# tyb311/TCCT

Hardware: AMD Instinct MI355X
Metric: OCT B-scans/sec fwd+bwd(+clip+AdamW), stc_tt bs=8 1x800x1100 (higher is better)
Workload: dtype bf16; 1 GPU; stc_tt --los=di bs=8/GPU 1x800x1100 (net tensors 3x800x1104); global_batch=8, parallelism=dp1, ranks=1, grad_allreduce=none, slowest_step=101

## Files before the change

include/tcct_hip.h:

```cpp
#ifndef TCCT_HIP_H
#define TCCT_HIP_H
#include <stdint.h>
#ifdef __cplusplus
extern "C" {
#endif

typedef void* tcct_stream_t;

enum { TCCT_F32 = 0, TCCT_BF16 = 1 };
enum { TCCT_ACT_NONE = 0, TCCT_ACT_LRELU = 1, TCCT_ACT_HSWISH = 2, TCCT_ACT_GELU = 3, TCCT_ACT_SIGMOID = 4,
       TCCT_ACT_ABS = 5 };

int tcct_version(void);
const char* tcct_last_error(void);
int tcct_set_outputs_prezeroed(int on);

int tcct_image_to_nhwc4(const float* img, void* out, int N, int Csrc, int H, int Wsrc, int Wdst, int dtype,
                        tcct_stream_t stream);
int tcct_u8_gather2d(const uint8_t* src, uint8_t* dst, int N, int SH, int SW, int C, int sy0, int sx0, int sh, int sw, int DH, int DW,
                     int dy0, int dx0, int dh, int dw, int flipy, int flipx, int mul, int div, int fill, tcct_stream_t stream);
int tcct_onehot_to_index(const int64_t* onehot, uint8_t* lab, int N, int C, int64_t HW, tcct_stream_t stream);
int tcct_labels_to_u8(const int64_t* lab, uint8_t* out, int N, int H, int Wsrc, int Wdst, tcct_stream_t stream);
int tcct_nhwc_to_nchw_f32(const void* x, float* y, int N, int64_t HW, int C, int dtype, tcct_stream_t stream);

// ... 74 lines not shown
                      int KW, int padh, int padw, int dy_dtype, int dx_dtype, tcct_stream_t stream);
int tcct_conv2d_wgrad(const void* x, const void* dy, float* dw, float* dbias, int N, int H, int W, int Cin,
                      int Cin_w, int Cout, int KH, int KW, int stride, int padh, int padw, int x_dtype, int dy_dtype,
                      tcct_stream_t stream);

int tcct_conv32f_pack_weights(const float* w, float* wp, int KH, int KW, int transposed, tcct_stream_t stream);
int tcct_conv32f_fwd(const float* x, const float* wp, const float* bias, const float* yadd, float* y, int N, int H, int W, int KH, int KW, int PH,
                     int PW, tcct_stream_t stream);
int tcct_conv32f_wgrad(const float* x, const float* dy, float* dw, float* dbias, int N, int H, int W, int KH, int KW, int PH, int PW,
                       tcct_stream_t stream);
int tcct_conv32f_pack_weights_sub(const float* w, float* wp, int KH, int KW, int transposed, int cin_total, int o_off, int i_off, tcct_stream_t stream);
int tcct_conv32f_fwd_strided(const float* x, const float* wp, const float* bias, float* y, int N, int H, int W, int KH, int KW, int PH, int PW, int xs,
                             int xo, int ys, int yo, int accumulate, tcct_stream_t stream);
int tcct_conv32f_wgrad_strided(const float* x, const float* dy, float* dw, float* dbias, int N, int H, int W, int KH, int KW, int PH, int PW, int xs,
                               int xo, int ds, int dof, int ldi, int o_off, int i_off, tcct_stream_t stream);
int tcct_pwf_fwd(const float* x, const float* w, const float* bias, float* y, int64_t M, int K, int N, int transposed, tcct_stream_t stream);
int tcct_pwf_wgrad(const float* x, const float* dy, float* dw, float* dbias, int64_t M, int K, int N, tcct_stream_t stream);
int tcct_conv32_pack_weights(const float* w, void* wp, int KH, int KW, int transposed, tcct_stream_t stream);
int tcct_conv32_pack_weights_multi(const void* desc, int n, tcct_stream_t stream);
int tcct_conv32_pack_weights_both(const float* w, void* wp2, int KH, int KW, tcct_stream_t stream);
int tcct_conv32_fwd(const void* x, const void* wp, const float* bias, void* y, int N, int H, int W, int KH, int KW, int PH,
                    int PW, tcct_stream_t stream);

int tcct_conv32_fwd_bnstats(const void* x, const void* wp, const float* bias, void* y, int N, int H, int W, int KH, int KW, int PH,
                            int PW, double* stats, int pre_act, tcct_stream_t stream);
int tcct_conv32_fwd_affine(const void* x, const void* wp, const float* bias, void* y, int N, int H, int W, int KH, int KW,
                           int PH, int PW, const float* ab, int pre_act, int post_act, tcct_stream_t stream);
int tcct_pw_fwd_affine(const void* x, const float* w, const float* bias, void* y, int64_t M, int K, int N, const float* ab,
                       int pre_act, int post_act, int out_dtype, tcct_stream_t stream);
int tcct_pw_fwd_affine_residual(const void* x, const float* w, const float* bias, const float* ab, const void* res, void* y, int64_t M, int K, int N,
                                tcct_stream_t stream);
int tcct_pw_fwd_cat2_affine(const void* x1, const void* x2, const float* w, const float* bias, const float* ab, int post_act, void* y, int64_t M, int K, int N,
                            tcct_stream_t stream);
int tcct_pw_fwd_xaff_affine_residual(const void* y_prev, const float* ab_prev, const float* w, const float* bias, const float* ab, const void* res, void* y,
                                     int64_t M, int K, int N, tcct_stream_t stream);
int tcct_conv32_fwd_add(const void* x, const void* wp, const float* bias, const void* res, void* y, int N, int H, int W, int KH, int KW,
                        int PH, int PW, tcct_stream_t stream);
int tcct_conv32_chain33(const void* x, const void* wp1, const float* bias1, void* mid, const void* wp2, const float* bias2, void* y,
                        const void* res, int N, int H, int W, double* stats, tcct_stream_t stream);
int tcct_conv32_pack_weights_sub(const float* w, void* wp, int KH, int KW, int transposed, int cin_total, int o_off, int i_off,
                                 tcct_stream_t stream);
int tcct_conv32_fwd_strided(const void* x, const void* wp, const float* bias, void* y, int N, int H, int W, int KH, int KW, int PH,
                            int PW, int xs, int xo, int ys, int yo, int accumulate, tcct_stream_t stream);
int tcct_conv32_fwd_strided_bnstats(const void* x, const void* wp, const float* bias, void* y, int N, int H, int W, int KH, int KW, int PH,
                                    int PW, int xs, int xo, int ys, int yo, int accumulate, double* stats, int pre_act, tcct_stream_t stream);
int tcct_conv32_fwd_strided_affine(const void* x, const void* wp, const float* bias, void* y, int N, int H, int W, int KH, int KW, int PH, int PW, int xs,
                                   int xo, int ys, int yo, const float* ab, int pre_act, int post_act, tcct_stream_t stream);
int64_t tcct_conv32_wgrad_mode(int mode);
int64_t tcct_conv32_fwd_mode(int mode);
int tcct_conv32_wgrad_strided(const void* x, const void* dy, float* dw, float* dbias, int N, int H, int W, int KH, int KW, int PH,
                              int PW, int xs, int xo, int ds, int dof, int cin_total, int o_off, int i_off, tcct_stream_t stream);
int tcct_conv32_wgrad(const void* x, const void* dy, float* dw, float* dbias, int N, int H, int W, int KH, int KW, int PH,
                      int PW, tcct_stream_t stream);
int tcct_conv32_bwd3x3(const void* x, const void* dy, const void* wp_t, const void* dskip, void* dx, float* dw, float* dbias, int N, int H,
                       int W, tcct_stream_t stream);

int tcct_pw_fwd(const void* x, const float* w, const float* bias, void* y, int64_t M, int K, int N, int transposed,
                int out_dtype, tcct_stream_t stream);
int tcct_pw_wgrad(const void* x, const void* dy, float* dw, float* dbias, int64_t M, int K, int N, tcct_stream_t stream);
int tcct_pw_bwd(const void* x, const void* dy, const float* w, const void* res, void* dx, float* dw, float* dbias, int64_t M, int K, int N,
                tcct_stream_t stream);
int tcct_pw_bwd_cat2(const void* x1, const void* x2, const void* dy, const float* w, void* dx1, void* dx2, float* dw, int64_t M, int K, int N,
                     tcct_stream_t stream);
int tcct_pw_bwd_residual2(const void* x, const void* dy, const float* w, const void* res, void* dx_sum, void* dx_plain, float* dw, float* dbias,
                          int64_t M, int K, int N, tcct_stream_t stream);
int64_t tcct_pw_bwd_bn_supported(int K, int N, int post, int red_post, int split);
int tcct_pw_bwd_bn(const void* x, const void* x2, const void* dz, const void* y, const float* coef, int post, const float* w, const void* res,
                   void* dx, void* dx2, float* dw, float* dbias, int64_t M, int K, int N, const void* y_prev, const float* ab_prev,
                   int red_post, double* sums_prev, tcct_stream_t stream);
int tcct_pw_bwd_bn_sums(const void* x, const void* x2, const void* dz, const void* y, const double* sums, int raw, const float* mean_rstd,
                        const float* ab, float* dgamma, float* dbeta, int post, const float* w, const void* res, void* dx, void* dx2, float* dw,
                        float* dbias, int64_t M, int K, int N, const void* y_prev, const float* ab_prev, int red_post, double* sums_prev,
                        tcct_stream_t stream);
int tcct_pw_wgrad_strided(const void* x, const void* dy, int64_t ldy, float* dw, float* dbias, int64_t M, int K, int N,
                          tcct_stream_t stream);
int tcct_pw_fwd_residual(const void* x, const float* w, const float* bias, const void* res, const float* scale, int64_t per_sample,
                         void* y, void* y_plain, int64_t M, int K, int N, tcct_stream_t stream);
int tcct_pw_fwd_bnstats_xaff(const void* y_prev, const float* ab_prev, const float* w, const float* bias, void* y, int64_t M, int K, int N, double* stats,
                             tcct_stream_t stream);
int tcct_pw_bwd_bn_sums_xaff(const void* y_prev, const float* ab_prev, const void* dz, const void* y, const double* sums, int raw, const float* mean_rstd,
                             const float* ab, float* dgamma, float* dbeta, const float* w, const void* res, void* dx, float* dw, float* dbias, int64_t M,
                             int K, int N, int red_post, double* sums_prev, tcct_stream_t stream);
int tcct_pw_fwd_gelu_residual(const void* x1, const float* w, const float* bias, const void* res, const float* scale, int64_t per_sample, void* y,
                              int64_t M, int K, int N, tcct_stream_t stream);
int tcct_pw_bwd_residual2_sum(const void* x, const void* dy_a, const void* dy_b, const float* w, const void* res, void* dx_sum, void* dx_plain, float* dw,
                              float* dbias, int64_t M, int K, int N, tcct_stream_t stream);
int tcct_pw_bwd_lnb(const void* x, const void* dy, const float* w, const void* t, const float* mean_rstd, const float* gamma, const void* res, void* dt,
                    float* dw, float* dbias, float* dgamma, float* dbeta, int64_t M, int K, int N, tcct_stream_t stream);
int tcct_pw_bwd_gelu(const void* x1, const void* dy, const float* w, void* dx1, float* dw, float* dbias, int64_t M, int K, int N, tcct_stream_t stream);
int tcct_pw_dgrad_residual(const void* dy, const float* w, const void* res, void* dx_sum, void* dx_plain, int64_t M, int Nout, int K,
                           tcct_stream_t stream);
int tcct_pw_fwd_cat2(const void* x1, const void* x2, int K1, const float* w, const float* bias, void* y, int64_t M, int K, int N,
                     double* stats, int pre_act, tcct_stream_t stream);
int tcct_pw_fwd_f32_upadd(const void* x, const float* w, const float* bias, float* y, int B, int uH, int uW, int K, int N, const float* up, tcct_stream_t stream);
int tcct_pw_dgrad_split2(const void* dy, const float* w, void* dx1, void* dx2, int K1, int64_t M, int Nout, int K, tcct_stream_t stream);
int tcct_pw_bwd_cat2_bias(const void* x1, const void* x2, const void* dy, const float* w, void* dx1, void* dx2, float* dw, float* dbias, int64_t M,
                          int K, int N, tcct_stream_t stream);
int tcct_tail_compose(const float* w1, const float* b1, const float* w2, const float* b2, float* wc, float* c, tcct_stream_t stream);
int tcct_tail_compose_bwd(const float* w1, const float* b1, const float* w2, const float* dwc, const float* dc, float* dw1, float* db1, float* dw2,
                          float* db2, tcct_stream_t stream);
int tcct_tail_compose3(const float* w1, const float* b1, const float* w2, const float* b2, const float* w3, const float* b3, int C, float* wcc, float* wa,
                       float* wb, float* ccc, tcct_stream_t stream);
int tcct_tail_compose3_bwd(const float* w1, const float* b1, const float* w2, const float* b2, const float* w3, int C, const float* dwa, const float* dwb,
                           const float* dccc, float* dw1, float* db1, float* dw2, float* db2, float* dw3, float* db3, tcct_stream_t stream);
int tcct_pw_fwd_cat2_f32(const void* x1, const void* x2, int K1, const float* w, const float* bias, float* y, int64_t M, int K, int N, tcct_stream_t stream);
int tcct_head_compose(const float* wt, const float* bt, const float* wa, const float* ba, int C, float* wh, float* ch, tcct_stream_t stream);
int tcct_head_compose_bwd(const float* wt, const float* bt, const float* wa, int C, const float* dwh, const float* dch, float* dwt, float* dbt,
                          float* dwa, float* dba, tcct_stream_t stream);
int tcct_pw_wgrad_cat2(const void* x1, const void* x2, int K1, const void* dy, float* dw, float* dbias, int64_t M, int K, int N,
                       tcct_stream_t stream);
int tcct_pw_fwd_bnstats(const void* x, const float* w, const float* bias, void* y, int64_t M, int K, int N, double* stats, int pre_act,
                        tcct_stream_t stream);

int tcct_im2col3x3_c3(const void* x4, void* out, int N, int H, int W, int stride, int dtype, tcct_stream_t stream);
int tcct_c3_fwd(const void* x4, const float* w, const float* bias, void* y, int B, int H, int W, int stride, double* stats, int stat_pre,
                const float* ab, int pre_act, int post_act, tcct_stream_t stream);
int tcct_c3_wgrad(const void* x4, const void* dy, float* dw, float* dbias, int B, int H, int W, int stride, tcct_stream_t stream);
int tcct_c3_bn_fwd_train(const void* x4, const float* w, const float* bias, void* z, int B, int H, int W, int stride, double* sums,
                         const float* gamma, const float* beta, float eps, float momentum, float* running_mean, float* running_var,
                         int64_t* num_batches_tracked, float* mean_rstd, float* ab, int post_act, tcct_stream_t stream);
int tcct_c3_bn_fwd_eval(const void* x4, const float* w, const float* bias, void* z, int B, int H, int W, int stride, const float* ab, int post_act,
                        tcct_stream_t stream);
int tcct_c3_bn_bwd_reduce(const void* x4, const float* w, const float* bias, const void* dz, int B, int H, int W, int stride, const float* ab,
                          double* raw, int post_act, tcct_stream_t stream);
int tcct_c3_bn_bwd_wgrad(const void* x4, const float* w, const float* bias, const void* dz, int B, int H, int W, int stride, const float* coef,
                         float* dw, float* dbias, int post_act, tcct_stream_t stream);
int64_t tcct_c3_bn_bwd_prefetch(int tiles_ahead);
int tcct_c3_bn_bwd_onepass(const void* x4, const float* w, const float* bias, const void* dz, int B, int H, int W, int stride, const float* mean_rstd,
                           const float* ab, float* work, double* sums, float* dw, float* dbias, float* dgamma, float* dbeta, int post_act, tcct_stream_t stream);
int tcct_pw_wgrad_smalln(const void* x, const void* dy, float* dw, float* dbias, int64_t M, int K, int N, int x_dtype,
                         int dy_dtype, tcct_stream_t stream);

int tcct_stream_copy(const void* src, void* dst, int64_t nbytes, tcct_stream_t stream);

int64_t tcct_kernel_census(int which, int reset);
int tcct_marker(int id, tcct_stream_t stream);

int tcct_dwconv3x3_fwd(const void* x, const float* w, const float* bias, void* y, int N, int H, int W, int C,
                       int stride, int add_input, int dtype, tcct_stream_t stream);
int tcct_dwconv3x3_fwd_bnstats(const void* x, const float* w, const float* bias, void* y, int N, int H, int W, int C, int stride,
                               int add_input, double* stats, int dtype, tcct_stream_t stream);
int tcct_dwconv3x3_dgrad(const void* dy, const float* w, void* dx, int N, int H, int W, int C, int stride,
                         int add_input, int dtype, tcct_stream_t stream);
int tcct_dwconv3x3_dgrad_add(const void* dy, const float* w, const void* res, void* dx, int N, int H, int W, int C, int stride,
                             int add_input, int dtype, tcct_stream_t stream);
int tcct_dwconv3x3_wgrad(const void* x, const void* dy, float* dw, float* dbias, int N, int H, int W, int C,
                         int stride, int dtype, tcct_stream_t stream);
int tcct_dwconv3x3_fwd_xaff(const void* x, const float* xab, const float* w, const float* bias, void* y, int N, int H, int W, int C, int stride,
                            double* stats, int dtype, tcct_stream_t stream);
int tcct_dwconv3x3_wgrad_xaff(const void* x, const float* xab, const void* dy, float* dw, float* dbias, int N, int H, int W, int C, int stride, int dtype,
                              tcct_stream_t stream);
int tcct_dwconv3x3_dgrad_bnred(const void* dy, const float* w, const void* y_prev, const float* ab_prev, void* dx, double* raw, int N, int H, int W, int C,
                               int dtype, tcct_stream_t stream);

int tcct_metapool_fwd(const void* x, void* y, int B, int64_t N, int C, int dtype, tcct_stream_t stream);
int tcct_metapool_bwd(const void* dy, void* dx, int B, int64_t N, int C, int dtype, tcct_stream_t stream);
int tcct_metapool_residual_fwd(const void* x, const void* res, const float* scale, void* y, int B, int64_t N, int C, int dtype,
                               tcct_stream_t stream);
int tcct_metapool_scaled_bwd(const void* dy, const float* scale, void* dx, int B, int64_t N, int C, int dtype, tcct_stream_t stream);
int tcct_ln_metapool_residual_fwd(const void* t, void* y, int B, int64_t N, int C, const float* gamma, const float* beta, float eps, const float* scale,
                                  int dtype, tcct_stream_t stream);
int tcct_ln_metapool_residual_ln_fwd(const void* t, void* y, void* y2, int B, int64_t N, int C, const float* gamma, const float* beta, float eps,
                                     const float* scale, const float* gamma2, const float* beta2, float eps2, float* mean_rstd2, int dtype, tcct_stream_t stream);
int tcct_ln_metapool_residual_bwd(const void* t, const void* dy, void* dt, int B, int64_t N, int C, const float* gamma, float eps, const float* scale,
                                  float* dgamma, float* dbeta, int dtype, tcct_stream_t stream);
int tcct_maxpool2_fwd(const void* x, void* y, int N, int H, int W, int C, int dtype, tcct_stream_t stream);
int tcct_maxpool2_bwd(const void* x, const void* dy, void* dx, int N, int H, int W, int C, int dtype, tcct_stream_t stream);
int tcct_maxpool2_bwd_add(const void* x, const void* dy, const void* res, void* dx, int N, int H, int W, int C, int dtype,
                          tcct_stream_t stream);
int tcct_bilinear_fwd(const void* x, void* y, int N, int H, int W, int C, int Ho, int Wo, int align_corners, int dtype,
                      tcct_stream_t stream);
int tcct_bilinear_bwd_separable(const float* dy, float* dx, float* workspace, int N, int H, int W, int C, int Ho, int Wo,
                                int align_corners, tcct_stream_t stream);
int tcct_bilinear_add_fwd(const void* x, const void* res, void* y, int N, int H, int W, int C, int Ho, int Wo, int align_corners,
                          int dtype, tcct_stream_t stream);
int64_t tcct_bilinear_bwd_x2(int on);
int tcct_bilinear_bwd(const void* dy, void* dx, int N, int H, int W, int C, int Ho, int Wo, int align_corners, int dtype,
                      tcct_stream_t stream);
int tcct_l2norm_fwd(const void* x, void* y, int64_t M, int C, float eps, int dtype, tcct_stream_t stream);
int tcct_l2norm_bwd(const void* x, const void* dy, void* dx, int64_t M, int C, float eps, int dtype, tcct_stream_t stream);
int tcct_l2norm_bwd_scaled(const void* x, const void* dy, void* dx, int64_t M, int C, float eps, float scale, int dtype,
                           tcct_stream_t stream);
int tcct_l2norm_bwd_scaled_add(const void* x, const void* dy, const void* res, void* dx, int64_t M, int C, float eps, float scale, int dtype,
                               tcct_stream_t stream);
int tcct_normadd_fwd(const void* g0, const void* g1, const void* g2, float* inv1, float* inv2, void* out, int N, int H, int W, int C,
                     int h1, int w1, int h2, int w2, float eps, int dtype, tcct_stream_t stream);

int tcct_softmax_dice_fwd(const void* logits, const uint8_t* labels, int64_t M, int C, double* sums, float* loss,
                          int dtype, tcct_stream_t stream);
int tcct_softmax_dice_bwd(const void* logits, const uint8_t* labels, int64_t M, int C, const double* sums,
                          const float* grad_out, float grad_scale, void* dlogits, int dtype, tcct_stream_t stream);
int tcct_updice_fwd(const float* low, const uint8_t* labels, int B, int h, int w, int H, int W, int C, double* sums, float* loss,
                    tcct_stream_t stream);
int tcct_updice_bwd(const float* low, const uint8_t* labels, int B, int h, int w, int H, int W, int C, const double* sums,
                    const float* grad_out, float grad_scale, float* ws, float* dlow, tcct_stream_t stream);
int tcct_dice_ds_fwd(const void* logits, int dtype, const uint8_t* labels, int B, int H, int W, int C, const float* low1, int h1, int w1, const float* low2,
                     int h2, int w2, const float* low3, int h3, int w3, float coff, double* sums, float* loss, tcct_stream_t stream);
int tcct_softmax_pick(const void* logits, const uint8_t* labels, int64_t M, int C, float* prob_lab, uint8_t* argmax,
                      int dtype, tcct_stream_t stream);
int tcct_confusion_counts(const uint8_t* pred, const uint8_t* labels, int N, int64_t HW, int C, float* out,
                          tcct_stream_t stream);

int tcct_gate_fusion_fwd(const void* x1, const void* x2, const float* field, void* y, int N, int H, int W, int C, int hs, int ws,
                         int dtype, tcct_stream_t stream);
int tcct_gate_fusion_bwd(const void* dy, const float* field, void* dx1, void* dx2, int N, int H, int W, int C, int hs, int ws,
                         int dtype, tcct_stream_t stream);

int tcct_mask_boundaries(const uint8_t* mask, int32_t* out, int N, int H, int W, int C, tcct_stream_t stream);

int tcct_slice_channels_fwd(const void* x, float* y, int64_t M, int C, int start, int n, int dtype, tcct_stream_t stream);
int tcct_slice_channels_bwd(const float* dy, void* dx, int64_t M, int C, int start, int n, int dtype, tcct_stream_t stream);
int tcct_label_planes(const uint8_t* labels, float* onehot, float* edge, int N, int H, int W, int start, int n,
                      tcct_stream_t stream);
int tcct_gumbel_colsoftmax_fwd(const float* x, const float* eps, float* out, float* stats, int N, int H, int W, int CH,
                               tcct_stream_t stream);
int tcct_gumbel_colsoftmax_bwd(const float* x, const float* eps, const float* stats, const float* dout, float* dx, int N,
                               int H, int W, int CH, tcct_stream_t stream);
int tcct_colsoftmax_fwd(const float* x, float* y, int N, int H, int W, tcct_stream_t stream);
int tcct_colsoftmax_bwd(const float* y, const float* dy, float* dx, int N, int H, int W, tcct_stream_t stream);
int tcct_colwsum_fwd(const float* x, const float* wts, float* out, int N, int H, int W, tcct_stream_t stream);
int tcct_colwsum_bwd(const float* dout, const float* wts, float* dx, int N, int H, int W, tcct_stream_t stream);
int tcct_mse_fwd(const float* a, const float* b, int64_t n, double* acc, float* out, tcct_stream_t stream);
int tcct_mse_bwd(const float* a, const float* b, int64_t n, const float* grad_out, float grad_scale, float* da, float* db,
                 tcct_stream_t stream);

int64_t tcct_fpl_select_workspace_bytes();
int tcct_fpl_select(const void* feat, const uint8_t* labels, const float* prob, int64_t M, int C, void* workspace, uint32_t* counts,
                    uint8_t* binmap, float* pro_sum, int dtype, tcct_stream_t stream);
int tcct_fpl_loss(const float* pro_sum, const uint32_t* counts, const float* buf_grad, int C, float* pro, float* loss, float* dpro_over_n,
                  tcct_stream_t stream);
int tcct_fpl_backward(const uint8_t* labels, const uint8_t* binmap, const float* dpro_over_n, const float* grad_out,
                      float grad_scale, int64_t M, void* dfeat, int dtype, tcct_stream_t stream);
int tcct_l2norm_bwd_fplgrad(const void* x, const uint8_t* labels, const uint8_t* binmap, const float* dpro_over_n, const float* grad_out,
                            float grad_scale, int ncls, const void* res, void* dx, int64_t M, float eps, float scale, int dtype, tcct_stream_t stream);
int tcct_bilinear_bwd_fplgrad(const uint8_t* labels, const uint8_t* binmap, const float* dpro_over_n, const float* grad_out, float grad_scale, int ncls,
                              void* dx, int N, int H, int W, int Ho, int Wo, int align_corners, int dtype, tcct_stream_t stream);

int64_t tcct_fatt_kstats_workspace_bytes(int B, int64_t N, int C);
int tcct_fatt_kstats(const void* qkv, void* workspace, float* stats, int B, int64_t N, int C, int heads, int dtype, tcct_stream_t stream);
int tcct_fatt_ktv(const void* qkv, const float* stats, float* M, int B, int64_t N, int C, int heads, int dtype, tcct_stream_t stream);
int tcct_fatt_dktv(const void* qkv, const void* dout, float* dM, float scale, int B, int64_t N, int C, int heads, int dtype,
                   tcct_stream_t stream);
int tcct_fatt_apply_fwd(const void* qkv, const float* M, const void* cv, void* out, float scale, int B, int64_t N, int C, int heads,
                        int dtype, tcct_stream_t stream);
int tcct_fatt_apply_bwd(const void* qkv, const float* stats, const float* M, const float* dM, const void* cv, const void* dout,
                        void* dqkv, void* dcv, float scale, int B, int64_t N, int C, int heads, int dtype, tcct_stream_t stream);
int tcct_dwk_strided_fwd(const void* x, int64_t ldx, const float* w, const float* bias, void* y, int64_t ldy, int B, int H, int W, int Cg,
                         int K, int flip, int accumulate, int dtype, tcct_stream_t stream);
int tcct_dwk_strided_wgrad(const void* x, int64_t ldx, const void* dy, int64_t ldy, float* dw, float* dbias, int B, int H, int W, int Cg,
                           int K, int dtype, tcct_stream_t stream);

int tcct_grad_sumsq(const float* g, int64_t n, double* acc, tcct_stream_t stream);
int tcct_clip_adamw(float* p, const float* g, float* m, float* v, int64_t n, const double* sumsq, float max_norm,
                    float grad_mul, float lr, double beta1, double beta2, float eps, float weight_decay, int step,
                    float* total_norm_out, tcct_stream_t stream);

int tcct_clip_adamw_dev(float* p, const float* g, float* m, float* v, int64_t n, const double* sumsq, float max_norm,
                        float grad_mul, float* state, double beta1, double beta2, float eps, float weight_decay,
                        float* total_norm_out, tcct_stream_t stream);

#ifdef __cplusplus
}
#endif
#endif
```

tcct_amd/csrc/dwconv.hip:

```cpp
#include "common.h"
#include <cstdlib>
#include <type_traits>

#define DB 256

template <typename T, int VEC>
__device__ __forceinline__ void ldv(const T* p, float* o) {
    if (VEC == 4) { f4 a = ld4(p); o[0] = a.v[0]; o[1] = a.v[1]; o[2] = a.v[2]; o[3] = a.v[3]; }
    else o[0] = ldf(p);
}
template <typename T, int VEC>
__device__ __forceinline__ void stv(T* p, const float* o) {
    if (VEC == 4) { f4 a; a.v[0] = o[0]; a.v[1] = o[1]; a.v[2] = o[2]; a.v[3] = o[3]; st4(p, a); }
    else stf(p, o[0]);
}

struct DwPos { int n, ho0, ho1, wo, c; };
__device__ __forceinline__ bool dw_pos(int C, int VEC, int Ho, int Wo, int segh, int wblocks, int hstrips, DwPos& p, int cpt = 1) {
    const int CV = C / VEC, PW = DB / CV, t = threadIdx.x;
    if (t >= PW * CV) return false;
    int bid = (int)xcd_band(blockIdx.x, gridDim.x);
    const int wb = bid % wblocks; bid /= wblocks;
    const int hs = bid % hstrips;
    p.n = bid / hstrips;
// ... 177 lines not shown
                        for (int ky = 0; ky < 3; ++ky)
#pragma unroll
                            for (int kx = 0; kx < 3; ++kx) a += R[j * STRIDE + ky][cc + kx].get(k) * wk[ky * 3 + kx][k];
                        if (add_input) a += R[j * STRIDE + 1][cc + 1].get(k);
                        acc[k] = a;
                    }
                    const bool live = ho + j < p.ho1 && cout[cc] != DW_OOB;
                    dw_storeb(ry, live ? (uint32_t)(ho + j) * (uint32_t)(Wo * C) * ES + cout[cc] : DW_OOB, acc, (const T*)nullptr);
                    if (stats && live) {
                        if (aux_mode) {
#pragma unroll
                            for (int k = 0; k < VEC; ++k) {
                                const float yv = RS[j][cc].get(k), u = xa[k] * yv + xb[k];
                                const float d = dw_rnd(acc[k], (const T*)nullptr) * (u < -3.f ? 0.f : (u <= 3.f ? (2.f * u + 3.f) * (1.f / 6.f) : 1.f));
                                st_s[k] += (SAcc)d; st_q[k] += (SAcc)d * (SAcc)yv;
                            }
                        } else {
#pragma unroll
                            for (int k = 0; k < VEC; ++k) { const SAcc r = dw_rnd(acc[k], (const T*)nullptr); st_s[k] += r; st_q[k] += r * r; }
                        }
                    }
                }
            }
#pragma unroll
            for (int i = 0; i < K::CARRY; ++i)
#pragma unroll
                for (int kx = 0; kx < NC; ++kx) R[i][kx] = R[NEWC + i][kx];
#pragma unroll
            for (int i = 0; i < NEWC; ++i)
#pragma unroll
                for (int kx = 0; kx < NC; ++kx) R[K::CARRY + i][kx] = NX[i][kx];
#pragma unroll
            for (int j = 0; j < RBC; ++j)
#pragma unroll
                for (int cc = 0; cc < CPT; ++cc) RS[j][cc] = RSN[j][cc];
        }
    } else {
#pragma unroll
    for (int i = 0; i < ROWSC; ++i) dw_load_row<T, VEC, NC>(R[i], img, p.ho0 * STRIDE - 1 + i, H, W, C, wi0);
    for (int ho = p.ho0; ho < p.ho1; ho += RBC) {
        if (ho + RBC < p.ho1) {
#pragma unroll
            for (int i = 0; i < NEWC; ++i) dw_load_row<T, VEC, NC>(NX[i], img, (ho + RBC) * STRIDE - 1 + K::CARRY + i, H, W, C, wi0);
        }
#pragma unroll
        for (int j = 0; j < RBC; ++j) {
            if (ho + j < p.ho1) {
#pragma unroll
                for (int cc = 0; cc < CPT; ++cc) {
                    if (CPT > 1 && p.wo + cc >= Wo) break;
                    float acc[VEC];
                    Raw<T, VEC> rr;
                    if (rin) rr.load(rin + ((int64_t)(ho + j) * Wo + p.wo + cc) * C); else rr.zero();
#pragma unroll
                    for (int k = 0; k < VEC; ++k) {
                        float a = bv[k] + rr.get(k);
#pragma unroll
                        for (int ky = 0; ky < 3; ++ky)
#pragma unroll
                            for (int kx = 0; kx < 3; ++kx) a += R[j * STRIDE + ky][cc + kx].get(k) * wk[ky * 3 + kx][k];
                        if (add_input) a += R[j * STRIDE + 1][cc + 1].get(k);
                        acc[k] = a;
                    }
                    stv<T, VEC>(out + ((int64_t)(ho + j) * Wo + p.wo + cc) * C, acc);
                }
            }
        }
#pragma unroll
        for (int i = 0; i < K::CARRY; ++i)
#pragma unroll
            for (int kx = 0; kx < NC; ++kx) R[i][kx] = R[NEWC + i][kx];
#pragma unroll
        for (int i = 0; i < NEWC; ++i)
#pragma unroll
            for (int kx = 0; kx < NC; ++kx) R[K::CARRY + i][kx] = NX[i][kx];
    }
    }
    }
    if (VEC == 4 && stats) {
        const int CV = C / VEC, PW = DB / CV, t = threadIdx.x;
#pragma unroll
        for (int k = 0; k < VEC; ++k) { s_red[t * 8 + k] = st_s[k]; s_red[t * 8 + 4 + k] = st_q[k]; }
        __syncthreads();
        if (t < C) {
            const int cvv = t / VEC, k = t % VEC;
            double a = 0.0, b = 0.0;
            for (int pp = 0; pp < PW; ++pp) { a += (double)s_red[(pp * CV + cvv) * 8 + k]; b += (double)s_red[(pp * CV + cvv) * 8 + 4 + k]; }
            atomicAdd(&stats[t], a); atomicAdd(&stats[C + t], b);
        }
    }
}

static void dw_geometry(int N, int Ho, int Wo, int C, int vec, int target_blocks, int max_segh, int& segh, int& wblocks, int& hstrips,
                        int cpt = 1) {
    const int PW = DB / (C / vec) * cpt;
    wblocks = (Wo + PW - 1) / PW;
    segh = max_segh;
    while (segh > 8 && (int64_t)N * wblocks * ((Ho + segh - 1) / segh) < target_blocks) segh >>= 1;
    hstrips = (Ho + segh - 1) / segh;
}

template <typename T, int VEC, bool FLIP, int MODE = 0>
static void dw_fwd_launch(const void* x, const float* w, const float* bias, void* y, int N, int H, int W, int C, int stride,
                          int Ho, int Wo, int add_input, hipStream_t st, const void* res = nullptr, double* stats = nullptr, const float* xab = nullptr) {
    int segh, wblocks, hstrips;
    static int cpt_on = -1;
    if (cpt_on < 0) cpt_on = 1;
    if (stride == 1 && VEC == 4 && sizeof(T) == 2 && cpt_on && Wo >= 128 && C >= 32) {
        dw_geometry(N, Ho, Wo, C, VEC, 1024, 32, segh, wblocks, hstrips, 4);
        dim3 g4((unsigned)((int64_t)N * wblocks * hstrips));
        hipLaunchKernelGGL((k_dw_fwd<T, VEC, 1, FLIP, (VEC == 4 ? 4 : 1), MODE>), g4, dim3(DB), 0, st, (const T*)x, w, bias, (T*)y, N, H, W, C, Ho, Wo, add_input, segh, wblocks, hstrips, (const T*)res, stats, xab);
        return;
    }
    dw_geometry(N, Ho, Wo, C, VEC, 1024, 32, segh, wblocks, hstrips);
    dim3 g((unsigned)((int64_t)N * wblocks * hstrips)), b(DB);
    if (stride == 1) hipLaunchKernelGGL((k_dw_fwd<T, VEC, 1, FLIP, 1, MODE>), g, b, 0, st, (const T*)x, w, bias, (T*)y, N, H, W, C, Ho, Wo, add_input, segh, wblocks, hstrips, (const T*)res, stats, xab);
    else hipLaunchKernelGGL((k_dw_fwd<T, VEC, 2, FLIP, 1, MODE>), g, b, 0, st, (const T*)x, w, bias, (T*)y, N, H, W, C, Ho, Wo, add_input, segh, wblocks, hstrips, (const T*)res, stats, xab);
}

extern "C" int tcct_dwconv3x3_fwd(const void* x, const float* w, const float* bias, void* y, int N, int H, int W, int C,
                                  int stride, int add_input, int dtype, tcct_stream_t stream) {
    TCCT_CHECK(stride == 1 || stride == 2, "dwconv3x3_fwd: stride %d", stride);
    TCCT_CHECK(!(add_input && stride != 1), "dwconv3x3_fwd: add_input needs stride 1");
    TCCT_CHECK(N >= 1 && H >= 1 && W >= 1 && C >= 1, "dwconv3x3_fwd: empty tensor");
    int Ho = (H + 2 - 3) / stride + 1, Wo = (W + 2 - 3) / stride + 1;
    int vec = (C % 4 == 0) ? 4 : 1;
    TCCT_CHECK(C / vec <= DB, "dwconv3x3_fwd: C=%d too large", C);
    TCCT_CHECK((int64_t)H * W * C * 4 < (1ll << 31), "dwconv3x3_fwd: one image of %d x %d x %d elements exceeds the 32-bit byte offsets of the kernels", H, W, C);
    hipStream_t st = (hipStream_t)stream;
    if (vec == 4) { TCCT_DISPATCH(dtype, (dw_fwd_launch<T, 4, false>(x, w, bias, y, N, H, W, C, stride, Ho, Wo, add_input, st))); }
    else { TCCT_DISPATCH(dtype, (dw_fwd_launch<T, 1, false>(x, w, bias, y, N, H, W, C, stride, Ho, Wo, add_input, st))); }
    TCCT_LAUNCH_OK();
}
extern "C" int tcct_dwconv3x3_fwd_bnstats(const void* x, const float* w, const float* bias, void* y, int N, int H, int W, int C, int stride,
                                          int add_input, double* stats, int dtype, tcct_stream_t stream) {
    TCCT_CHECK(stride == 1 || stride == 2, "dwconv3x3_fwd_bnstats: stride %d", stride);
    TCCT_CHECK(!(add_input && stride != 1), "dwconv3x3_fwd_bnstats: add_input needs stride 1");
    TCCT_CHECK(N >= 1 && H >= 1 && W >= 1 && C >= 4 && C % 4 == 0 && C <= DB && stats != nullptr, "dwconv3x3_fwd_bnstats: needs C %% 4 == 0, C <= 256, stats");
    TCCT_CHECK((int64_t)H * W * C * 4 < (1ll << 31), "dwconv3x3_fwd_bnstats: one image of %d x %d x %d elements exceeds the 32-bit byte offsets of the kernels", H, W, C);
    int Ho = (H + 2 - 3) / stride + 1, Wo = (W + 2 - 3) / stride + 1;
    TCCT_DISPATCH(dtype, (dw_fwd_launch<T, 4, false>(x, w, bias, y, N, H, W, C, stride, Ho, Wo, add_input, (hipStream_t)stream, nullptr, stats)));
    TCCT_LAUNCH_OK();
}
extern "C" int tcct_dwconv3x3_fwd_xaff(const void* x, const float* xab, const float* w, const float* bias, void* y, int N, int H, int W, int C, int stride,
                                       double* stats, int dtype, tcct_stream_t stream) {
    TCCT_CHECK(stride == 1 || stride == 2, "dwconv3x3_fwd_xaff: stride %d", stride);
    TCCT_CHECK(N >= 1 && H >= 1 && W >= 1 && C >= 4 && C % 4 == 0 && C <= DB && xab != nullptr, "dwconv3x3_fwd_xaff: needs C %% 4 == 0, C <= 256, xab");
    TCCT_CHECK((int64_t)H * W * C * 4 < (1ll << 31), "dwconv3x3_fwd_xaff: one image of %d x %d x %d elements exceeds the 32-bit byte offsets of the kernels", H, W, C);
    int Ho = (H + 2 - 3) / stride + 1, Wo = (W + 2 - 3) / stride + 1;
    TCCT_DISPATCH(dtype, (dw_fwd_launch<T, 4, false, 1>(x, w, bias, y, N, H, W, C, stride, Ho, Wo, 0, (hipStream_t)stream, nullptr, stats, xab)));
    TCCT_LAUNCH_OK();
}

template <typename T, int VEC>
__global__ void __launch_bounds__(DB) k_dw_dgrad_s2(const T* __restrict__ dy, const float* __restrict__ w, T* __restrict__ dx,
                                                    int N, int H, int W, int C, int Ho, int Wo, int segh, int wblocks, int hstrips,
                                                    const T* __restrict__ res) {
    const int Qh = (H + 1) / 2, Qw = (W + 1) / 2;
    DwPos p;
    if (!dw_pos(C, VEC, Qh, Qw, segh, wblocks, hstrips, p)) return;
    float wk[9][VEC];
#pragma unroll
    for (int k = 0; k < VEC; ++k)
#pragma unroll
        for (int tp = 0; tp < 9; ++tp) wk[tp][k] = w[(p.c + k) * 9 + tp];
    const T* g = dy + (int64_t)p.n * Ho * Wo * C + p.c;
    T* out = dx + (int64_t)p.n * H * W * C + p.c;
    const T* rin = res ? res + (int64_t)p.n * H * W * C + p.c : nullptr;
    const int b = p.wo;
    if (VEC == 4) {
        const uint32_t ES = sizeof(T), in_bytes = (uint32_t)H * W * C * ES;
        const int nu = __builtin_amdgcn_readfirstlane(p.n);
        const __amdgpu_buffer_rsrc_t rg = __builtin_amdgcn_make_buffer_rsrc((void*)(dy + (int64_t)nu * Ho * Wo * C), 0, (uint32_t)Ho * Wo * C * ES, 0x00020000);
        const __amdgpu_buffer_rsrc_t ro = __builtin_amdgcn_make_buffer_rsrc((void*)(dx + (int64_t)nu * H * W * C), 0, in_bytes, 0x00020000);
        const __amdgpu_buffer_rsrc_t rr = __builtin_amdgcn_make_buffer_rsrc((void*)((res ? res : dx) + (int64_t)nu * H * W * C), 0, res ? in_bytes : 0u, 0x00020000);
        const uint32_t cg0 = (uint32_t)(b * C + p.c) * ES, cg1 = b + 1 < Wo ? cg0 + (uint32_t)C * ES : DW_OOB;
        const uint32_t co0 = (uint32_t)(2 * b * C + p.c) * ES, co1 = 2 * b + 1 < W ? co0 + (uint32_t)C * ES : DW_OOB;
        auto ldb = [&](Raw<T, VEC> (&d)[2], int a) {
            const bool rok = a < Ho;
            const uint32_t r0 = (uint32_t)a * (uint32_t)(Wo * C) * ES;
            d[0].loadb(rg, rok ? r0 + cg0 : DW_OOB);
            d[1].loadb(rg, (rok && cg1 != DW_OOB) ? r0 + cg1 : DW_OOB);
        };
        auto ldr = [&](Raw<T, VEC> (&q)[4], int a, bool live) {
            const uint32_t r0 = (uint32_t)(2 * a) * (uint32_t)(W * C) * ES, r1 = r0 + (uint32_t)(W * C) * ES;
            const bool row1 = live && 2 * a + 1 < H;
            q[0].loadb(rr, live ? r0 + co0 : DW_OOB);
            q[1].loadb(rr, (live && co1 != DW_OOB) ? r0 + co1 : DW_OOB);
            q[2].loadb(rr, row1 ? r1 + co0 : DW_OOB);
            q[3].loadb(rr, (row1 && co1 != DW_OOB) ? r1 + co1 : DW_OOB);
        };
        auto emitb = [&](const Raw<T, VEC> (&u)[2], const Raw<T, VEC> (&v)[2], const Raw<T, VEC> (&q)[4], int a, bool live) {
            float o00[VEC], o01[VEC], o10[VEC], o11[VEC];
#pragma unroll
            for (int k = 0; k < VEC; ++k) {
                const float u0 = u[0].get(k), u1 = u[1].get(k), v0 = v[0].get(k), v1 = v[1].get(k);
                o00[k] = u0 * wk[4][k] + q[0].get(k);
                o01[k] = u0 * wk[5][k] + u1 * wk[3][k] + q[1].get(k);
                o10[k] = u0 * wk[7][k] + v0 * wk[1][k] + q[2].get(k);
                o11[k] = u0 * wk[8][k] + u1 * wk[6][k] + v0 * wk[2][k] + v1 * wk[0][k] + q[3].get(k);
            }
            const uint32_t r0 = (uint32_t)(2 * a) * (uint32_t)(W * C) * ES, r1 = r0 + (uint32_t)(W * C) * ES;
            const bool row1 = live && 2 * a + 1 < H;
            dw_storeb(ro, live ? r0 + co0 : DW_OOB, o00, (const T*)nullptr);
            dw_storeb(ro, (live && co1 != DW_OOB) ? r0 + co1 : DW_OOB, o01, (const T*)nullptr);
            dw_storeb(ro, row1 ? r1 + co0 : DW_OOB, o10, (const T*)nullptr);
            dw_storeb(ro, (row1 && co1 != DW_OOB) ? r1 + co1 : DW_OOB, o11, (const T*)nullptr);
        };
        Raw<T, VEC> d0[2], d1[2], d2[2], n1[2], n2[2], q0[4], q1[4], m0[4], m1[4];
        ldb(d0, p.ho0); ldb(d1, p.ho0 + 1); ldb(d2, p.ho0 + 2);
        ldr(q0, p.ho0, true); ldr(q1, p.ho0 + 1, p.ho0 + 1 < p.ho1);
        for (int a = p.ho0; a < p.ho1; a += 2) {
            const bool more = a + 2 < p.ho1;
            ldb(n1, more ? a + 3 : Ho); ldb(n2, more ? a + 4 : Ho);
            ldr(m0, a + 2, more); ldr(m1, a + 3, a + 3 < p.ho1);
            emitb(d0, d1, q0, a, true);
            emitb(d1, d2, q1, a + 1, a + 1 < p.ho1);
#pragma unroll
            for (int j = 0; j < 2; ++j) { d0[j] = d2[j]; d1[j] = n1[j]; d2[j] = n2[j]; }
#pragma unroll
            for (int j = 0; j < 4; ++j) { q0[j] = m0[j]; q1[j] = m1[j]; }
        }
        return;
    }
    auto ld = [&](float (&d)[2][VEC], int a) {
#pragma unroll
        for (int j = 0; j < 2; ++j) {
            if (a < Ho && b + j < Wo) ldv<T, VEC>(g + ((int64_t)a * Wo + b + j) * C, d[j]);
            else {
#pragma unroll
                for (int k = 0; k < VEC; ++k) d[j][k] = 0.f;
            }
        }
    };
    auto emit = [&](const float (&u)[2][VEC], const float (&v)[2][VEC], int a) {
        float o00[VEC], o01[VEC], o10[VEC], o11[VEC];
#pragma unroll
        for (int k = 0; k < VEC; ++k) {
            o00[k] = u[0][k] * wk[4][k];
            o01[k] = u[0][k] * wk[5][k] + u[1][k] * wk[3][k];
            o10[k] = u[0][k] * wk[7][k] + v[0][k] * wk[1][k];
            o11[k] = u[0][k] * wk[8][k] + u[1][k] * wk[6][k] + v[0][k] * wk[2][k] + v[1][k] * wk[0][k];
        }
        const int hi = 2 * a, wi = 2 * b;
        T* o = out + ((int64_t)hi * W + wi) * C;
        if (rin) {
            const T* ri = rin + ((int64_t)hi * W + wi) * C;
            float r[VEC];
            ldv<T, VEC>(ri, r);
#pragma unroll
            for (int k = 0; k < VEC; ++k) o00[k] += r[k];
            if (wi + 1 < W) {
                ldv<T, VEC>(ri + C, r);
#pragma unroll
                for (int k = 0; k < VEC; ++k) o01[k] += r[k];
            }
            if (hi + 1 < H) {
                ldv<T, VEC>(ri + (int64_t)W * C, r);
#pragma unroll
                for (int k = 0; k < VEC; ++k) o10[k] += r[k];
                if (wi + 1 < W) {
                    ldv<T, VEC>(ri + (int64_t)W * C + C, r);
#pragma unroll
                    for (int k = 0; k < VEC; ++k) o11[k] += r[k];
                }
            }
        }
        stv<T, VEC>(o, o00);
        if (wi + 1 < W) stv<T, VEC>(o + C, o01);
        if (hi + 1 < H) {
            stv<T, VEC>(o + (int64_t)W * C, o10);
            if (wi + 1 < W) stv<T, VEC>(o + (int64_t)W * C + C, o11);
        }
    };
    float d0[2][VEC], d1[2][VEC];
    ld(d0, p.ho0);
    for (int a = p.ho0; a < p.ho1; a += 2) {
        ld(d1, a + 1);
        emit(d0, d1, a);
        if (a + 1 >= p.ho1) break;
        ld(d0, a + 2);
        emit(d1, d0, a + 1);
    }
}

static int dw_dgrad_impl(const void* dy, const float* w, const void* res, void* dx, int N, int H, int W, int C, int stride,
                         int add_input, int dtype, tcct_stream_t stream) {
    TCCT_CHECK(stride == 1 || stride == 2, "dwconv3x3_dgrad: stride %d", stride);
    TCCT_CHECK(!(add_input && stride != 1), "dwconv3x3_dgrad: add_input needs stride 1");
    TCCT_CHECK(N >= 1 && H >= 1 && W >= 1 && C >= 1, "dwconv3x3_dgrad: empty tensor");
    int Ho = (H + 2 - 3) / stride + 1, Wo = (W + 2 - 3) / stride + 1;
    int vec = (C % 4 == 0) ? 4 : 1;
    TCCT_CHECK(C / vec <= DB, "dwconv3x3_dgrad: C=%d too large", C);
    TCCT_CHECK((int64_t)H * W * C * 4 < (1ll << 31), "dwconv3x3_dgrad: one image of %d x %d x %d elements exceeds the 32-bit byte offsets of the kernels", H, W, C);
    hipStream_t st = (hipStream_t)stream;
    if (stride == 1) {
        if (vec == 4) { TCCT_DISPATCH(dtype, (dw_fwd_launch<T, 4, true>(dy, w, nullptr, dx, N, H, W, C, 1, H, W, add_input, st, res))); }
        else { TCCT_DISPATCH(dtype, (dw_fwd_launch<T, 1, true>(dy, w, nullptr, dx, N, H, W, C, 1, H, W, add_input, st, res))); }
        TCCT_LAUNCH_OK();
    }
    int segh, wblocks, hstrips;
    dw_geometry(N, (H + 1) / 2, (W + 1) / 2, C, vec, 1024, 32, segh, wblocks, hstrips);
    dim3 g((unsigned)((int64_t)N * wblocks * hstrips)), b(DB);
    if (vec == 4) { TCCT_DISPATCH(dtype, hipLaunchKernelGGL((k_dw_dgrad_s2<T, 4>), g, b, 0, st, (const T*)dy, w, (T*)dx, N, H, W, C, Ho, Wo, segh, wblocks, hstrips, (const T*)res)); }
    else { TCCT_DISPATCH(dtype, hipLaunchKernelGGL((k_dw_dgrad_s2<T, 1>), g, b, 0, st, (const T*)dy, w, (T*)dx, N, H, W, C, Ho, Wo, segh, wblocks, hstrips, (const T*)res)); }
    TCCT_LAUNCH_OK();
}
extern "C" int tcct_dwconv3x3_dgrad(const void* dy, const float* w, void* dx, int N, int H, int W, int C, int stride,
                                    int add_input, int dtype, tcct_stream_t stream) {
    return dw_dgrad_impl(dy, w, nullptr, dx, N, H, W, C, stride, add_input, dtype, stream);
}
extern "C" int tcct_dwconv3x3_dgrad_add(const void* dy, const float* w, const void* res, void* dx, int N, int H, int W, int C,
                                        int stride, int add_input, int dtype, tcct_stream_t stream) {
    TCCT_CHECK(res != nullptr, "dwconv3x3_dgrad_add: res is NULL");
    return dw_dgrad_impl(dy, w, res, dx, N, H, W, C, stride, add_input, dtype, stream);
}

extern "C" int tcct_dwconv3x3_dgrad_bnred(const void* dy, const float* w, const void* y_prev, const float* ab_prev, void* dx, double* raw, int N, int H, int W,
                                          int C, int dtype, tcct_stream_t stream) {
    TCCT_CHECK(N >= 1 && H >= 1 && W >= 1 && C >= 4 && C % 4 == 0 && C <= DB && y_prev && ab_prev && raw, "dwconv3x3_dgrad_bnred: needs C %% 4 == 0, C <= 256, y_prev, ab_prev, raw");
    TCCT_CHECK((int64_t)H * W * C * 4 < (1ll << 31), "dwconv3x3_dgrad_bnred: one image of %d x %d x %d elements exceeds the 32-bit byte offsets of the kernels", H, W, C);
    TCCT_DISPATCH(dtype, (dw_fwd_launch<T, 4, true, 2>(dy, w, nullptr, dx, N, H, W, C, 1, H, W, 0, (hipStream_t)stream, y_prev, raw, ab_prev)));
    TCCT_LAUNCH_OK();
}

template <typename T, int VEC, int STRIDE, int CPT = 1, bool XAFF = false>
__global__ void __launch_bounds__(DB) k_dw_wgrad(const T* __restrict__ x, const T* __restrict__ dy, float* __restrict__ dw,
                                                 float* __restrict__ dbias, int N, int H, int W, int C, int Ho, int Wo, int segh,
                                                 int wblocks, int hstrips, const float* __restrict__ xab = nullptr) {
    static_assert(CPT == 1 || (STRIDE == 1 && VEC == 4), "several columns per thread: stride 1, 4-channel vectors");
    constexpr int NC = CPT + 2;
    extern __shared__ float sm[];
    const int CV = C / VEC, PW = DB / CV;
    const int t = threadIdx.x;
    float acc[10][VEC];
#pragma unroll
    for (int a = 0; a < 10; ++a)
#pragma unroll
        for (int k = 0; k < VEC; ++k) acc[a][k] = 0.f;
    typedef DwChunk<STRIDE> K;
    DwPos p;
    if (dw_pos(C, VEC, Ho, Wo, segh, wblocks, hstrips, p, CPT)) {
        const T* img = x + (int64_t)p.n * H * W * C + p.c;
        const T* gimg = dy + (int64_t)p.n * Ho * Wo * C + p.c;
        const int wi0 = p.wo * STRIDE - 1;
      if (VEC == 4) {
        Raw<T, VEC> R[K::ROWS][NC], NX[K::NEW][NC], G[K::RB][CPT], GX[K::RB][CPT];
        const uint32_t ES = sizeof(T);
        const int nu = __builtin_amdgcn_readfirstlane(p.n);
        const __amdgpu_buffer_rsrc_t rx = __builtin_amdgcn_make_buffer_rsrc((void*)(x + (int64_t)nu * H * W * C), 0, (uint32_t)H * W * C * ES, 0x00020000);
        const __amdgpu_buffer_rsrc_t rg = __builtin_amdgcn_make_buffer_rsrc((void*)(dy + (int64_t)nu * Ho * Wo * C), 0, (uint32_t)Ho * Wo * C * ES, 0x00020000);
        uint32_t cin[NC], cg[CPT];
#pragma unroll
        for (int kx = 0; kx < NC; ++kx) cin[kx] = (unsigned)(wi0 + kx) < (unsigned)W ? (uint32_t)((wi0 + kx) * C + p.c) * ES : DW_OOB;
#pragma unroll
        for (int cc = 0; cc < CPT; ++cc) cg[cc] = p.wo + cc < Wo ? (uint32_t)((p.wo + cc) * C + p.c) * ES : DW_OOB;
        auto load_row = [&](Raw<T, VEC> (&r)[NC], int hi, bool live) {
            const bool rok = live && (unsigned)hi < (unsigned)H;
            const uint32_t ro = (uint32_t)hi * (uint32_t)(W * C) * ES;
#pragma unroll
            for (int kx = 0; kx < NC; ++kx) r[kx].loadb(rx, (rok && cin[kx] != DW_OOB) ? ro + cin[kx] : DW_OOB);
        };
        auto load_g = [&](Raw<T, VEC> (&g)[K::RB][CPT], int ho) {
#pragma unroll
            for (int j = 0; j < K::RB; ++j)
#pragma unroll
                for (int cc = 0; cc < CPT; ++cc)
                    g[j][cc].loadb(rg, (ho + j < p.ho1 && cg[cc] != DW_OOB) ? (uint32_t)(ho + j) * (uint32_t)(Wo * C) * ES + cg[cc] : DW_OOB);
        };
#pragma unroll
        for (int i = 0; i < K::ROWS; ++i) load_row(R[i], p.ho0 * STRIDE - 1 + i, true);
        float xa[VEC], xb[VEC];
#pragma unroll
        for (int k = 0; k < VEC; ++k) { xa[k] = XAFF ? xab[p.c + k] : 1.f; xb[k] = XAFF ? xab[C + p.c + k] : 0.f; }
        auto xf_row = [&](Raw<T, VEC> (&r)[NC], int hi, bool live) {
            const bool rok = live && (unsigned)hi < (unsigned)H;
#pragma unroll
            for (int kx = 0; kx < NC; ++kx) r[kx] = dw_xf(r[kx], xa, xb, rok && cin[kx] != DW_OOB);
        };
        if (XAFF) {
#pragma unroll
            for (int i = 0; i < K::CARRY; ++i) xf_row(R[i], p.ho0 * STRIDE - 1 + i, true);
        }
        load_g(G, p.ho0);
        for (int ho = p.ho0; ho < p.ho1; ho += K::RB) {
            const bool more = ho + K::RB < p.ho1;
#pragma unroll
            for (int i = 0; i < K::NEW; ++i) load_row(NX[i], (ho + K::RB) * STRIDE - 1 + K::CARRY + i, more);
            load_g(GX, ho + K::RB);
            if (XAFF) {
#pragma unroll
                for (int i = 0; i < K::NEW; ++i) xf_row(R[K::CARRY + i], ho * STRIDE - 1 + K::CARRY + i, true);
            }
#pragma unroll
            for (int j = 0; j < K::RB; ++j) {
#pragma unroll
                for (int cc = 0; cc < CPT; ++cc) {
#pragma unroll
                    for (int k = 0; k < VEC; ++k) {
                        const float g = G[j][cc].get(k);
                        acc[9][k] += g;
#pragma unroll
                        for (int ky = 0; ky < 3; ++ky)
#pragma unroll
                            for (int kx = 0; kx < 3; ++kx) acc[ky * 3 + kx][k] += R[j * STRIDE + ky][cc + kx].get(k) * g;
                    }
                }
            }
#pragma unroll
            for (int i = 0; i < K::CARRY; ++i)
#pragma unroll
                for (int kx = 0; kx < NC; ++kx) R[i][kx] = R[K::NEW + i][kx];
#pragma unroll
            for (int i = 0; i < K::NEW; ++i)
#pragma unroll
                for (int kx = 0; kx < NC; ++kx) R[K::CARRY + i][kx] = NX[i][kx];
#pragma unroll
            for (int j = 0; j < K::RB; ++j)
#pragma unroll
                for (int cc = 0; cc < CPT; ++cc) G[j][cc] = GX[j][cc];
        }
      } else {
        Raw<T, VEC> R[K::ROWS][3], NX[K::NEW][3], G[K::RB], GX[K::RB];
#pragma unroll
        for (int i = 0; i < K::ROWS; ++i) dw_load_row<T, VEC>(R[i], img, p.ho0 * STRIDE - 1 + i, H, W, C, wi0);
#pragma unroll
        for (int j = 0; j < K::RB; ++j) {
            if (p.ho0 + j < p.ho1) G[j].load(gimg + ((int64_t)(p.ho0 + j) * Wo + p.wo) * C);
            else G[j].zero();
        }
        for (int ho = p.ho0; ho < p.ho1; ho += K::RB) {
            if (ho + K::RB < p.ho1) {
#pragma unroll
                for (int i = 0; i < K::NEW; ++i) dw_load_row<T, VEC>(NX[i], img, (ho + K::RB) * STRIDE - 1 + K::CARRY + i, H, W, C, wi0);
#pragma unroll
                for (int j = 0; j < K::RB; ++j) {
                    if (ho + K::RB + j < p.ho1) GX[j].load(gimg + ((int64_t)(ho + K::RB + j) * Wo + p.wo) * C);
                    else GX[j].zero();
                }
            }
#pragma unroll
            for (int j = 0; j < K::RB; ++j) {
#pragma unroll
                for (int k = 0; k < VEC; ++k) {
                    const float g = G[j].get(k);
                    acc[9][k] += g;
#pragma unroll
                    for (int ky = 0; ky < 3; ++ky)
#pragma unroll
                        for (int kx = 0; kx < 3; ++kx) acc[ky * 3 + kx][k] += R[j * STRIDE + ky][kx].get(k) * g;
                }
            }
#pragma unroll
            for (int i = 0; i < K::CARRY; ++i)
#pragma unroll
                for (int kx = 0; kx < 3; ++kx) R[i][kx] = R[K::NEW + i][kx];
#pragma unroll
            for (int i = 0; i < K::NEW; ++i)
#pragma unroll
                for (int kx = 0; kx < 3; ++kx) R[K::CARRY + i][kx] = NX[i][kx];
#pragma unroll
            for (int j = 0; j < K::RB; ++j) G[j] = GX[j];
        }
      }
    }
#pragma unroll
    for (int a = 0; a < 10; ++a)
#pragma unroll
        for (int k = 0; k < VEC; ++k) sm[(t * 10 + a) * VEC + k] = acc[a][k];
    __syncthreads();
    for (int o = t; o < C * 10; o += DB) {
        int ch = o / 10, a = o % 10;
        int cvv = ch / VEC, k = ch % VEC;
        float s = 0.f;
        for (int pp = 0; pp < PW; ++pp) s += sm[((pp * CV + cvv) * 10 + a) * VEC + k];
// ... 51 lines not shown
```

tcct_amd/csrc/pw_mfma.hip:

```cpp
#include "common.h"
#include "c3_geom.h"
#include <cstdlib>

typedef __attribute__((ext_vector_type(8))) __bf16 bf16x8;
typedef __attribute__((ext_vector_type(16))) float f32x16;
typedef __attribute__((ext_vector_type(4))) short s16x4;
typedef __attribute__((ext_vector_type(8))) short s16x8;
typedef __attribute__((__vector_size__(4 * sizeof(unsigned int)))) unsigned int u32x4;

#define PWB 256

__device__ __forceinline__ void st_out4(bf16* p, float a, float b, float c, float d) {
    uint2 o; o.x = pack_bf16x2(a, b); o.y = pack_bf16x2(c, d);
    *reinterpret_cast<uint2*>(p) = o;
}
__device__ __forceinline__ void st_out4(float* p, float a, float b, float c, float d) {
    *reinterpret_cast<float4*>(p) = make_float4(a, b, c, d);
}

__device__ __forceinline__ float rnd_out(float v, const bf16*) { return __bfloat162float(__float2bfloat16(v)); }
__device__ __forceinline__ float rnd_out(float v, const float*) { return v; }

struct PwUp { const float* p; int uH, uW, Ho, Wo; float sh, sw; uint32_t m_howo, m_wo; };
struct PwSplit { const bf16* x2; int K1; void* y2; int N1; const bf16* res; const float* rscale; int64_t per_sample; bf16* yplain; C3Geom c3; PwUp up; };
// ... 1038 lines not shown
                    }
                };
                if (SPLIT) {
                    const uint32_t off2 = mm < M ? (uint32_t)((mm * KS + (kt * 32) % KS + cch * 8) * 2) : 0x80000000u;
                    __builtin_amdgcn_raw_buffer_store_b128(o, kt * 32 < KS ? ro : rp, off2, 0, 0);
                    if (RED && kt < RKT) red_acc(o, kt * 32 + cch * 8);
                    continue;
                }
                const uint32_t off = mm < M ? (uint32_t)((mm * K + kt * 32 + cch * 8) * 2) : 0x80000000u;
                if (GX) {
                    const u32x4 xv = xq[GX ? kt : 0][h2];
#pragma unroll
                    for (int k = 0; k < 4; ++k)
                        o[k] = pack_bf16x2(__uint_as_float(o[k] << 16) * gelu_grad1(__uint_as_float(xv[k] << 16)),
                                           __uint_as_float(o[k] & 0xffff0000u) * gelu_grad1(__uint_as_float(xv[k] & 0xffff0000u)));
                }
                if (res) {
                    if (dx_plain) __builtin_amdgcn_raw_buffer_store_b128(o, rp, off, 0, 0);
                    const u32x4 rv = __builtin_amdgcn_raw_buffer_load_b128(rr, off, 0, 0);
#pragma unroll
                    for (int k = 0; k < 4; ++k)
                        o[k] = pack_bf16x2(__uint_as_float(o[k] << 16) + __uint_as_float(rv[k] << 16),
                                           __uint_as_float(o[k] & 0xffff0000u) + __uint_as_float(rv[k] & 0xffff0000u));
                }
                __builtin_amdgcn_raw_buffer_store_b128(o, ro, off, 0, 0);
                if (RED) red_acc(o, kt * 32 + cch * 8);
            }
            wave_lds_fence();
        }
        __syncthreads();
    }
    if (RED) {
        __syncthreads();
        float* red = reinterpret_cast<float*>(smem);
        constexpr int KR = SPLIT ? K / 2 : K;
#pragma unroll
        for (int kt = 0; kt < RKT; ++kt) {
#pragma unroll
            for (int k = 0; k < 8; ++k) {
                float a = rs[kt][k], b = rq[kt][k];
#pragma unroll
                for (int o = 32; o > 2; o >>= 1) { a += __shfl_xor(a, o, 64); b += __shfl_xor(b, o, 64); }
                if (lane < 4) {
                    red[wave * 2 * KR + kt * 32 + 8 * lane + k] = a;
                    red[wave * 2 * KR + KR + kt * 32 + 8 * lane + k] = b;
                }
            }
        }
        __syncthreads();
        for (int i2 = tid; i2 < KR; i2 += PWB) {
            double a = 0.0, b = 0.0;
#pragma unroll
            for (int wv = 0; wv < 4; ++wv) { a += (double)red[wv * 2 * KR + i2]; b += (double)red[wv * 2 * KR + KR + i2]; }
            atomicAdd(&bn.sums_prev[i2], a); atomicAdd(&bn.sums_prev[KR + i2], b);
        }
        __syncthreads();
    }
    if (LNB) {
        __syncthreads();
        float* red = reinterpret_cast<float*>(smem);
#pragma unroll
        for (int kt = 0; kt < KT; ++kt) {
#pragma unroll
            for (int k = 0; k < 8; ++k) {
                float a = rs[kt][k], b = rq[kt][k];
#pragma unroll
                for (int o = 32; o > 2; o >>= 1) { a += __shfl_xor(a, o, 64); b += __shfl_xor(b, o, 64); }
                if (lane < 4) {
                    red[wave * 2 * K + kt * 32 + 8 * lane + k] = a;
                    red[wave * 2 * K + K + kt * 32 + 8 * lane + k] = b;
                }
            }
        }
        __syncthreads();
        for (int i2 = tid; i2 < K; i2 += PWB) {
            float a = 0.f, b = 0.f;
#pragma unroll
            for (int wv = 0; wv < 4; ++wv) { a += red[wv * 2 * K + i2]; b += red[wv * 2 * K + K + i2]; }
            atomicAdd(&bn.dgamma[i2], a); atomicAdd(&bn.dbeta[i2], b);
        }
        __syncthreads();
    }
#pragma unroll
    for (int a = 0; a < (NT * KT + 3) / 4; ++a) {
        const int ti = wave + 4 * a;
        if (ti < NT * KT) {
            const int ct = ti / KT, kt = ti - ct * KT;
#pragma unroll
            for (int k = 0; k < 16; ++k) {
                const int co = ct * 32 + (k & 3) + 8 * (k >> 2) + 4 * hh;
                atomicAdd(&dw[(int64_t)co * K + kt * 32 + r], accw[a][k]);
            }
            if (dbias && kt == 0) {
                const float sb = bsum[a] + __shfl_xor(bsum[a], 32, 64);
                if (lane < 32) atomicAdd(&dbias[ct * 32 + r], sb);
            }
        }
    }
}

static int pw_bwd_impl(const void* x, const void* dy, const float* w, const void* res, void* dx, void* dx_plain, float* dw, float* dbias,
                       int64_t M, int K, int N, tcct_stream_t stream, bool split = false, int bnp = -1, int redp = -1,
                       PwBnBwd bn = PwBnBwd{nullptr, nullptr, nullptr, nullptr, nullptr, nullptr, 0, nullptr, nullptr, nullptr, nullptr}, bool gelu_x = false,
                       int xap = -1, bool lnb = false, bool dy2 = false);
extern "C" int tcct_pw_bwd_cat2(const void* x1, const void* x2, const void* dy, const float* w, void* dx1, void* dx2, float* dw, int64_t M,
                                int K, int N, tcct_stream_t stream) {
    TCCT_CHECK(K == 128 && x2 != nullptr && dx2 != nullptr, "pw_bwd_cat2: two halves of 64 channels only (K=%d)", K);
    return pw_bwd_impl(x1, dy, w, x2, dx1, dx2, dw, nullptr, M, K, N, stream, true);
}
extern "C" int tcct_pw_bwd_cat2_bias(const void* x1, const void* x2, const void* dy, const float* w, void* dx1, void* dx2, float* dw, float* dbias,
                                     int64_t M, int K, int N, tcct_stream_t stream) {
    TCCT_CHECK((K == 128 || (K == 64 && N == 32)) && x2 != nullptr && dx2 != nullptr, "pw_bwd_cat2_bias: K=%d N=%d (128 -> any, or 64 -> 32)", K, N);
    return pw_bwd_impl(x1, dy, w, x2, dx1, dx2, dw, dbias, M, K, N, stream, true);
}
extern "C" int tcct_pw_bwd(const void* x, const void* dy, const float* w, const void* res, void* dx, float* dw, float* dbias, int64_t M,
                           int K, int N, tcct_stream_t stream) {
    return pw_bwd_impl(x, dy, w, res, dx, nullptr, dw, dbias, M, K, N, stream);
}
extern "C" int tcct_pw_bwd_residual2(const void* x, const void* dy, const float* w, const void* res, void* dx_sum, void* dx_plain, float* dw,
                                     float* dbias, int64_t M, int K, int N, tcct_stream_t stream) {
    TCCT_CHECK(res != nullptr && dx_plain != nullptr && dx_plain != dx_sum, "pw_bwd_residual2: needs res and two distinct outputs");
    return pw_bwd_impl(x, dy, w, res, dx_sum, dx_plain, dw, dbias, M, K, N, stream);
}
extern "C" int64_t tcct_pw_bwd_bn_supported(int K, int N, int post, int red_post, int split) {
    const bool p_ok = post == TCCT_ACT_NONE || post == TCCT_ACT_HSWISH;
    const bool r_ok = red_post == -1 || red_post == TCCT_ACT_NONE || red_post == TCCT_ACT_HSWISH;
    if (!p_ok || !r_ok) return 0;
    if (split) return K == 128 && N == 96 && post == TCCT_ACT_HSWISH && red_post == -1;
    if (K == N && (K == 64 || K == 96)) return red_post == -1 || K == 64;
    if (N == 32 && (K == 32 || K == 96 || K == 128)) return red_post == -1 && post == TCCT_ACT_NONE;
    return 0;
}
static int pw_bwd_bn_impl(const void* x, const void* x2, const void* dz, PwBnBwd bn, int post, const float* w, const void* res, void* dx, void* dx2,
                          float* dw, float* dbias, int64_t M, int K, int N, int red_post, tcct_stream_t stream);
extern "C" int tcct_pw_bwd_bn(const void* x, const void* x2, const void* dz, const void* y, const float* coef, int post, const float* w,
                              const void* res, void* dx, void* dx2, float* dw, float* dbias, int64_t M, int K, int N, const void* y_prev,
                              const float* ab_prev, int red_post, double* sums_prev, tcct_stream_t stream) {
    TCCT_CHECK(coef != nullptr, "pw_bwd_bn: coef is NULL");
    return pw_bwd_bn_impl(x, x2, dz, PwBnBwd{(const bf16*)y, coef, (const bf16*)y_prev, ab_prev, sums_prev, nullptr, 0, nullptr, nullptr, nullptr, nullptr},
                          post, w, res, dx, dx2, dw, dbias, M, K, N, red_post, stream);
}
extern "C" int tcct_pw_bwd_bn_sums(const void* x, const void* x2, const void* dz, const void* y, const double* sums, int raw, const float* mean_rstd,
                                   const float* ab, float* dgamma, float* dbeta, int post, const float* w, const void* res, void* dx, void* dx2,
                                   float* dw, float* dbias, int64_t M, int K, int N, const void* y_prev, const float* ab_prev, int red_post,
                                   double* sums_prev, tcct_stream_t stream) {
    TCCT_CHECK(sums && mean_rstd && ab && dgamma && dbeta, "pw_bwd_bn_sums: NULL argument");
    return pw_bwd_bn_impl(x, x2, dz, PwBnBwd{(const bf16*)y, nullptr, (const bf16*)y_prev, ab_prev, sums_prev, sums, raw, mean_rstd, ab, dgamma, dbeta},
                          post, w, res, dx, dx2, dw, dbias, M, K, N, red_post, stream);
}
extern "C" int tcct_pw_bwd_bn_sums_xaff(const void* y_prev, const float* ab_prev, const void* dz, const void* y, const double* sums, int raw,
                                        const float* mean_rstd, const float* ab, float* dgamma, float* dbeta, const float* w, const void* res, void* dx,
                                        float* dw, float* dbias, int64_t M, int K, int N, int red_post, double* sums_prev, tcct_stream_t stream) {
    TCCT_CHECK(y_prev && ab_prev && sums && mean_rstd && ab && dgamma && dbeta, "pw_bwd_bn_sums_xaff: NULL argument");
    TCCT_CHECK(K == N && ((K == 64 && red_post == TCCT_ACT_HSWISH && sums_prev) || (K == 96 && red_post < 0)), "pw_bwd_bn_sums_xaff: K=%d N=%d red_post=%d unsupported", K, N, red_post);
    if (red_post >= 0 && !tcct_skip_zero_fill() && hipMemsetAsync(sums_prev, 0, sizeof(double) * 2 * K, (hipStream_t)stream) != hipSuccess) { tcct_set_error("pw_bwd_bn_sums_xaff: memset failed"); return -2; }
    return pw_bwd_impl(y_prev, dz, w, res, dx, nullptr, dw, dbias, M, K, N, stream, false, TCCT_ACT_NONE, red_post,
                       PwBnBwd{(const bf16*)y, nullptr, (const bf16*)y_prev, ab_prev, sums_prev, sums, raw, mean_rstd, ab, dgamma, dbeta}, false, TCCT_ACT_HSWISH);
}
static int pw_bwd_bn_impl(const void* x, const void* x2, const void* dz, PwBnBwd bn, int post, const float* w, const void* res, void* dx, void* dx2,
                          float* dw, float* dbias, int64_t M, int K, int N, int red_post, tcct_stream_t stream) {
    const void* y = bn.y; const void* y_prev = bn.yprev; const float* ab_prev = bn.abprev; double* sums_prev = bn.sums_prev;
    const bool split = x2 != nullptr;
    TCCT_CHECK(tcct_pw_bwd_bn_supported(K, N, post, red_post, split ? 1 : 0), "pw_bwd_bn: K=%d N=%d post=%d red_post=%d split=%d unsupported", K, N, post,
               red_post, (int)split);
    TCCT_CHECK(y != nullptr && (red_post < 0 || (y_prev && ab_prev && sums_prev)), "pw_bwd_bn: NULL argument");
    TCCT_CHECK(!split || (dx2 != nullptr && res == nullptr), "pw_bwd_bn: the concatenated form takes x2 / dx2 and no residual");
    if (red_post >= 0 && !tcct_skip_zero_fill() &&
        hipMemsetAsync(sums_prev, 0, sizeof(double) * 2 * (split ? K / 2 : K), (hipStream_t)stream) != hipSuccess) { tcct_set_error("pw_bwd_bn: memset failed"); return -2; }
    return pw_bwd_impl(x, dz, w, split ? x2 : res, dx, split ? dx2 : nullptr, dw, dbias, M, K, N, stream, split, post, red_post, bn);
}
extern "C" int tcct_pw_bwd_gelu(const void* x1, const void* dy, const float* w, void* dx1, float* dw, float* dbias, int64_t M, int K, int N,
                                tcct_stream_t stream) {
    TCCT_CHECK(K == N && (K == 64 || K == 96), "pw_bwd_gelu: K=%d N=%d unsupported (64 or 96 square; 128 spills 30 VGPRs)", K, N);
    return pw_bwd_impl(x1, dy, w, nullptr, dx1, nullptr, dw, dbias, M, K, N, stream, false, -1, -1,
                       PwBnBwd{nullptr, nullptr, nullptr, nullptr, nullptr, nullptr, 0, nullptr, nullptr, nullptr, nullptr}, true);
}
extern "C" int tcct_pw_bwd_residual2_sum(const void* x, const void* dy_a, const void* dy_b, const float* w, const void* res, void* dx_sum, void* dx_plain, float* dw,
                                         float* dbias, int64_t M, int K, int N, tcct_stream_t stream) {
    TCCT_CHECK(K == 32 && N == 32, "pw_bwd_residual2_sum: K=%d N=%d unsupported (32 x 32)", K, N);
    TCCT_CHECK(dy_b != nullptr && res != nullptr && dx_plain != nullptr && dx_plain != dx_sum, "pw_bwd_residual2_sum: needs dy_b, res and two distinct outputs");
    return pw_bwd_impl(x, dy_a, w, res, dx_sum, dx_plain, dw, dbias, M, K, N, stream, false, -1, -1,
                       PwBnBwd{(const bf16*)dy_b, nullptr, nullptr, nullptr, nullptr, nullptr, 0, nullptr, nullptr, nullptr, nullptr}, false, -1, false, true);
}
extern "C" int tcct_pw_bwd_lnb(const void* x, const void* dy, const float* w, const void* t, const float* mean_rstd, const float* gamma, const void* res,
                               void* dt, float* dw, float* dbias, float* dgamma, float* dbeta, int64_t M, int K, int N, tcct_stream_t stream) {
    TCCT_CHECK(K == 64 && N == 64, "pw_bwd_lnb: K=%d N=%d unsupported (64 x 64)", K, N);
    TCCT_CHECK(t && mean_rstd && gamma && res && dgamma && dbeta, "pw_bwd_lnb: NULL argument");
    hipStream_t st = (hipStream_t)stream;
    if (!tcct_skip_zero_fill() && (hipMemsetAsync(dgamma, 0, sizeof(float) * K, st) != hipSuccess || hipMemsetAsync(dbeta, 0, sizeof(float) * K, st) != hipSuccess)) {
        tcct_set_error("pw_bwd_lnb: memset failed"); return -2;
    }
    return pw_bwd_impl(x, dy, w, res, dt, nullptr, dw, dbias, M, K, N, stream, false, -1, -1,
                       PwBnBwd{nullptr, nullptr, (const bf16*)t, gamma, nullptr, nullptr, 0, mean_rstd, nullptr, dgamma, dbeta}, false, -1, true);
}
static int pw_bwd_impl(const void* x, const void* dy, const float* w, const void* res, void* dx, void* dx_plain, float* dw, float* dbias,
                       int64_t M, int K, int N, tcct_stream_t stream, bool split, int bnp, int redp, PwBnBwd bn, bool gelu_x, int xap, bool lnb, bool dy2) {
    TCCT_CHECK(K % 32 == 0 && N % 32 == 0 && K >= 32 && N >= 32 && K <= 128 && N <= 128, "pw_bwd: K=%d N=%d unsupported (32..128)", K, N);
    TCCT_CHECK(M > 0 && M * (int64_t)(K > N ? K : N) * 2 < (1LL << 31), "pw_bwd: tensor exceeds the 2 GiB buffer-descriptor range");
    hipStream_t st = (hipStream_t)stream;
    if (!tcct_skip_zero_fill() && hipMemsetAsync(dw, 0, sizeof(float) * (size_t)N * K, st) != hipSuccess) { tcct_set_error("pw_bwd: memset failed"); return -2; }
    if (dbias && !tcct_skip_zero_fill() && hipMemsetAsync(dbias, 0, sizeof(float) * N, st) != hipSuccess) { tcct_set_error("pw_bwd: memset failed"); return -2; }
    const int NT = N / 32, KT = K / 32;
    const int SX = 64 * KT + ((KT & 1) ? 0 : 64), SD = 64 * NT + ((NT & 1) ? 0 : 64), SW = 2 * N + 16;
    const size_t lds = (size_t)PB_P * (SX + SD) + (((size_t)K * SW + 15) & ~(size_t)15) + 4 * 2560 + (bnp >= 0 ? (size_t)5 * N * 4 : 0) +
                       ((redp >= 0 || xap >= 0 || lnb) ? (size_t)2 * K * 4 : 0);
    TCCT_CHECK(lds <= 160 * 1024, "pw_bwd: %zu B of LDS", lds);
    const int64_t tiles = (M + PB_P - 1) / PB_P;
    int per_cu = (int)((160 * 1024) / (lds + 256));
    if (per_cu > 2) per_cu = 2;
    int64_t gx = 256 * per_cu;
    if (gx > tiles) gx = tiles;
#define BLX(NTV, KTV, SPV, BNV, RDV) { static bool at_ = false; if (!at_) { (void)hipFuncSetAttribute((const void*)k_pw_bwd<NTV, KTV, SPV, BNV, RDV>, hipFuncAttributeMaxDynamicSharedMemorySize, 160 * 1024); at_ = true; } \
        hipLaunchKernelGGL((k_pw_bwd<NTV, KTV, SPV, BNV, RDV>), dim3((unsigned)gx), dim3(PWB), lds, st, (const bf16*)x, (const bf16*)dy, w, (const bf16*)res, (bf16*)dx, (bf16*)dx_plain, dw, dbias, M, bn); }
    if (dy2) {
        { static bool at_ = false; if (!at_) { (void)hipFuncSetAttribute((const void*)k_pw_bwd<1, 1, false, -1, -1, false, -1, false, true>, hipFuncAttributeMaxDynamicSharedMemorySize, 160 * 1024); at_ = true; }
          hipLaunchKernelGGL((k_pw_bwd<1, 1, false, -1, -1, false, -1, false, true>), dim3((unsigned)gx), dim3(PWB), lds, st, (const bf16*)x, (const bf16*)dy, w, (const bf16*)res, (bf16*)dx, (bf16*)dx_plain, dw, dbias, M, bn); }
        TCCT_LAUNCH_OK();
    }
    if (lnb) {
#define BLN(T) { static bool at_ = false; if (!at_) { (void)hipFuncSetAttribute((const void*)k_pw_bwd<T, T, false, -1, -1, false, -1, true>, hipFuncAttributeMaxDynamicSharedMemorySize, 160 * 1024); at_ = true; } \
        hipLaunchKernelGGL((k_pw_bwd<T, T, false, -1, -1, false, -1, true>), dim3((unsigned)gx), dim3(PWB), lds, st, (const bf16*)x, (const bf16*)dy, w, (const bf16*)res, (bf16*)dx, (bf16*)dx_plain, dw, dbias, M, bn); }
        BLN(2)
#undef BLN
        TCCT_LAUNCH_OK();
    }
    if (xap >= 0) {
#define BLXA(NTV, RDV) { static bool at_ = false; if (!at_) { (void)hipFuncSetAttribute((const void*)k_pw_bwd<NTV, NTV, false, 0, RDV, false, 2>, hipFuncAttributeMaxDynamicSharedMemorySize, 160 * 1024); at_ = true; } \
        hipLaunchKernelGGL((k_pw_bwd<NTV, NTV, false, 0, RDV, false, 2>), dim3((unsigned)gx), dim3(PWB), lds, st, (const bf16*)x, (const bf16*)dy, w, (const bf16*)res, (bf16*)dx, (bf16*)dx_plain, dw, dbias, M, bn); }
        if (NT == 2 && redp == TCCT_ACT_HSWISH) BLXA(2, 2) else if (NT == 3 && redp < 0) BLXA(3, -1)
        else { tcct_set_error("pw_bwd: x-affine form K=N=%d red_post=%d has no kernel", K, redp); return -1; }
#undef BLXA
        TCCT_LAUNCH_OK();
    }
    if (bnp >= 0) {
        const int H = TCCT_ACT_HSWISH;
#define BN_SQ(T) \
        if (bnp == 0 && redp < 0) BLX(T, T, false, 0, -1) else BLX(T, T, false, 2, -1)
#define BN_SQR(T) \
        if (bnp == 0 && redp == 0) BLX(T, T, false, 0, 0) else if (bnp == 0 && redp == H) BLX(T, T, false, 0, 2) \
        else if (bnp == H && redp == 0) BLX(T, T, false, 2, 0) else BLX(T, T, false, 2, 2)
        static_assert(TCCT_ACT_HSWISH == 2 && TCCT_ACT_NONE == 0, "activation codes are template arguments below");
        if (split) BLX(3, 4, true, 2, -1)
        else if (NT == 1 && KT == 1) BLX(1, 1, false, 0, -1)
        else if (NT == 1 && KT == 3) BLX(1, 3, false, 0, -1)
        else if (NT == 1 && KT == 4) BLX(1, 4, false, 0, -1)
        else if (NT == 2) { if (redp < 0) { BN_SQ(2) } else { BN_SQR(2) } }
        else { BN_SQ(3) }
#undef BN_SQ
#undef BN_SQR
        TCCT_LAUNCH_OK();
    }
    if (gelu_x) {
#define BLG(T) { static bool at_ = false; if (!at_) { (void)hipFuncSetAttribute((const void*)k_pw_bwd<T, T, false, -1, -1, true>, hipFuncAttributeMaxDynamicSharedMemorySize, 160 * 1024); at_ = true; } \
        hipLaunchKernelGGL((k_pw_bwd<T, T, false, -1, -1, true>), dim3((unsigned)gx), dim3(PWB), lds, st, (const bf16*)x, (const bf16*)dy, w, (const bf16*)res, (bf16*)dx, (bf16*)dx_plain, dw, dbias, M, bn); }
        if (NT == 2) BLG(2) else BLG(3)
#undef BLG
        TCCT_LAUNCH_OK();
    }
    if (split && KT == 2) { BLX(1, 2, true, -1, -1) TCCT_LAUNCH_OK(); }
#define BL(NTV, KTV) BLX(NTV, KTV, false, -1, -1)
#define BLS(NTV) BLX(NTV, 4, true, -1, -1)
#define BLK(NTV) switch (KT) { case 1: BL(NTV, 1) break; case 2: BL(NTV, 2) break; case 3: BL(NTV, 3) break; default: if (split) BLS(NTV) else BL(NTV, 4) break; }
    switch (NT) { case 1: BLK(1) break; case 2: BLK(2) break; case 3: BLK(3) break; default: BLK(4) break; }
#undef BLK
#undef BLS
#undef BL
#undef BLX
    TCCT_LAUNCH_OK();
}

template <int NT, int KT, bool STATS, bool SPLIT, bool RES = false, bool GX = false, int XAP = -1, bool AFF = false>
__global__ void __launch_bounds__(PWB, 2)
k_pw_fwd2(const bf16* __restrict__ x, const bf16* __restrict__ x2, const float* __restrict__ w, const float* __restrict__ bias,
          bf16* __restrict__ y, int64_t M, double* __restrict__ stats, int stat_pre, PwRes pr) {
    constexpr int K = 32 * KT, N = 32 * NT;
    constexpr int SX = 2 * K + 16, SW = 2 * K + 16;
    constexpr int XS = K / 16;
    extern __shared__ __attribute__((aligned(16))) unsigned char smem[];
    unsigned char* sX = smem;
    unsigned char* sW = sX + PB_P * SX;
    float* sB = reinterpret_cast<float*>(sW + N * SW);
    unsigned char* sS = reinterpret_cast<unsigned char*>(sB + N);
    const int tid = threadIdx.x, lane = tid & 63, wave = tid >> 6;
    const int r = lane & 31, hh = lane >> 5;
    for (int i = tid; i < N * (K / 8); i += PWB) {
        const int n = i / (K / 8), c8 = i - n * (K / 8);
        const float4 a = *reinterpret_cast<const float4*>(w + (int64_t)n * K + c8 * 8);
        const float4 b = *reinterpret_cast<const float4*>(w + (int64_t)n * K + c8 * 8 + 4);
        uint4 o;
        o.x = pack_bf16x2(a.x, a.y); o.y = pack_bf16x2(a.z, a.w); o.z = pack_bf16x2(b.x, b.y); o.w = pack_bf16x2(b.z, b.w);
        *reinterpret_cast<uint4*>(sW + n * SW + c8 * 16) = o;
    }
    if (tid < N) sB[tid] = bias ? bias[tid] : 0.f;
    float* sXA = reinterpret_cast<float*>(sS + 4 * 2560);
    if (XAP >= 0) for (int i = tid; i < 2 * K; i += PWB) sXA[i] = pr.xab[i];
    float* sAF = sXA + (XAP >= 0 ? 2 * K : 0);
    if (AFF) for (int i = tid; i < 2 * N; i += PWB) sAF[i] = pr.aff ? pr.aff[i] : (i < N ? 1.f : 0.f);
    float ss[STATS ? NT : 1][8], sq[STATS ? NT : 1][8];
#pragma unroll
    for (int a = 0; a < (STATS ? NT : 1); ++a)
#pragma unroll
        for (int k = 0; k < 8; ++k) ss[a][k] = sq[a][k] = 0.f;
    const int64_t tiles = (M + PB_P - 1) / PB_P;
    constexpr int KS = SPLIT ? K / 2 : K;
    const uint32_t xbytes = (uint32_t)(M * KS * 2), ybytes = (uint32_t)(M * N * 2);
    const __amdgpu_buffer_rsrc_t rx = __builtin_amdgcn_make_buffer_rsrc((void*)x, 0, xbytes, 0x00020000);
    const __amdgpu_buffer_rsrc_t rx2 = __builtin_amdgcn_make_buffer_rsrc((void*)(SPLIT ? x2 : x), 0, xbytes, 0x00020000);
    const __amdgpu_buffer_rsrc_t ro = __builtin_amdgcn_make_buffer_rsrc((void*)y, 0, ybytes, 0x00020000);
    const __amdgpu_buffer_rsrc_t rres = __builtin_amdgcn_make_buffer_rsrc((void*)(RES ? (const void*)pr.res : (const void*)y), 0, ybytes, 0x00020000);
    const __amdgpu_buffer_rsrc_t rpl = __builtin_amdgcn_make_buffer_rsrc((void*)((RES && pr.yplain) ? pr.yplain : y), 0, ybytes, 0x00020000);
    u32x4 px[XS];
    auto prefetch = [&](int64_t tile) {
        const uint32_t bx = (uint32_t)(tile * PB_P * KS * 2);
#pragma unroll
        for (int j = 0; j < XS; ++j) {
            if (SPLIT && j >= XS / 2) px[j] = __builtin_amdgcn_raw_buffer_load_b128(rx2, bx + (uint32_t)(tid + (j - XS / 2) * PWB) * 16u, 0, 0);
            else px[j] = __builtin_amdgcn_raw_buffer_load_b128(rx, bx + (uint32_t)(tid + j * PWB) * 16u, 0, 0);
        }
    };
    auto stage = [&]() {
#pragma unroll
        for (int j = 0; j < XS; ++j) {
            const int jj = (SPLIT && j >= XS / 2) ? j - XS / 2 : j;
            const int q = tid + jj * PWB, p = q / (KS / 8), c = q - p * (KS / 8);
            u32x4 xv_ = GX ? gelu8(px[j]) : px[j];
            if (XAP >= 0) xv_ = affine8<XAP < 0 ? 0 : XAP>(xv_, sXA + c * 8, sXA + K + c * 8);
            *reinterpret_cast<u32x4*>(sX + p * SX + ((SPLIT && j >= XS / 2) ? KS * 2 : 0) + c * 16) = xv_;
        }
    };
    const unsigned char* bB = sX + (32 * wave + r) * SX + hh * 16;
    int64_t tile = blockIdx.x;
    if (tile < tiles) {
        prefetch(tile);
        __syncthreads();
        stage();
        prefetch(tile + gridDim.x);
    }
    __syncthreads();
    for (; tile < tiles; tile += gridDim.x) {
        f32x16 acc[NT];
#pragma unroll
        for (int nt = 0; nt < NT; ++nt)
#pragma unroll
            for (int k = 0; k < 16; ++k) acc[nt][k] = 0.f;
#pragma unroll
        for (int st = 0; st < 2 * KT; ++st) {
            const bf16x8 fb = *reinterpret_cast<const bf16x8*>(bB + st * 32);
#pragma unroll
            for (int nt = 0; nt < NT; ++nt) {
                const bf16x8 fa = *reinterpret_cast<const bf16x8*>(sW + (nt * 32 + r) * SW + st * 32 + hh * 16);
                acc[nt] = __builtin_amdgcn_mfma_f32_32x32x16_bf16(fa, fb, acc[nt], 0, 0, 0);
            }
        }
        __syncthreads();
        if (GX || XAP >= 0) {
            const bool do_stage = tile + (int64_t)gridDim.x < tiles;
            const uint32_t bx = (uint32_t)((tile + 2 * (int64_t)gridDim.x) * PB_P * KS * 2);
#pragma unroll
            for (int j = 0; j < XS; ++j) {
                u32x4 xv_ = px[j];
                px[j] = __builtin_amdgcn_raw_buffer_load_b128(rx, bx + (uint32_t)(tid + j * PWB) * 16u, 0, 0);
                if (do_stage) {
                    const int q = tid + j * PWB, p = q / (KS / 8), c = q - p * (KS / 8);
                    if (GX) xv_ = gelu8(xv_);
                    if (XAP >= 0) xv_ = affine8<XAP < 0 ? 0 : XAP>(xv_, sXA + c * 8, sXA + K + c * 8);
                    *reinterpret_cast<u32x4*>(sX + p * SX + c * 16) = xv_;
                }
            }
        } else {
            if (tile + (int64_t)gridDim.x < tiles) stage();
            prefetch(tile + 2 * (int64_t)gridDim.x);
        }
        unsigned char* sc = sS + wave * 2560;
        const int64_t m0 = tile * PB_P + 32 * wave;
#pragma unroll
        for (int nt = 0; nt < NT; ++nt) {
#pragma unroll
            for (int q = 0; q < 4; ++q) {
                const float4 bq = *reinterpret_cast<const float4*>(sB + nt * 32 + 8 * q + 4 * hh);
                float v0 = acc[nt][4 * q] + bq.x, v1 = acc[nt][4 * q + 1] + bq.y, v2 = acc[nt][4 * q + 2] + bq.z, v3 = acc[nt][4 * q + 3] + bq.w;
                if (AFF) {
                    const float4 aq = *reinterpret_cast<const float4*>(sAF + nt * 32 + 8 * q + 4 * hh);
                    const float4 cq = *reinterpret_cast<const float4*>(sAF + N + nt * 32 + 8 * q + 4 * hh);
                    float v4[4] = {v0, v1, v2, v3};
                    const float a4[4] = {aq.x, aq.y, aq.z, aq.w}, c4[4] = {cq.x, cq.y, cq.z, cq.w};
                    affine4(v4, a4, c4, TCCT_ACT_NONE, pr.aff_post);
                    v0 = v4[0]; v1 = v4[1]; v2 = v4[2]; v3 = v4[3];
                }
                uint2 o;
                o.x = pack_bf16x2(v0, v1);
                o.y = pack_bf16x2(v2, v3);
                *reinterpret_cast<uint2*>(sc + r * 80 + (8 * q + 4 * hh) * 2) = o;
            }
            wave_lds_fence();
#pragma unroll
            for (int h2 = 0; h2 < 2; ++h2) {
                const int p = (lane >> 2) + 16 * h2, cch = lane & 3;
                u32x4 o = *reinterpret_cast<const u32x4*>(sc + p * 80 + cch * 16);
                const int64_t mm = m0 + p;
                const bool inb = mm < M;
                const uint32_t off = inb ? (uint32_t)((mm * N + nt * 32 + cch * 8) * 2) : 0x80000000u;
                if (RES) {
                    if (pr.yplain) __builtin_amdgcn_raw_buffer_store_b128(o, rpl, off, 0, 0);
                    const u32x4 rv = __builtin_amdgcn_raw_buffer_load_b128(rres, off, 0, 0);
                    const float sc_ = pr.rscale ? pr.rscale[(inb ? mm : 0) / pr.per_sample] : 1.f;
#pragma unroll
                    for (int k = 0; k < 4; ++k)
                        o[k] = pack_bf16x2(__uint_as_float(rv[k] << 16) + sc_ * __uint_as_float(o[k] << 16),
                                           __uint_as_float(rv[k] & 0xffff0000u) + sc_ * __uint_as_float(o[k] & 0xffff0000u));
                }
                __builtin_amdgcn_raw_buffer_store_b128(o, ro, off, 0, 0);
                if (STATS) {
                    if (inb) {
#pragma unroll
                        for (int k = 0; k < 4; ++k) {
                            float u0 = __uint_as_float(o[k] << 16), u1 = __uint_as_float(o[k] & 0xffff0000u);
                            if (stat_pre != TCCT_ACT_NONE) { u0 = act_fwd(stat_pre, u0); u1 = act_fwd(stat_pre, u1); }
                            ss[nt][2 * k] += u0; sq[nt][2 * k] += u0 * u0; ss[nt][2 * k + 1] += u1; sq[nt][2 * k + 1] += u1 * u1;
                        }
                    }
                }
            }
            wave_lds_fence();
        }
        __syncthreads();
    }
    if (STATS) {
        __syncthreads();
        float* red = reinterpret_cast<float*>(smem);
#pragma unroll
        for (int nt = 0; nt < NT; ++nt)
#pragma unroll
            for (int k = 0; k < 8; ++k) {
                float a = ss[nt][k], b = sq[nt][k];
#pragma unroll
                for (int o = 32; o > 2; o >>= 1) { a += __shfl_xor(a, o, 64); b += __shfl_xor(b, o, 64); }
                if (lane < 4) {
                    red[wave * 2 * N + nt * 32 + 8 * lane + k] = a;
                    red[wave * 2 * N + N + nt * 32 + 8 * lane + k] = b;
                }
            }
        __syncthreads();
        for (int i2 = tid; i2 < N; i2 += PWB) {
            double a = 0.0, b = 0.0;
#pragma unroll
            for (int wv = 0; wv < 4; ++wv) { a += (double)red[wv * 2 * N + i2]; b += (double)red[wv * 2 * N + N + i2]; }
            atomicAdd(&stats[i2], a); atomicAdd(&stats[N + i2], b);
        }
    }
}

static bool pw_fwd2_ok(int64_t M, int K, int N, int K1, bool has_x2) {
    if (K % 32 || N % 32 || K < 64 || K > 128 || N < 32 || N > 128) return false;
    if (M * (int64_t)(K > N ? K : N) * 2 >= (1LL << 31)) return false;
    if (has_x2 && !(K == 128 && K1 == 64)) return false;
    return true;
}
static int pw_fwd2_launch(const void* x, const void* x2, const float* w, const float* bias, void* y, int64_t M, int K, int N, double* stats,
                          int stat_pre, tcct_stream_t stream, PwRes pr, bool gelu_x) {
    const int NT = N / 32, KT = K / 32;
    const size_t lds = (size_t)PB_P * (2 * K + 16) + (size_t)N * (2 * K + 16) + (size_t)N * 4 + 4 * 2560 + (pr.xab ? (size_t)2 * K * 4 : 0) + (pr.has_aff ? (size_t)2 * N * 4 : 0);
    const int64_t tiles = (M + PB_P - 1) / PB_P;
    int per_cu = (int)((160 * 1024) / (lds + 256));
    if (per_cu > 2) per_cu = 2;
    int64_t gx = 256 * per_cu;
    if (gx > tiles) gx = tiles;
    hipStream_t st = (hipStream_t)stream;
#define F2(NTV, KTV, SV, PV) { static bool at_ = false; if (!at_) { (void)hipFuncSetAttribute((const void*)k_pw_fwd2<NTV, KTV, SV, PV>, hipFuncAttributeMaxDynamicSharedMemorySize, 160 * 1024); at_ = true; } \
        hipLaunchKernelGGL((k_pw_fwd2<NTV, KTV, SV, PV>), dim3((unsigned)gx), dim3(PWB), lds, st, (const bf16*)x, (const bf16*)x2, w, bias, (bf16*)y, M, stats, stat_pre, pr); }
#define F2R(NTV, KTV) { static bool at_ = false; if (!at_) { (void)hipFuncSetAttribute((const void*)k_pw_fwd2<NTV, KTV, false, false, true>, hipFuncAttributeMaxDynamicSharedMemorySize, 160 * 1024); at_ = true; } \
        hipLaunchKernelGGL((k_pw_fwd2<NTV, KTV, false, false, true>), dim3((unsigned)gx), dim3(PWB), lds, st, (const bf16*)x, (const bf16*)x2, w, bias, (bf16*)y, M, stats, stat_pre, pr); }
#define F2K(NTV, SV) switch (KT) { case 2: F2(NTV, 2, SV, false) break; case 3: F2(NTV, 3, SV, false) break; default: if (x2) F2(NTV, 4, SV, true) else F2(NTV, 4, SV, false) break; }
#define F2RK(NTV) switch (KT) { case 2: F2R(NTV, 2) break; case 3: F2R(NTV, 3) break; default: F2R(NTV, 4) break; }
#define F2N(SV) switch (NT) { case 1: F2K(1, SV) break; case 2: F2K(2, SV) break; case 3: F2K(3, SV) break; default: F2K(4, SV) break; }
#define F2G(T) { static bool at_ = false; if (!at_) { (void)hipFuncSetAttribute((const void*)k_pw_fwd2<T, T, false, false, true, true>, hipFuncAttributeMaxDynamicSharedMemorySize, 160 * 1024); at_ = true; } \
        hipLaunchKernelGGL((k_pw_fwd2<T, T, false, false, true, true>), dim3((unsigned)gx), dim3(PWB), lds, st, (const bf16*)x, (const bf16*)x2, w, bias, (bf16*)y, M, stats, stat_pre, pr); }
#define F2A(T) { static bool at_ = false; if (!at_) { (void)hipFuncSetAttribute((const void*)k_pw_fwd2<T, T, true, false, false, false, 2>, hipFuncAttributeMaxDynamicSharedMemorySize, 160 * 1024); at_ = true; } \
        hipLaunchKernelGGL((k_pw_fwd2<T, T, true, false, false, false, 2>), dim3((unsigned)gx), dim3(PWB), lds, st, (const bf16*)x, (const bf16*)x2, w, bias, (bf16*)y, M, stats, stat_pre, pr); }
#define F2F(NTV, KTV, SPV, RSV) { static bool at_ = false; if (!at_) { (void)hipFuncSetAttribute((const void*)k_pw_fwd2<NTV, KTV, false, SPV, RSV, false, -1, true>, hipFuncAttributeMaxDynamicSharedMemorySize, 160 * 1024); at_ = true; } \
        hipLaunchKernelGGL((k_pw_fwd2<NTV, KTV, false, SPV, RSV, false, -1, true>), dim3((unsigned)gx), dim3(PWB), lds, st, (const bf16*)x, (const bf16*)x2, w, bias, (bf16*)y, M, stats, stat_pre, pr); }
#define F2X(T) { static bool at_ = false; if (!at_) { (void)hipFuncSetAttribute((const void*)k_pw_fwd2<T, T, false, false, true, false, 2, true>, hipFuncAttributeMaxDynamicSharedMemorySize, 160 * 1024); at_ = true; } \
        hipLaunchKernelGGL((k_pw_fwd2<T, T, false, false, true, false, 2, true>), dim3((unsigned)gx), dim3(PWB), lds, st, (const bf16*)x, (const bf16*)x2, w, bias, (bf16*)y, M, stats, stat_pre, pr); }
    if (pr.has_aff && pr.xab) {
        if (NT == 2) F2X(2) else if (NT == 3) F2X(3) else F2X(4)
    }
    else
    if (pr.has_aff) {
        if (x2) F2F(3, 4, true, false)
        else if (pr.res) { if (NT == 2) F2F(2, 2, false, true) else if (NT == 3) F2F(3, 3, false, true) else F2F(4, 4, false, true) }
        else { if (NT == 2) F2F(2, 2, false, false) else if (NT == 3) F2F(3, 3, false, false) else F2F(4, 4, false, false) }
    }
    else
    if (pr.xab) { if (NT == 2) F2A(2) else F2A(3) }
    else
    if (gelu_x) { if (NT == 2) F2G(2) else F2G(3) }
    else
    if (pr.res) { switch (NT) { case 1: F2RK(1) break; case 2: F2RK(2) break; case 3: F2RK(3) break; default: F2RK(4) break; } }
    else if (stats) { F2N(true) } else { F2N(false) }
#undef F2X
#undef F2F
#undef F2G
#undef F2A
#undef F2RK
#undef F2R
#undef F2N
#undef F2K
#undef F2
    TCCT_LAUNCH_OK();
}

static int pw_fwd2_route(const void* x, const void* x2, const float* w, const float* bias, void* y, int64_t M, int K, int N, double* stats,
                         int stat_pre, tcct_stream_t stream, const bf16* res, const float* rscale, int64_t per_sample, bf16* yplain) {
    return pw_fwd2_launch(x, x2, w, bias, y, M, K, N, stats, stat_pre, stream, PwRes{res, rscale, per_sample, yplain});
}
extern "C" int tcct_pw_fwd_bnstats_xaff(const void* y_prev, const float* ab_prev, const float* w, const float* bias, void* y, int64_t M, int K, int N,
                                        double* stats, tcct_stream_t stream) {
    TCCT_CHECK(K == N && (K == 64 || K == 96) && ab_prev && stats, "pw_fwd_bnstats_xaff: K=%d N=%d unsupported (64 or 96 square) or NULL argument", K, N);
    TCCT_CHECK(M > 0 && M * (int64_t)K * 2 < (1LL << 31), "pw_fwd_bnstats_xaff: tensor exceeds the 2 GiB buffer-descriptor range");
    return pw_fwd2_launch(y_prev, nullptr, w, bias, y, M, K, N, stats, 0, stream, PwRes{nullptr, nullptr, 1, nullptr, ab_prev});
}
extern "C" int tcct_pw_fwd_gelu_residual(const void* x1, const float* w, const float* bias, const void* res, const float* scale, int64_t per_sample,
                                         void* y, int64_t M, int K, int N, tcct_stream_t stream) {
    TCCT_CHECK(K == N && (K == 64 || K == 96), "pw_fwd_gelu_residual: K=%d N=%d unsupported (64 or 96 square, as tcct_pw_bwd_gelu)", K, N);
    TCCT_CHECK(res != nullptr && per_sample >= 1 && M > 0 && M * (int64_t)K * 2 < (1LL << 31), "pw_fwd_gelu_residual: needs res, per_sample >= 1, < 2 GiB tensors");
    return pw_fwd2_launch(x1, nullptr, w, bias, y, M, K, N, nullptr, 0, stream, PwRes{(const bf16*)res, scale, per_sample, nullptr}, true);
}

template <typename T>
__global__ void k_im2col3x3_c3(const T* __restrict__ x4, T* __restrict__ out, int N, int H, int W, int stride, int Ho, int Wo) {
    const int64_t total = (int64_t)N * Ho * Wo * 8;
    for (int64_t i = (int64_t)blockIdx.x * blockDim.x + threadIdx.x; i < total; i += (int64_t)gridDim.x * blockDim.x) {
        const int sub = (int)(i & 7);
        int64_t p = i >> 3;
        const int wo = (int)(p % Wo);
        int64_t q = p / Wo;
        const int ho = (int)(q % Ho);
        const int64_t n = q / Ho;
        f4 o;
#pragma unroll
        for (int j = 0; j < 4; ++j) {
            const int k = sub * 4 + j;
            float v = 0.f;
            if (k < 27) {
                const int tap = k / 3, ch = k - tap * 3;
                const int hi = ho * stride + tap / 3 - 1, wi = wo * stride + tap % 3 - 1;
                if (hi >= 0 && hi < H && wi >= 0 && wi < W) v = ldf(x4 + ((n * H + hi) * (int64_t)W + wi) * 4 + ch);
            }
            o.v[j] = v;
        }
        st4(out + p * 32 + sub * 4, o);
    }
}
extern "C" int tcct_im2col3x3_c3(const void* x4, void* out, int N, int H, int W, int stride, int dtype, tcct_stream_t stream) {
    TCCT_CHECK(stride == 1 || stride == 2, "im2col3x3_c3: stride %d", stride);
    int Ho = (H - 1) / stride + 1, Wo = (W - 1) / stride + 1;
    int64_t total = (int64_t)N * Ho * Wo * 8;
    TCCT_DISPATCH(dtype, hipLaunchKernelGGL(k_im2col3x3_c3<T>, dim3(tcct_grid(total, PWB, 1 << 16)), dim3(PWB), 0, (hipStream_t)stream, (const T*)x4, (T*)out, N, H, W, stride, Ho, Wo));
    TCCT_LAUNCH_OK();
}

template <typename Tx, typename Td>
__global__ void k_pw_wgrad_smalln(const Tx* __restrict__ x, const Td* __restrict__ dy, float* __restrict__ dw, float* __restrict__ dbias,
                                  int64_t M, int K, int N) {
    extern __shared__ float smf[];
    const int KV = K >> 2, R = PWB / KV;
    const int t = threadIdx.x, kv = t % KV, r = t / KV;
    float acc[8][4], bs[8];
#pragma unroll
    for (int n = 0; n < 8; ++n) { bs[n] = 0.f; acc[n][0] = acc[n][1] = acc[n][2] = acc[n][3] = 0.f; }
    if (r < R) {
        const int64_t step = (int64_t)gridDim.x * R;
        for (int64_t m0 = (int64_t)blockIdx.x * R + r; m0 < M; m0 += 2 * step) {
            f4 xv[2];
            float d[2][8];
#pragma unroll
            for (int u = 0; u < 2; ++u) {
                const int64_t m = m0 + u * step;
                const bool ok = m < M;
                xv[u] = ok ? ld4(x + m * K + kv * 4) : f4zero();
#pragma unroll
                for (int n = 0; n < 8; ++n) d[u][n] = (ok && n < N) ? ldf(dy + m * N + n) : 0.f;
            }
#pragma unroll
            for (int u = 0; u < 2; ++u)
#pragma unroll
                for (int n = 0; n < 8; ++n) {
                    bs[n] += d[u][n];
#pragma unroll
                    for (int j = 0; j < 4; ++j) acc[n][j] += d[u][n] * xv[u].v[j];
                }
        }
    }
    for (int i = t; i < R * N * K; i += PWB) smf[i] = 0.f;
    __syncthreads();
    if (r < R) {
#pragma unroll
        for (int n = 0; n < 8; ++n)
            if (n < N) {
#pragma unroll
                for (int j = 0; j < 4; ++j) smf[(r * N + n) * K + kv * 4 + j] = acc[n][j];
            }
    }
    __syncthreads();
    for (int i = t; i < N * K; i += PWB) {
        float a = 0.f;
        for (int rr = 0; rr < R; ++rr) a += smf[rr * N * K + i];
        atomicAdd(&dw[i], a);
    }
    if (dbias && kv == 0 && r < R) {
#pragma unroll
        for (int n = 0; n < 8; ++n)
            if (n < N) atomicAdd(&dbias[n], bs[n]);
    }
}
__global__ void __launch_bounds__(PWB, 2)
k_pw_wgrad_smalln_mfma(const bf16* __restrict__ x, const float* __restrict__ dy, float* __restrict__ dw, float* __restrict__ dbias,
                       int64_t M, int N) {
    __shared__ __attribute__((aligned(16))) unsigned char smem[2 * PW_P * 64];
    unsigned char* sX = smem;
    unsigned char* sD = smem + PW_P * 64;
    const int tid = threadIdx.x, lane = tid & 63, wave = tid >> 6;
    const int r = lane & 31, hh = lane >> 5;
    for (int i = tid; i < PW_P * 4; i += PWB) *reinterpret_cast<uint4*>(sD + i * 16) = make_uint4(0, 0, 0, 0);
    f32x16 acc;
#pragma unroll
    for (int k = 0; k < 16; ++k) acc[k] = 0.f;
    float bsum = 0.f;
    uint4 px[2];
    float pdv[8];
    const int dp = tid;
    auto prefetch = [&](int64_t tile) {
        const int64_t m0 = tile * PW_P;
#pragma unroll
        for (int j = 0; j < 2; ++j) {
            const int i = tid + j * PWB, p = i >> 2, c = i & 3;
            px[j] = make_uint4(0, 0, 0, 0);
            if (m0 + p < M) px[j] = *reinterpret_cast<const uint4*>(x + (m0 + p) * 32 + c * 8);
        }
#pragma unroll
        for (int n = 0; n < 8; ++n) pdv[n] = (dp < PW_P && n < N && m0 + dp < M) ? dy[(m0 + dp) * N + n] : 0.f;
    };
    const int li = lane & 15, lq = li >> 2, lpp = li & 3, lg = lane >> 4;
    const int loff = (8 * (lg >> 1) + lq) * 64 + (16 * (lg & 1) + 4 * lpp) * 2;
    auto tr2 = [&](const unsigned char* p) {
        s16x4 lo = __builtin_amdgcn_ds_read_tr16_b64_v4i16((__attribute__((address_space(3))) s16x4*)p);
        s16x4 hi = __builtin_amdgcn_ds_read_tr16_b64_v4i16((__attribute__((address_space(3))) s16x4*)(p + 256));
        s16x8 v = __builtin_shufflevector(lo, hi, 0, 1, 2, 3, 4, 5, 6, 7);
        return __builtin_bit_cast(bf16x8, v);
    };
    const int64_t tiles = (M + PW_P - 1) / PW_P;
    int64_t tile = blockIdx.x;
    if (tile < tiles) prefetch(tile);
    for (; tile < tiles; tile += gridDim.x) {
        __syncthreads();
#pragma unroll
        for (int j = 0; j < 2; ++j) { const int i = tid + j * PWB; *reinterpret_cast<uint4*>(sX + (i >> 2) * 64 + (i & 3) * 16) = px[j]; }
        if (dp < PW_P) {
            uint4 o;
            o.x = pack_bf16x2(pdv[0], pdv[1]); o.y = pack_bf16x2(pdv[2], pdv[3]); o.z = pack_bf16x2(pdv[4], pdv[5]); o.w = pack_bf16x2(pdv[6], pdv[7]);
            *reinterpret_cast<uint4*>(sD + dp * 64) = o;
        }
        __syncthreads();
        if (tile + gridDim.x < tiles) prefetch(tile + gridDim.x);
#pragma unroll
        for (int c2 = 0; c2 < 2; ++c2) {
            const int ch = wave + 4 * c2;
            const bf16x8 a = tr2(sD + loff + ch * 1024);
            const bf16x8 b = tr2(sX + loff + ch * 1024);
#pragma unroll
            for (int j = 0; j < 8; ++j) bsum += (float)a[j];
// ... 46 lines not shown
```

tcct_amd/nets/tcct.py:

```python
import math

import torch
from torch import nn

from .. import ops
from .._lib import TcctError

KSIZES = (13, 11, 9, 7, 5)


def _conv(m, x, out_dtype=None, stats_pre=None):
    return ops.conv2d(x, m.weight, m.bias, stride=m.stride[0], pad=tuple(m.padding), out_dtype=out_dtype, stats_pre=stats_pre)


def _dw(m, x, add_input=False, bn_stats=False, deferred=None):
    return ops.dwconv3x3(x, m.weight, m.bias, stride=m.stride[0], add_input=add_input, bn_stats=bn_stats, deferred=deferred)


def _bn(m, x, pre=None, post=None, residual=None):
    return ops.batchnorm(x, m.weight, m.bias, m.running_mean, m.running_var, m.num_batches_tracked, eps=m.eps,
                         momentum=m.momentum, pre_act=pre, post_act=post, training=m.training, residual=residual)


def _bn_args(m):
# ... 11 lines not shown
    y = ops.conv_bn_act(x, mc.weight, mc.bias, mc.stride[0], tuple(mc.padding), bn, pre, post)
    return y if residual is None else ops.add(y, residual)


def _nchw_view(y):
    return y.permute(0, 3, 1, 2)


class CrossCNNBlock(nn.Module):

    def __init__(self, in_c, out_c, ksize):
        super().__init__()
        ksize = self._ksize(ksize)
        self.block12 = nn.Sequential(nn.Conv2d(in_c, out_c, 3, padding=1), nn.Conv2d(out_c, out_c, 3, padding=1),
                                     nn.LeakyReLU(), nn.BatchNorm2d(out_c))
        self.block34 = nn.Sequential(nn.Conv2d(in_c, out_c, (1, ksize), padding=(0, ksize // 2)),
                                     nn.Conv2d(out_c, out_c, (ksize, 1), padding=(ksize // 2, 0)),
                                     nn.Conv2d(out_c, out_c, 3, padding=1), nn.LeakyReLU(), nn.BatchNorm2d(out_c))
        self.block5 = nn.Sequential(nn.Conv2d(out_c, out_c, 3, padding=1), nn.LeakyReLU(), nn.BatchNorm2d(out_c))

    @staticmethod
    def _ksize(ksize):
        return ksize

    def forward(self, x, pool=False):
        tr = self.training
        m0 = self.block12[0]
        m1c = self.block12[1]
        if ops.conv3x3_chain_ok(x, m0.weight, m0.bias, m1c.weight, m1c.bias, m0.stride[0], m0.padding, m1c.stride[0], m1c.padding):
            a, x2 = ops.conv3x3_chain(x, m0.weight, m0.bias, m1c.weight, m1c.bias, stats_pre='lrelu' if tr else None, fork=True)
        elif not tr and ops.conv3x3_chain_infer_ok(x, m0.weight, m1c.weight, m0.stride[0], m0.padding, m1c.stride[0], m1c.padding):
            a, x2 = ops.conv3x3_chain_infer(x, m0.weight, m0.bias, m1c.weight, m1c.bias), x
        else:
            a0, x2 = ops.conv2d_fork(x, m0.weight, m0.bias, m0.stride[0], tuple(m0.padding))
            a = _conv(m1c, a0, stats_pre='lrelu' if tr else None)
        b = _conv(self.block34[2], _conv(self.block34[1], _conv(self.block34[0], x2)), stats_pre='lrelu' if tr else None)
        if tr:
            m1, m2 = self.block12[3], self.block34[4]
            c = ops.bn2_add_act(a, (m1.weight, m1.bias, m1.running_mean, m1.running_var, m1.num_batches_tracked, m1.eps, m1.momentum),
                                b, (m2.weight, m2.bias, m2.running_mean, m2.running_var, m2.num_batches_tracked, m2.eps, m2.momentum))
        else:
            if torch.is_grad_enabled() or not ops.INFER_FUSE:
                c = ops.add_act(_bn(self.block12[3], a, pre='lrelu'), _bn(self.block34[4], b, pre='lrelu'), 'gelu')
            else:
                m1, m2 = self.block12[3], self.block34[4]
                c = ops.bn2_add_act_eval(a, (m1.weight, m1.bias, m1.running_mean, m1.running_var, m1.eps),
                                         b, (m2.weight, m2.bias, m2.running_mean, m2.running_var, m2.eps))
        if not pool:
            return _conv_bn(self.block5[0], self.block5[2], c, pre='lrelu')
        mc, mb = self.block5[0], self.block5[2]
        if mb.training:
            y = _conv(mc, c, stats_pre='lrelu')
            if ops.bn_pool_ok(y, True):
                return ops.batchnorm_maxpool2_fork(y, mb.weight, mb.bias, mb.running_mean, mb.running_var, mb.num_batches_tracked, eps=mb.eps,
                                                   momentum=mb.momentum, pre_act='lrelu')
            return ops.maxpool2_fork(_bn(mb, y, pre='lrelu'))
        return ops.maxpool2_fork(_conv_bn(mc, mb, c, pre='lrelu'))


class PlainCNNBlock(CrossCNNBlock):

    @staticmethod
    def _ksize(ksize):
        return 3


class CrossResNet(nn.Module):
    __name__ = 'crnet'

    def __init__(self, in_ch=3, out_ch=6, flag_tiny=False, Block=CrossCNNBlock):
        super().__init__()
        layers = (32, 32, 32, 32, 32) if flag_tiny else (32, 64, 96, 128, 256)
        self.layer_dims = layers
        self.pool = nn.MaxPool2d(kernel_size=2)
        self.path_estan = nn.ModuleList([Block(layers[0], layers[0], KSIZES[0])])
        for i in range(len(layers) - 1):
            self.path_estan.append(Block(layers[i], layers[i + 1], KSIZES[i + 1]))
        self.cnn = nn.Sequential(nn.Conv2d(3, layers[0], 3, 1, 1), nn.BatchNorm2d(layers[0]))

    def forward(self, x, levels=None):
        xs = []
        for _ in self.iter_levels(x, xs, levels):
            pass
        return xs

    def iter_levels(self, x, xs, levels=None):
        m = self.cnn[1]
        if ops.conv3x3_c3_bn_ok(x, self.cnn[0].weight, m.training, None):
            x = ops.conv3x3_c3_bn(x, self.cnn[0].weight, self.cnn[0].bias, _bn_args(m), 1)
        elif self.training or torch.is_grad_enabled() or not ops.INFER_FUSE:
            x = _bn(m, ops.conv3x3_c3(x, self.cnn[0].weight, self.cnn[0].bias, 1, stats_pre='none' if self.training else None))
        else:
            x = ops.conv3x3_c3(x, self.cnn[0].weight, self.cnn[0].bias, 1, infer_bn=(m.weight, m.bias, m.running_mean, m.running_var, m.eps))
        n = len(self.path_estan) if levels is None else int(levels)
        for i, enc in enumerate(self.path_estan[:n]):
            if i + 1 < n:
                x, skip = enc(x, pool=True)
                xs.append(skip)
                if i == 0:
                    x = ops.grad_mark(x, 'deep')
            else:
                x = enc(x)
                xs.append(x)
            yield i


class Conv2d_BN(nn.Module):

    def __init__(self, in_ch, out_ch, kernel_size=1, stride=1, pad=0, act=False):
        super().__init__()
        self.conv = nn.Conv2d(in_ch, out_ch, kernel_size, stride, pad, bias=False)
        self.bn = nn.BatchNorm2d(out_ch)
        fan_out = kernel_size * kernel_size * out_ch
        self.conv.weight.data.normal_(0.0, math.sqrt(2.0 / fan_out))
        self.act = act

    def forward(self, x, residual=None, x_final=False):
        sp = 'none' if self.training else None
        if self.conv.in_channels == 3:
            if ops.conv3x3_c3_bn_ok(x, self.conv.weight, self.bn.training, 'hswish' if self.act else None):
                return ops.conv3x3_c3_bn(x, self.conv.weight, None, _bn_args(self.bn), self.conv.stride[0], 'hswish' if self.act else None)
            if self.training or torch.is_grad_enabled() or not ops.INFER_FUSE:
                y = ops.conv3x3_c3(x, self.conv.weight, None, self.conv.stride[0], stats_pre=sp)
                return _bn(self.bn, y, post='hswish' if self.act else None)
            m = self.bn
            return ops.conv3x3_c3(x, self.conv.weight, None, self.conv.stride[0], post_act='hswish' if self.act else None,
                                  infer_bn=(m.weight, m.bias, m.running_mean, m.running_var, m.eps))
        return _conv_bn(self.conv, self.bn, x, post='hswish' if self.act else None, residual=residual, x_final=x_final)

    def forward_deferred(self, x):
        if not (ops.BN_DEFER_DW and self.act and self.bn.training and self.conv.in_channels != 3):
            return None
        y = _conv(self.conv, x, stats_pre='none')
        m = self.bn
        if not ops.batchnorm_deferred_ok(y, True, 'hswish'):
            return _bn(m, y, post='hswish'), None
        return ops.batchnorm_deferred(y, m.weight, m.bias, m.running_mean, m.running_var, m.num_batches_tracked, m.eps, m.momentum, 'hswish')


class DWConv2d_BN(nn.Module):

    def __init__(self, in_ch, out_ch, kernel_size=3, stride=1):
        super().__init__()
        self.dwconv = nn.Conv2d(in_ch, out_ch, kernel_size, stride, (kernel_size - 1) // 2, groups=out_ch, bias=False)
        self.pwconv = nn.Conv2d(out_ch, out_ch, 1, 1, 0, bias=False)
        self.bn = nn.BatchNorm2d(out_ch)
        for m in (self.dwconv, self.pwconv):
            n = m.kernel_size[0] * m.kernel_size[1] * m.out_channels
            m.weight.data.normal_(0, math.sqrt(2.0 / n))

    def forward(self, x, fork=False, deferred=None):
        if fork:
            m = self.dwconv
            d, alias = ops.dwconv3x3_fork(x, m.weight, m.bias, stride=m.stride[0])
            return _conv_bn(self.pwconv, self.bn, d, post='hswish'), alias
        return _conv_bn(self.pwconv, self.bn, _dw(self.dwconv, x, deferred=deferred), post='hswish')


class DWCPatchEmbed(nn.Module):

    def __init__(self, embed_dim, stride):
        super().__init__()
        self.patch_conv = DWConv2d_BN(embed_dim, embed_dim, 3, stride)

    def forward(self, x, fork=False, deferred=None):
        return self.patch_conv(x, fork, deferred)


class Patch_Embed_stage(nn.Module):

    def __init__(self, embed_dim, isPool=False):
        super().__init__()
        self.patch_embeds = nn.ModuleList([DWCPatchEmbed(embed_dim, 2 if isPool else 1)])

    def forward(self, x, fork=False, deferred=None):
        return self.patch_embeds[0](x, fork, deferred)


class ConvPosEnc(nn.Module):

    def __init__(self, dim, k=3):
        super().__init__()
        self.proj = nn.Conv2d(dim, dim, k, 1, k // 2, groups=dim)


class ConvRelPosEnc(nn.Module):

    def __init__(self, Ch, h, window):
        super().__init__()
        if isinstance(window, int):
            window = {window: h}
        elif not isinstance(window, dict):
            raise ValueError()
        self.conv_list = nn.ModuleList()
        self.head_splits = []
        for k, split in window.items():
            self.conv_list.append(nn.Conv2d(split * Ch, split * Ch, (k, k), padding=(k // 2, k // 2), groups=split * Ch))
            self.head_splits.append(split)
        self.channel_splits = [x * Ch for x in self.head_splits]


class FactorAtt_ConvRelPosEnc(nn.Module):

    def __init__(self, dim, num_heads=8, qkv_bias=False, qk_scale=None, shared_crpe=None):
        super().__init__()
        self.num_heads = num_heads
        self.scale = qk_scale or (dim // num_heads) ** -0.5
        self.qkv = nn.Linear(dim, dim * 3, bias=qkv_bias)
        self.proj = nn.Linear(dim, dim)
        self.crpe = shared_crpe

    def mix(self, x, size):
        if sum(self.crpe.channel_splits) != x.shape[-1]:
            raise ValueError(f'crpe head splits {self.crpe.head_splits} do not cover {self.num_heads} heads')
        qkv = ops.conv2d(x, self.qkv.weight, self.qkv.bias)
        return ops.factor_att(qkv, size, self.num_heads, self.scale, self.crpe.conv_list)

    def forward(self, x, size):
        return ops.conv2d(self.mix(x, size), self.proj.weight, self.proj.bias)


class Mlp(nn.Module):

    def __init__(self, dim, hidden):
        super().__init__()
        self.fc1 = nn.Linear(dim, hidden)
        self.fc2 = nn.Linear(hidden, dim)


class MHCABlock(nn.Module):

    def __init__(self, dim, mlp_ratio, drop_path, shared_cpe, shared_crpe, att='pool', num_heads=8):
        super().__init__()
        self.cpe = shared_cpe
        self.crpe = shared_crpe
        if att == 'factor':
            self.att = FactorAtt_ConvRelPosEnc(dim, num_heads=num_heads, qkv_bias=True, shared_crpe=shared_crpe)
        elif att != 'pool':
            raise ValueError(f"att must be 'pool' (MetaPool, tcct.py:449) or 'factor', got {att!r}")
        self.mlp = Mlp(dim, dim * mlp_ratio)
        self.drop_prob = float(drop_path)
        self.norm1 = nn.LayerNorm(dim, eps=1e-6)
        self.norm2 = nn.LayerNorm(dim, eps=1e-6)

    def forward(self, x, scales, fork=False):
        B, H, W, C = x.shape
        m = self.cpe.proj
        if fork:
            x, x_alias = ops.dwconv3x3_fork(x, m.weight, m.bias, stride=m.stride[0], add_input=True)
        else:
            x = _dw(m, x, add_input=True)
        t = x.view(B, H * W, C)
        s1, s2 = scales if scales is not None else (None, None)
        att = getattr(self, 'att', None)
        cur2 = None
        if att is None and ops.ln_metapool_residual_ok(t, self.norm1.weight, self.norm1.bias):
            if ops.LN_POOL_LN2:
                t, cur2, mr2 = ops.ln_metapool_residual_ln(t, self.norm1.weight, self.norm1.bias, self.norm1.eps, s1, self.norm2.weight, self.norm2.bias,
                                                           self.norm2.eps)
                m_ = self.mlp
                if ops.mlp_tail_ok(t, cur2, m_.fc1.weight, m_.fc1.bias, m_.fc2.weight, m_.fc2.bias):
                    t = ops.mlp_tail(t, cur2, mr2, self.norm2.weight, self.norm2.bias, m_.fc1.weight, m_.fc1.bias, m_.fc2.weight, m_.fc2.bias, s2)
                    return (t.view(B, H, W, C), x_alias) if fork else t.view(B, H, W, C)
            else:
                t = ops.ln_metapool_residual(t, self.norm1.weight, self.norm1.bias, self.norm1.eps, s1)
        else:
            cur, t = ops.layernorm_fork(t, self.norm1.weight, self.norm1.bias, self.norm1.eps)
            if att is not None:
                t = ops.linear_residual(att.mix(cur, (H, W)), att.proj.weight, att.proj.bias, t, s1)
            else:
                t = ops.metapool_residual(cur, t, s1)
        if cur2 is None:
            cur, t = ops.layernorm_fork(t, self.norm2.weight, self.norm2.bias, self.norm2.eps)
        else:
            cur = cur2
        if self.training or torch.is_grad_enabled() or not ops.INFER_FUSE:
            y1 = ops.conv2d(cur, self.mlp.fc1.weight, self.mlp.fc1.bias)
            if ops.gelu_linear_residual_ok(y1, self.mlp.fc2.weight, self.mlp.fc2.bias, t):
                t = ops.gelu_linear_residual(y1, self.mlp.fc2.weight, self.mlp.fc2.bias, t, s2)
                return (t.view(B, H, W, C), x_alias) if fork else t.view(B, H, W, C)
            h = ops.act(y1, 'gelu')
        else:
            h = ops.conv_bn_act(cur, self.mlp.fc1.weight, self.mlp.fc1.bias, post_act='gelu')
        t = ops.linear_residual(h, self.mlp.fc2.weight, self.mlp.fc2.bias, t, s2)
        return (t.view(B, H, W, C), x_alias) if fork else t.view(B, H, W, C)


class MHCAEncoder(nn.Module):

    def __init__(self, dim, num_heads, mlp_ratio, drop_path, att='pool'):
        super().__init__()
        self.cpe = ConvPosEnc(dim, k=3)
        self.crpe = ConvRelPosEnc(Ch=dim // num_heads, h=num_heads, window={3: 2, 5: 3, 7: 3})
        self.MHCA_layers = nn.ModuleList([MHCABlock(dim, mlp_ratio, drop_path, self.cpe, self.crpe, att=att, num_heads=num_heads)])

    def forward(self, x, scales, fork=False):
        return self.MHCA_layers[0](x, scales, fork)


class ResBlock(nn.Module):

    def __init__(self, dim):
        super().__init__()
        self.conv1 = Conv2d_BN(dim, dim, act=True)
        self.dwconv = nn.Conv2d(dim, dim, 3, 1, 1, bias=False, groups=dim)
        self.norm = nn.BatchNorm2d(dim)
        self.conv2 = Conv2d_BN(dim, dim)
        for m in (self.conv1.conv, self.dwconv, self.conv2.conv):
            fan_out = m.kernel_size[0] * m.kernel_size[1] * m.out_channels // m.groups
            m.weight.data.normal_(0, math.sqrt(2.0 / fan_out))

    def forward(self, x):
        return self.tail(self.conv1(x), x)

    def tail(self, f, x, flink=None):
        y = _dw(self.dwconv, f, bn_stats=self.norm.training, deferred=flink)
        c2, m = self.conv2, self.norm
        if (ops.batchnorm_deferred_ok(y, m.training, 'hswish') and c2.bn.training and not c2.act
                and ops.pw_conv_bn_ok(y, c2.conv.weight, None, True, None, None)):
            ya, link = ops.batchnorm_deferred(y, m.weight, m.bias, m.running_mean, m.running_var, m.num_batches_tracked, m.eps, m.momentum, 'hswish')
            return ops.pw_conv_bn(ya, c2.conv.weight, None, _bn_args(c2.bn), None, residual=x, deferred=link)
        if not m.training and not c2.bn.training and not c2.act and ops.invres_tail_eval_ok(y, c2.conv.weight, c2.conv.bias, x):
            mb = c2.bn
            return ops.invres_tail_eval(y, (m.weight, m.bias, m.running_mean, m.running_var, m.eps), c2.conv.weight, c2.conv.bias,
                                        (mb.weight, mb.bias, mb.running_mean, mb.running_var, mb.eps), x)
        f = _bn(self.norm, y, post='hswish')
        return self.conv2(f, residual=x, x_final=True)


class MHCA_stage(nn.Module):

    def __init__(self, embed_dim, out_embed_dim, num_heads, mlp_ratio, drop_path, att='pool'):
        super().__init__()
        self.mhca_blks = nn.ModuleList([MHCAEncoder(embed_dim, num_heads, mlp_ratio, drop_path, att=att)])
        self.InvRes = ResBlock(embed_dim)
        self.aggregate = Conv2d_BN(embed_dim * 2, out_embed_dim, act=True)

    def forward(self, x, scales):
        if torch.is_grad_enabled() and x.requires_grad:
            c1 = self.InvRes.conv1
            flink = None
            if ops.pw_conv_bn_ok(x, c1.conv.weight, None, c1.bn.training, None, 'hswish'):
                if ops.BN_DEFER_DW and x.shape[-1] % 4 == 0 and x.shape[-1] <= 256:
                    (f, x1), flink = ops.pw_conv_bn(x, c1.conv.weight, None, _bn_args(c1.bn), 'hswish', fork=True, x_final=True, defer_apply=True)
                else:
                    f, x1 = ops.pw_conv_bn(x, c1.conv.weight, None, _bn_args(c1.bn), 'hswish', fork=True, x_final=True)
            else:
                f, x1 = ops.conv2d_fork(x, c1.conv.weight, None, 1, 0, stats_pre='none' if c1.bn.training else None)
                f = _bn(c1.bn, f, post='hswish')
            if ops.PARALLEL_BRANCHES and x.shape[0] * x.shape[1] * x.shape[2] <= ops.STAGE_FORK_MAX_PIXELS and torch.cuda.is_available():
                x2h = []

                def enc():
                    e_, x2_ = self.mhca_blks[0](x1, scales, fork=True)
                    x2h.append(x2_)
                    return e_
                r, e = ops.run_parallel('vit_enc', lambda: self.InvRes.tail(f, x2h[0], flink), enc)
            else:
                e, x2 = self.mhca_blks[0](x1, scales, fork=True)
                r = self.InvRes.tail(f, x2, flink)
        elif (not torch.is_grad_enabled() and ops.PARALLEL_BRANCHES and x.is_cuda and x.shape[0] * x.shape[1] * x.shape[2] <= ops.STAGE_FORK_MAX_PIXELS
              and x.shape[0] * x.shape[1] * x.shape[2] >= ops.FUSION_FORK_MIN_PIXELS and not torch.cuda.is_current_stream_capturing()):
            r, e = ops.run_parallel('vit_enc', lambda: self.InvRes(x), lambda: self.mhca_blks[0](x, scales))
        else:
            r = self.InvRes(x)
            e = self.mhca_blks[0](x, scales)
        ag = self.aggregate
        if ag.bn.training or torch.is_grad_enabled() or not ops.INFER_FUSE:
            if ops.pw_conv_bn_ok(r, ag.conv.weight, None, ag.bn.training, None, 'hswish', x2=e):
                return ops.pw_conv_bn(r, ag.conv.weight, None, _bn_args(ag.bn), 'hswish', x2=e, x_final=True)
            y = ops.conv1x1_cat2(r, e, ag.conv.weight, stats_pre='none' if ag.bn.training else None)
            return _bn(ag.bn, y, post='hswish')
        if ops.conv1x1_cat2_bn_act_eval_ok(r, e, ag.conv.weight, 'hswish'):
            m = ag.bn
            return ops.conv1x1_cat2_bn_act_eval(r, e, ag.conv.weight, (m.weight, m.bias, m.running_mean, m.running_var, m.eps), 'hswish')
        return ag(ops.concat2(r, e))


class Cls_head(nn.Module):

    def __init__(self, embed_dim, num_classes):
        super().__init__()
        self.cls = nn.Linear(embed_dim, num_classes)


class MPViT(nn.Module):
    __name__ = 'mpvit'

    def __init__(self, embed_dims=(64, 96, 128, 160), mlp_ratios=(1, 1, 1, 1), num_heads=(4, 4, 4, 4),
                 drop_path_rate=0.1, num_classes=1000, att='pool'):
        super().__init__()
        if att == 'factor':
            num_heads = (8, 8, 8, 8)
        self.att = att
        self.num_stages = 4
        self.embed_dims = list(embed_dims)
        dpr = [x.item() for x in torch.linspace(0, drop_path_rate, 4)]
        self.drop_probs = dpr
        self.stem = nn.Sequential(Conv2d_BN(3, embed_dims[0] // 2, 3, 2, 1, act=True),
                                  Conv2d_BN(embed_dims[0] // 2, embed_dims[0], 3, 1, 1, act=True))
        self.patch_embed_stages = nn.ModuleList([Patch_Embed_stage(embed_dims[i], isPool=i > 0) for i in range(4)])
        self.mhca_stages = nn.ModuleList([
            MHCA_stage(embed_dims[i], embed_dims[i + 1] if i + 1 < 4 else embed_dims[i], num_heads[i], mlp_ratios[i],
                       dpr[i], att=att) for i in range(4)])
        self.cls_head = Cls_head(embed_dims[-1], num_classes)
        for m in self.modules():
            if isinstance(m, nn.Linear):
                nn.init.trunc_normal_(m.weight, std=0.02)
                nn.init.constant_(m.bias, 0)
            elif isinstance(m, nn.LayerNorm):
                nn.init.constant_(m.bias, 0)
                nn.init.constant_(m.weight, 1.0)
        self.forced_dp_masks = None

    def _dp_scales(self, B, device):
        out = []
        forced = list(self.forced_dp_masks) if self.forced_dp_masks is not None else None
        if forced is None and self.training and any(p > 0.0 for p in self.drop_probs):
            act = [s for s in range(4) if self.drop_probs[s] > 0.0]
            key = (device, B, tuple(self.drop_probs))
            if getattr(self, '_dp_keep', (None,))[0] != key:
                keep = torch.tensor([1.0 - self.drop_probs[s] for s in act for _ in range(2)], device=device, dtype=torch.float32).view(-1, 1)
                self._dp_keep = (key, keep)
            keep = self._dp_keep[1]
            m = (torch.rand((2 * len(act), B), device=device) < keep).to(torch.float32) / keep
            it = iter(range(len(act)))
            return [((m[2 * i], m[2 * i + 1]) if self.drop_probs[s] > 0.0 else None) for s in range(4) for i in ([next(it)] if self.drop_probs[s] > 0.0 else [None])]
        for s in range(4):
            p = self.drop_probs[s]
            if p == 0.0 or not self.training:
                out.append(None)
                continue
            pair = []
            for _ in range(2):
                if forced is not None:
                    m = forced.pop(0).to(device=device, dtype=torch.float32)
                else:
                    m = torch.empty(B, device=device, dtype=torch.float32).bernoulli_(1 - p)
                pair.append((m / (1 - p)).contiguous())
            out.append(tuple(pair))
        return out

    def forward_features(self, x):
        xs = []
        for _ in self.iter_stages(x, xs):
            pass
        return xs

    def iter_stages(self, x, xs):
        scales = self._dp_scales(x.shape[0], x.device)
        x = self.stem[0](x)
        d0 = self.stem[1].forward_deferred(x)
        x, link0 = d0 if d0 is not None else (self.stem[1](x), None)
        for i in range(4):
            if i == 1:
                x = ops.grad_mark(x, 'deep')
            if i > 0 and torch.is_grad_enabled() and x.requires_grad:
                p, xs[-1] = self.patch_embed_stages[i](x, fork=True)
            else:
                p = self.patch_embed_stages[i](x, deferred=link0 if i == 0 else None)
            x = self.mhca_stages[i](p, scales[i])
            xs.append(x)
            yield i


def mpvit_tiny(**kw):
    return MPViT(**kw)


class MPUpBlock(nn.Module):

    def __init__(self, in_ch, out_ch):
        super().__init__()
        self.prep = nn.Sequential(nn.Conv2d(in_ch, out_ch, 3, 1, 1), nn.BatchNorm2d(out_ch), nn.LeakyReLU(inplace=True))
        self.post = nn.Sequential(nn.Conv2d(out_ch, out_ch, 1, 1, 0))

    def forward(self, x1, x2, with_sum=False, want_plain=True):
        y = _conv_bn(self.prep[0], self.prep[1], x1, post='lrelu')
        if with_sum:
            return ops.up_skip_conv(y, x2, self.post[0].weight, self.post[0].bias, True, want_plain=want_plain)
        u = ops.bilinear(y, (x1.shape[1] * 2, x1.shape[2] * 2), True, residual=x2)
        return _conv(self.post[0], u)

    def forward_through(self, x1, x2, t32, aux=None):
        p, t = self.post[0], t32
        probe = torch.empty((x1.shape[0], x1.shape[1], x1.shape[2], self.prep[0].out_channels), dtype=x1.dtype, device='meta')
        if not ((self.prep[1].training or (ops.INFER_FUSE and not torch.is_grad_enabled())) and ops.up_skip_conv_t32_ok(probe, x2, p.weight, p.bias, t.weight, t.bias)):
            return None
        y = _conv_bn(self.prep[0], self.prep[1], x1, post='lrelu')
        if aux is not None and ops.up_skip_conv_t32_aux_ok(probe, x2, p.weight, p.bias, t.weight, t.bias, aux.weight, aux.bias):
            if ops.TAIL_AUX_LOW:
                return ops.up_skip_conv_t32_aux_low(y, x2, p.weight, p.bias, t.weight, t.bias, aux.weight, aux.bias, True), ('y', y.detach())
            lg, v = ops.up_skip_conv_t32_aux(y, x2, p.weight, p.bias, t.weight, t.bias, aux.weight, aux.bias, True)
            return lg, ('v', v)
        return ops.up_skip_conv_t32(y, x2, p.weight, p.bias, t.weight, t.bias, True)


class FTC(nn.Module):
    __name__ = 'gtc'

    def __init__(self, base_cnn, base_vit, out_channels=5, filters=32, compute_dtype=torch.float32, legacy_heads=False,
                 flag_gate=False, flag_cnn=True, flag_vit=True):
        super().__init__()
        self.legacy_heads = bool(legacy_heads)
        self.flag_gate, self.flag_cnn, self.flag_vit = bool(flag_gate), bool(flag_cnn), bool(flag_vit)
        self.defer_aux_resize = False
        self.forced_gate_fields = None
        if not (self.flag_cnn or self.flag_vit):
            raise TcctError('FTC needs at least one of flag_cnn / flag_vit')
        self.base_vit = base_vit
        self.base_cnn = base_cnn
        ed, ld = base_vit.embed_dims, base_cnn.layer_dims
        for j, cin in enumerate((ed[1], ed[2], ed[3], ed[3])):
            setattr(self, f'tran_vit{j}', nn.Sequential(nn.Conv2d(cin, ld[j + 1], 1, 1, 0), nn.BatchNorm2d(ld[j + 1])))
        for j in range(4):
            setattr(self, f'tran_cnn{j}', nn.Sequential(nn.Conv2d(ld[j + 1], ld[j + 1], 1, 1, 0), nn.BatchNorm2d(ld[j + 1])))
        self.head = nn.Sequential(nn.Conv2d(ld[-1], ld[-1], 3, 1, 1), nn.BatchNorm2d(ld[-1]), nn.LeakyReLU())
        self.fuse = nn.Conv2d(ld[4], filters, kernel_size=1)
        self.dec1 = MPUpBlock(ld[-1], ld[-2])
        self.dec2 = MPUpBlock(ld[-2], ld[-3])
        self.dec3 = MPUpBlock(ld[-3], ld[-4])
        self.dec4 = MPUpBlock(ld[-4], filters)
        if not self.legacy_heads:
            self.t321 = nn.Conv2d(ld[-2], filters, 1)
            self.t322 = nn.Conv2d(ld[-3], filters, 1)
            self.t323 = nn.Conv2d(ld[-4], filters, 1)
            self.t324 = nn.Conv2d(filters, filters, 1)
        self.aux0 = nn.Conv2d(filters, out_channels, 1)
        self.aux1 = nn.Conv2d(filters, out_channels, 1)
        self.aux2 = nn.Conv2d(filters, out_channels, 1)
        self.aux4 = nn.Conv2d(filters, out_channels, 1)
        self.compute_dtype = compute_dtype
        self._feats_src = None
        self._feats = None
        self.eager_feats = False
        self.compose_heads = False
        self.main_head_only = False

    @property
    def feats(self):
        if self._feats is None and self._feats_src is not None:
            if self.legacy_heads:
                raise TcctError('the legacy-head layout (onnx/tcct_goals.py) is supported for inference and Dice/boundary training; its '
                                'six-tensor `feats` (tcct_goals.py:1021) is not built')
            g0, g1, g2, size = self._feats_src
            g0, g1, g2 = [g() if callable(g) else g for g in (g0, g1, g2)]
            self._feats = [_nchw_view(ops.norm_add3(g0, g1, g2))]
            self._feats_src = None
        return self._feats

    @feats.setter
    def feats(self, v):
        self._feats = v
        self._feats_src = None

    def set_compute_dtype(self, dt):
        if dt not in (torch.float32, torch.bfloat16):
            raise TcctError('compute dtype must be float32 or bfloat16')
        self.compute_dtype = dt
        return self

    def _to_nhwc4(self, x):
        if x.dim() != 4 or x.shape[1] not in (1, 3):
            raise TcctError(f'expected image batch [B,3,H,W] (or [B,1,H,W]), got {tuple(x.shape)}')
        if not x.is_cuda:
            raise TcctError('tcct_amd model needs a CUDA(HIP) input; there is no CPU fallback')
        B, Cs, H, W = x.shape
        if H % 16 or W % 16:
            raise TcctError(f'H and W must be multiples of 16 (got {H}x{W}); pad first (see tcct_amd.data.synth)')
        x = x.contiguous().float()
        out = torch.empty((B, H, W, 4), device=x.device, dtype=self.compute_dtype)
        ops.lib.image_to_nhwc4(x, out, B, Cs, H, W, W, ops.dtype_code(self.compute_dtype))
        return out

    def forward(self, x):
        size = (x.shape[2], x.shape[3])
        x = self._to_nhwc4(x)
        mho = self.main_head_only and not torch.is_grad_enabled() and not self.training
        if self.flag_vit and self.flag_cnn:
            cs, vs = [], []
            ops.run_interleaved('vit', self.base_cnn.iter_levels(x, cs), self.base_vit.iter_stages(x, vs), vs)
            (c1, c2, c3, c4, c5), (v2, v3, v4, v5) = [ops.grad_mark(t, 'dec') for t in cs], [ops.grad_mark(t, 'dec') for t in vs]
            def fuse_level(j, v, c):
                tv, tc = getattr(self, f'tran_vit{j}'), getattr(self, f'tran_cnn{j}')
                if self.flag_gate and self.training:
                    a1, a2 = _conv_bn(tv[0], tv[1], v), _conv_bn(tc[0], tc[1], c)
                    B_, Hh, Ww, Cc = a1.shape
                    fields = self.forced_gate_fields
                    field = fields.pop(0) if fields else torch.rand((B_, max(3, Hh // 32), max(3, Ww // 32), Cc), device=a1.device)
                    return ops.gate_fusion(a1, a2, field.to(device=a1.device, dtype=torch.float32).contiguous())
                if self.flag_gate:
                    sm = _conv_bn(tc[0], tc[1], c, residual=_conv_bn(tv[0], tv[1], v))
                    half = torch.empty_like(sm)
                    ops.lib.scale(sm, half, sm.numel(), 0.5, ops.dtype_code(sm.dtype))
                    return half
                if (ops.TRAN_FUSE and c.shape[-1] % 8 == 0 and ops.pw_conv_bn_ok(v, tv[0].weight, tv[0].bias, tv[1].training, None, None)
                        and ops.pw_conv_bn_ok(c, tc[0].weight, tc[0].bias, tc[1].training, None, None)):
                    yv, lv = ops.pw_conv_bn(v, tv[0].weight, tv[0].bias, _bn_args(tv[1]), None, defer_apply=True)
                    yc, lc = ops.pw_conv_bn(c, tc[0].weight, tc[0].bias, _bn_args(tc[1]), None, defer_apply=True)
                    return ops.affine2_add(yv, lv, yc, lc)
                return _conv_bn(tc[0], tc[1], c, residual=_conv_bn(tv[0], tv[1], v))
            pairs = ((v2, c2), (v3, c3), (v4, c4), (v5, c5))
            y8 = None
            if ops.fusion_fork_ok(c5) and not self.flag_gate and self.training:
                def high():
                    f3_, f4_ = fuse_level(2, *pairs[2]), fuse_level(3, *pairs[3])
                    return f3_, f4_, _conv_bn(self.head[0], self.head[1], f4_, post='lrelu')
                (f3, f4, y8), (f1, f2) = ops.run_parallel(ops.FUSE_STREAM_TAG, high, lambda: (fuse_level(0, *pairs[0]), fuse_level(1, *pairs[1])))
                f = [c1, f1, f2, f3, f4]
            else:
                f = [c1] + [fuse_level(j, v, c) for j, (v, c) in enumerate(pairs)]
        elif self.flag_cnn:
            f = list(self.base_cnn(x))
        else:
            cs, vs = [], []
            ops.run_interleaved('vit', self.base_cnn.iter_levels(x, cs, 1), self.base_vit.iter_stages(x, vs), vs)
            (c1,), (v2, v3, v4, v5) = cs, vs
            f = [c1] + [_conv_bn(getattr(self, f'tran_vit{j}')[0], getattr(self, f'tran_vit{j}')[1], v) for j, v in enumerate((v2, v3, v4, v5))]
        if not (self.flag_vit and self.flag_cnn) or y8 is None:
            y8 = _conv_bn(self.head[0], self.head[1], f[4], post='lrelu')
        y0_direct = None
        if self.legacy_heads:
            d3 = self.dec1(y8, f[3])
            d2 = self.dec2(d3, f[2])
            d1 = self.dec3(d2, f[1])
            d0 = self.dec4(d1, f[0])
            g0, g1, g2, g3 = d0, d1, d2, d3
            lg_direct = [None, None, None]
        else:
            d3, s3 = self.dec1(y8, f[3], with_sum=True)
            d2, s2 = self.dec2(d3, f[2], with_sum=True)
            d1, s1 = self.dec3(d2, f[1], with_sum=True)
            compose = (self.compose_heads and not self.eager_feats) or mho
            g0 = self.dec4.forward_through(d1, f[0], self.t324, aux=self.aux0 if compose else None)
            if isinstance(g0, tuple):
                y0_direct, (kind, src) = g0
                skip0, pw, tw = f[0], self.dec4.post[0], self.t324
                rebuild = ops.up_skip_conv_t32_from_v if kind == 'v' else ops.up_skip_conv_t32_from_y
                g0 = lambda: rebuild(src, skip0, pw.weight, pw.bias, tw.weight, tw.bias)
            if g0 is None:
                d0, s0 = self.dec4(d1, f[0], with_sum=True, want_plain=False)
                g0 = _conv(self.t324, s0)
            mids, lg_direct = [], []
            for t, aux, s_ in ((self.t323, self.aux1, s1), (self.t322, self.aux2, s2), (self.t321, self.aux4, s3)):
                if mho:
                    lg_direct.append(None)
                    mids.append(lambda t=t, s_=s_: self._rebuild(t, s_))
                elif self.training and compose and ops.head_through_t32_ok(s_, t.weight, t.bias, aux.weight, aux.bias):
                    lg_direct.append(ops.head_through_t32(s_, t.weight, t.bias, aux.weight, aux.bias))
                    mids.append(lambda t=t, s_=s_: self._rebuild(t, s_))
                else:
                    lg_direct.append(None)
                    mids.append(_conv(t, s_))
            g1, g2, g3 = mids
        self._feats_src = (g0, g1, g2, size)
        self._feats = None
        if self.eager_feats and not self.legacy_heads and not mho:
            forked = ops.norm_add3_fork(g0, g1, g2)
            if forked is not None:
                feats, g0, g1, g2 = forked
                self._feats, self._feats_src = [_nchw_view(feats)], None
        f32 = torch.float32
        y0 = y0_direct if y0_direct is not None else _conv(self.aux0, g0() if callable(g0) else g0, out_dtype=f32)
        if mho:
            return [_nchw_view(y0)]
        low = [lg if lg is not None else _conv(m, g, out_dtype=f32) for m, g, lg in zip((self.aux1, self.aux2, self.aux4), (g1, g2, g3), lg_direct)]
        if self.defer_aux_resize and torch.is_grad_enabled():
            return [_nchw_view(y0)] + [ops.LowResLogits(l_, size) for l_ in low]
        return [_nchw_view(y0)] + [_nchw_view(ops.bilinear(l_, size, False)) for l_ in low]

    @staticmethod
    def _rebuild(t, s_):
        with torch.no_grad():
            return _conv(t, s_)


def stc_tt(n_class=8, **args):
    model = FTC(base_vit=mpvit_tiny(att=args.get('att', 'pool')), base_cnn=CrossResNet(flag_tiny=True), out_channels=n_class,
                compute_dtype=args.get('compute_dtype', torch.float32), legacy_heads=args.get('legacy_heads', False))
    model.__name__ = 'stctt'
    return model


tcct = stc_tt


def _variant(name, n_class, args, flag_tiny=True, Block=CrossCNNBlock, **flags):
    model = FTC(base_vit=mpvit_tiny(), base_cnn=CrossResNet(flag_tiny=flag_tiny, Block=Block), out_channels=n_class,
                compute_dtype=args.get('compute_dtype', torch.float32), **flags)
    model.__name__ = name
    return model


def stc_tb(n_class=8, **args):
    return _variant('stctb', n_class, args, flag_tiny=False)


def gtc_tb(n_class=8, **args):
    return _variant('gtctb', n_class, args, flag_tiny=False, flag_gate=True)


def pnnu(n_class=8, **args):
    return _variant('pnnu', n_class, args, Block=PlainCNNBlock, flag_vit=False, flag_cnn=True)


def gtc_tt(n_class=8, **args):
    return _variant('gtctt', n_class, args, flag_gate=True)


def cnnu(n_class=8, **args):
    return _variant('cnnu', n_class, args, flag_vit=False, flag_cnn=True)


def vitu(n_class=8, **args):
    return _variant('vitu', n_class, args, flag_vit=True, flag_cnn=False)
```

tcct_amd/ops.py:

```python
import os
import weakref

import torch

from ._lib import lib, dtype_code, TcctError, launch_on, F32, BF16

ACT = {None: 0, 'none': 0, 'lrelu': 1, 'hswish': 2, 'gelu': 3, 'sigmoid': 4, 'abs': 5}


class _ZeroPool:

    def __init__(self):
        self.buf = None
        self.off = 0
        self.active = False
        self.frozen = False

    def begin(self, device, nbytes=8 << 20):
        if self.buf is None or self.buf.device != device or self.buf.numel() < nbytes:
            if self.frozen:
                raise TcctError('the zero pool cannot be re-allocated after a training step was captured into a hipGraph '
                                f'(pool on {self.buf.device}, step on {device})')
            self.buf = torch.empty(nbytes, device=device, dtype=torch.uint8)
        self.buf.zero_()
# ... 1410 lines not shown
        y._bn_sums = (box[1], box[0])
    return y


def im2col3x3_c3(x4, stride=1):
    _chk(x4)
    N, H, W, C = x4.shape
    if C != 4:
        raise TcctError('im2col3x3_c3 expects the 4-channel NHWC image')
    Ho, Wo = (H - 1) // stride + 1, (W - 1) // stride + 1
    out = torch.empty((N, Ho, Wo, 32), device=x4.device, dtype=x4.dtype)
    lib.im2col3x3_c3(x4.detach(), out, N, H, W, stride, dtype_code(x4.dtype))
    return out


C3_DIRECT = True


class _ConvC3(_FastFunction):

    @staticmethod
    def forward(ctx, x4, w, bias, stride, stats_box):
        _chk(x4, w, bias)
        B, H, W, _ = x4.shape
        Ho, Wo = (H - 1) // stride + 1, (W - 1) // stride + 1
        y = torch.empty((B, Ho, Wo, 32), device=x4.device, dtype=torch.bfloat16)
        sums = None
        if stats_box is not None:
            sums = ZERO.get((64,), torch.float64, x4.device) if ZERO.active else torch.zeros(64, device=x4.device, dtype=torch.float64)
            stats_box[1] = sums
        lib.c3_fwd(x4, w, bias, y, B, H, W, stride, sums, stats_box[0] if stats_box is not None else 0, None, 0, 0)
        ctx.save_for_backward(x4)
        ctx.cfg = (stride, w, bias)
        return y

    @staticmethod
    def backward(ctx, dy):
        x4, = ctx.saved_tensors
        stride, w, bias = ctx.cfg
        dy = _c(dy)
        B, H, W, _ = x4.shape
        with _wgrad_stream(_slot_written(w, bias), x4, dy):
            dw = _grad_out(w, tuple(w.shape))
            db = _grad_out(bias) if bias is not None else None
            lib.c3_wgrad(x4, dy, dw, db, B, H, W, stride)
        return None, _ret(dw, w), _ret(db, bias), None, None


def _c3_direct_ok(x4, w):
    B, H, W, C = x4.shape
    return (C3_DIRECT and x4.dtype == torch.bfloat16 and C == 4 and tuple(w.shape) == (32, 3, 3, 3) and w.dtype == torch.float32
            and w.is_contiguous() and B * H * W * 64 < 2 ** 31)


def conv3x3_c3(x4, w, bias, stride=1, stats_pre=None, infer_bn=None, post_act=None):
    if _c3_direct_ok(x4, w):
        _chk(x4)
        if infer_bn is not None:
            if torch.is_grad_enabled() and w.requires_grad:
                raise TcctError('conv3x3_c3(infer_bn=...) is inference-only (call it under torch.no_grad())')
            B, H, W, _ = x4.shape
            ab = torch.empty(64, device=x4.device, dtype=torch.float32)
            lib.bn_eval_ab(32, infer_bn[0], infer_bn[1], float(infer_bn[4]), infer_bn[2], infer_bn[3], torch.empty(64, device=x4.device, dtype=torch.float32), ab)
            y = torch.empty((B, (H - 1) // stride + 1, (W - 1) // stride + 1, 32), device=x4.device, dtype=torch.bfloat16)
            if C3_BN_FUSE and ACT[post_act] in (0, ACT['hswish']):
                lib.c3_bn_fwd_eval(x4, w, bias, y, B, H, W, stride, ab, ACT[post_act])
            else:
                lib.c3_fwd(x4, w, bias, y, B, H, W, stride, None, 0, ab, 0, ACT[post_act])
            return y
        box = [ACT[stats_pre], None] if stats_pre is not None else None
        y = _ConvC3.apply(x4, w, bias, stride, box)
        if box is not None and box[1] is not None:
            y._bn_sums = (box[1], box[0])
        return y
    w2 = torch.nn.functional.pad(w.permute(0, 2, 3, 1).reshape(w.shape[0], 27), (0, 5)).contiguous()
    if infer_bn is not None:
        return conv_bn_act(im2col3x3_c3(x4, stride), w2.view(w.shape[0], 32, 1, 1), bias, bn=infer_bn, post_act=post_act)
    return conv2d(im2col3x3_c3(x4, stride), w2.view(w.shape[0], 32, 1, 1), bias, stats_pre=stats_pre)


C3_BN_FUSE = True


class _ConvC3BN(_FastFunction):

    @staticmethod
    def forward(ctx, x4, w, bias, gamma, beta, rm, rv, nbt, eps, momentum, stride, post):
        _chk(x4, w, bias, gamma, beta)
        B, H, W, _ = x4.shape
        Ho, Wo = (H - 1) // stride + 1, (W - 1) // stride + 1
        z = torch.empty((B, Ho, Wo, 32), device=x4.device, dtype=torch.bfloat16)
        sums = ZERO.get((64,), torch.float64, x4.device) if ZERO.active else torch.zeros(64, device=x4.device, dtype=torch.float64)
        mean_rstd = torch.empty(64, device=x4.device, dtype=torch.float32)
        ab = torch.empty(64, device=x4.device, dtype=torch.float32)
        lib.c3_bn_fwd_train(x4, w, bias, z, B, H, W, stride, sums, gamma, beta, eps, momentum, rm, rv, nbt, mean_rstd, ab, post)
        ctx.save_for_backward(x4, mean_rstd, ab)
        ctx.cfg = (stride, post, w, bias, gamma, beta)
        return z

    @staticmethod
    def backward(ctx, dz):
        x4, mean_rstd, ab = ctx.saved_tensors
        stride, post, w, bias, gamma, beta = ctx.cfg
        dz = _as(dz, torch.bfloat16)
        B, H, W, _ = x4.shape
        M = dz.numel() // 32
        dev = x4.device
        raw = ZERO.get((64,), torch.float64, dev) if ZERO.active else torch.zeros(64, device=dev, dtype=torch.float64)
        coef = torch.empty(160, device=dev, dtype=torch.float32)
        with _wgrad_stream(_slot_written(w, bias, gamma, beta), x4, dz, coef, mean_rstd, ab):
            dg = _grad_out(gamma) if ZERO.active and getattr(gamma, '_grad_slot', None) is not None else torch.empty(32, device=dev, dtype=torch.float32)
            db_ = _grad_out(beta) if ZERO.active and getattr(beta, '_grad_slot', None) is not None else torch.empty(32, device=dev, dtype=torch.float32)
            dw = _grad_out(w, tuple(w.shape))
            dbias = _grad_out(bias) if bias is not None else None
            if C3_ONEPASS:
                if C3_BWD_FORM != _C3_FORM_SET[0]:
                    lib.c3_bn_bwd_prefetch(C3_BWD_FORM)
                    _C3_FORM_SET[0] = C3_BWD_FORM
                work = ZERO.get((4160,), torch.float32, dev) if ZERO.active else torch.zeros(4160, device=dev, dtype=torch.float32)
                s96 = ZERO.get((96,), torch.float64, dev) if ZERO.active else torch.zeros(96, device=dev, dtype=torch.float64)
                lib.c3_bn_bwd_onepass(x4, w, bias, dz, B, H, W, stride, mean_rstd, ab, work, s96, dw, dbias, dg, db_, post)
            else:
                lib.c3_bn_bwd_reduce(x4, w, bias, dz, B, H, W, stride, ab, raw, post)
                lib.bn_bwd_coef(raw, 1, M, 32, mean_rstd, ab, coef, dg, db_)
                lib.c3_bn_bwd_wgrad(x4, w, bias, dz, B, H, W, stride, coef, dw, dbias, post)
        return None, _ret(dw, w), _ret(dbias, bias), _ret(dg, gamma), _ret(db_, beta), None, None, None, None, None, None, None


C3_BWD_FORM = 4
_C3_FORM_SET = [4]
C3_ONEPASS = True


def conv3x3_c3_bn_ok(x4, w, bn_training, post_act):
    return (C3_BN_FUSE and bn_training and _c3_direct_ok(x4, w) and ACT[post_act] in (0, ACT['hswish']))


def conv3x3_c3_bn(x4, w, bias, bn, stride=1, post_act=None):
    gamma, beta, rm, rv, nbt, eps, mom = bn
    return _ConvC3BN.apply(x4, w, bias, gamma, beta, rm, rv, nbt, float(eps), float(mom), int(stride), ACT[post_act])


class _DwConv(_FastFunction):
    @staticmethod
    def forward(ctx, x, w, bias, stride, add_input, fork=False, stats_box=None, xab=None, xlink=None):
        ctx.set_materialize_grads(False)
        _chk(x, w, bias)
        N, H, W, C = x.shape
        Ho, Wo = (H - 1) // stride + 1, (W - 1) // stride + 1
        y = torch.empty((N, Ho, Wo, C), device=x.device, dtype=x.dtype)
        ctx.xab = xab
        ctx.xlink = xlink
        if xab is not None:
            if add_input or fork or C % 4 or C > 256:
                raise TcctError('dwconv3x3(deferred=...): plain convolution with C % 4 == 0, C <= 256 only')
            sums = None
            if stats_box is not None:
                sums = ZERO.get((2 * C,), torch.float64, x.device) if ZERO.active else torch.zeros(2 * C, device=x.device, dtype=torch.float64)
                stats_box[0] = sums
            lib.dwconv3x3_fwd_xaff(x, xab, w, bias, y, N, H, W, C, stride, sums, dtype_code(x.dtype))
        elif stats_box is not None and C % 4 == 0 and C <= 256:
            sums = ZERO.get((2 * C,), torch.float64, x.device) if ZERO.active else torch.zeros(2 * C, device=x.device, dtype=torch.float64)
            lib.dwconv3x3_fwd_bnstats(x, w, bias, y, N, H, W, C, stride, int(add_input), sums, dtype_code(x.dtype))
            stats_box[0] = sums
        else:
            lib.dwconv3x3_fwd(x, w, bias, y, N, H, W, C, stride, int(add_input), dtype_code(x.dtype))
        ctx.save_for_backward(x, w)
        ctx.cfg = (stride, add_input, bias is not None)
        ctx.bias_param = bias
        return (y, x.view_as(x)) if fork else y

    @staticmethod
    def backward(ctx, dy, dskip=None):
        x, w = ctx.saved_tensors
        stride, add_input, has_bias = ctx.cfg
        if dy is None:
            return dskip, None, None, None, None, None, None, None, None
        dy = _as(dy, x.dtype)
        N, H, W, C = x.shape
        dx = dw = db = None
        if ctx.needs_input_grad[0]:
            dx = torch.empty_like(x)
            if dskip is not None:
                lib.dwconv3x3_dgrad_add(dy, w, _as(dskip, x.dtype), dx, N, H, W, C, stride, int(add_input), dtype_code(x.dtype))
            elif ctx.xab is not None and ctx.xlink is not None and stride == 1 and BN_FUSE_RED and BN_RED_DW:
                raw = ZERO.get((2 * C,), torch.float64, x.device) if ZERO.active else torch.zeros(2 * C, device=x.device, dtype=torch.float64)
                lib.dwconv3x3_dgrad_bnred(dy, w, x, ctx.xab, dx, raw, N, H, W, C, dtype_code(x.dtype))
                ctx.xlink.sums = raw
            else:
                lib.dwconv3x3_dgrad(dy, w, dx, N, H, W, C, stride, int(add_input), dtype_code(x.dtype))
        if ctx.needs_input_grad[1] or (has_bias and ctx.needs_input_grad[2]):
            keep = (x, dy) if ctx.xab is None else (x, dy, ctx.xab)
            with _wgrad_stream(DW_WGRAD_SIDE and _slot_written(w, ctx.bias_param if has_bias else None), *keep):
                dw = _grad_out(w)
                db = _grad_out(ctx.bias_param) if has_bias else None
                if ctx.xab is not None:
                    lib.dwconv3x3_wgrad_xaff(x, ctx.xab, dy, dw, db, N, H, W, C, stride, dtype_code(x.dtype))
                else:
                    lib.dwconv3x3_wgrad(x, dy, dw, db, N, H, W, C, stride, dtype_code(x.dtype))
        return dx, _ret(dw, w), _ret(db, ctx.bias_param), None, None, None, None, None, None


def dwconv3x3(x, w, bias=None, stride=1, add_input=False, bn_stats=False, deferred=None):
    xab = deferred.ab if deferred is not None else None
    if bn_stats:
        box = [None]
        y = _DwConv.apply(x, w, bias, stride, add_input, False, box, xab, deferred)
        if box[0] is not None:
            y._bn_sums = (box[0], ACT['none'])
        return y
    return _DwConv.apply(x, w, bias, stride, add_input, False, None, xab, deferred)


def dwconv3x3_fork(x, w, bias=None, stride=1, add_input=False):
    if not (torch.is_grad_enabled() and x.requires_grad):
        return dwconv3x3(x, w, bias, stride, add_input), x
    return _DwConv.apply(x, w, bias, stride, add_input, True)


class _BatchNorm(_FastFunction):
    @staticmethod
    def forward(ctx, x, gamma, beta, rm, rv, nbt, eps, momentum, pre, post, training, res=None, link=None):
        _chk(x, gamma, beta)
        C = x.shape[-1]
        M = x.numel() // C
        dc = dtype_code(x.dtype)
        mean_rstd = torch.empty(2 * C, device=x.device, dtype=torch.float32)
        ab = torch.empty(2 * C, device=x.device, dtype=torch.float32)
        if training:
            fused = getattr(x, '_bn_sums', None)
            if fused is not None and fused[1] == pre and fused[0].numel() == 2 * C:
                sums = fused[0]
            else:
                sums = ZERO.get((2 * C,), torch.float64, x.device)
                lib.bn_stats(x, M, C, pre, sums, dc)
        else:
            lib.bn_eval_ab(C, gamma, beta, eps, rm, rv, mean_rstd, ab)
        y = torch.empty_like(x)
        if res is not None:
            _chk(res)
            if res.shape != x.shape or res.dtype != x.dtype:
                raise TcctError('batchnorm: residual must have the shape and dtype of the input')
        if training:
            lib.bn_apply_train(x, res, y, M, C, sums, gamma, beta, eps, momentum, rm, rv, nbt, mean_rstd, ab, pre, post, dc)
        elif res is not None:
            lib.bn_apply_add(x, res, y, M, C, ab, pre, post, dc)
        else:
            lib.bn_apply(x, y, M, C, ab, pre, post, dc)
        if training:
            ctx.save_for_backward(x, gamma, mean_rstd, ab)
            ctx.cfg = (pre, post)
            ctx.beta_param = beta
            ctx.has_res = res is not None
            ctx.link = link
            if link is not None:
                link.y, link.ab = x, ab
        return y

    @staticmethod
    def backward(ctx, dy):
        x, gamma, mean_rstd, ab = ctx.saved_tensors
        pre, post = ctx.cfg
        dy = _as(dy, x.dtype)
        C = x.shape[-1]
        M = x.numel() // C
        dc = dtype_code(x.dtype)
        link = getattr(ctx, 'link', None)
        if link is not None and link.sums is not None:
            sums = torch.empty(2 * C, device=x.device, dtype=torch.float64)
            lib.bn_sums_from_raw(link.sums, mean_rstd, C, sums)
            link.sums = None
        else:
            sums = ZERO.get((2 * C,), torch.float64, x.device)
            lib.bn_bwd_reduce(x, dy, M, C, mean_rstd, ab, pre, post, sums, dc)
        dx = torch.empty_like(x)
        dg = _grad_out(gamma) if ZERO.active and getattr(gamma, '_grad_slot', None) is not None else torch.empty(C, device=x.device, dtype=torch.float32)
        db = _grad_out(ctx.beta_param) if ZERO.active and getattr(ctx.beta_param, '_grad_slot', None) is not None else torch.empty(C, device=x.device, dtype=torch.float32)
        lib.bn_bwd_apply(x, dy, dx, M, C, mean_rstd, ab, gamma, sums, pre, post, dg, db, dc)
        return dx, _ret(dg, gamma), _ret(db, ctx.beta_param), None, None, None, None, None, None, None, None, (dy if ctx.has_res else None), None


BN_FUSE = True
BN_FUSE_RED = True


class BnLink:
    __slots__ = ('y', 'ab', 'post', 'sums')

    def __init__(self, y, ab, post):
        self.y, self.ab, self.post, self.sums = y, ab, post, None


def _bn_link_of(x, final):
    if not (final and BN_FUSE and BN_FUSE_RED):
        return None
    return getattr(x, '_bn_link', None)


class _PwConvBN(_FastFunction):

    @staticmethod
    def forward(ctx, x, x2, w, bias, gamma, beta, rm, rv, nbt, eps, momentum, post, res, fork, link, prev, xdef=None, defer_apply=False):
        ctx.set_materialize_grads(False)
        _chk(x, x2, w, bias, gamma, beta, res)
        K1 = x.shape[-1]
        K = K1 + (x2.shape[-1] if x2 is not None else 0)
        N = w.shape[0]
        M = x.numel() // K1
        y = torch.empty(x.shape[:-1] + (N,), device=x.device, dtype=x.dtype)
        sums = ZERO.get((2 * N,), torch.float64, x.device) if ZERO.active else torch.zeros(2 * N, device=x.device, dtype=torch.float64)
        if xdef is not None:
            lib.pw_fwd_bnstats_xaff(x, xdef, w, bias, y, M, K, N, sums)
        elif x2 is not None:
            lib.pw_fwd_cat2(x, x2, K1, w, bias, y, M, K, N, sums, 0)
        else:
            lib.pw_fwd_bnstats(x, w, bias, y, M, K, N, sums, 0)
        mean_rstd = torch.empty(2 * N, device=x.device, dtype=torch.float32)
        ab = torch.empty(2 * N, device=x.device, dtype=torch.float32)
        if defer_apply:
            lib.bn_finalize(sums, M, N, gamma, beta, eps, momentum, rm, rv, nbt, mean_rstd, ab)
            z = y.view_as(y)
        else:
            z = torch.empty_like(y)
            lib.bn_apply_train(y, res, z, M, N, sums, gamma, beta, eps, momentum, rm, rv, nbt, mean_rstd, ab, 0, post, dtype_code(y.dtype))
        ctx.save_for_backward(x, x2, w, y, mean_rstd, ab)
        wsrc = w if hasattr(w, '_grad_slot') or w._base is None else w._base
        ctx.cfg = (post, res is not None, wsrc, bias, gamma, beta, link, prev, M, K, N)
        ctx.xdef = xdef
        link.y, link.ab = y, ab
        return (z, x.view_as(x)) if fork else z

    @staticmethod
    def backward(ctx, dz, dalias=None):
        x, x2, w, y, mean_rstd, ab = ctx.saved_tensors
        post, has_res, wsrc, bsrc, gamma, beta, link, prev, M, K, N = ctx.cfg
        if dz is None:
            return (dalias,) + (None,) * 17
        dz = _as(dz, y.dtype)
        if link.sums is not None:
            sums, raw = link.sums, 1
            link.sums = None
        else:
            sums, raw = ZERO.get((2 * N,), torch.float64, y.device), 0
            lib.bn_bwd_reduce(y, dz, M, N, mean_rstd, ab, 0, post, sums, dtype_code(y.dtype))
        dg = _grad_out(gamma) if ZERO.active and getattr(gamma, '_grad_slot', None) is not None else torch.empty(N, device=y.device, dtype=torch.float32)
        db_ = _grad_out(beta) if ZERO.active and getattr(beta, '_grad_slot', None) is not None else torch.empty(N, device=y.device, dtype=torch.float32)
        dx = torch.empty_like(x)
        dx2 = torch.empty_like(x2) if x2 is not None else None
        dw = _grad_out(wsrc, tuple(w.shape))
        dbias = _grad_out(bsrc) if bsrc is not None else None
        ypv = abp = sp = None
        redp = -1
        if prev is not None:
            redp = prev.post
            ypv, abp = prev.y, prev.ab
            sp = prev.sums = ZERO.get((2 * x.shape[-1],), torch.float64, y.device)
        dskip = _as(dalias, x.dtype) if dalias is not None else None
        if ctx.xdef is not None:
            lib.pw_bwd_bn_sums_xaff(x, ctx.xdef, dz, y, sums, raw, mean_rstd, ab, dg, db_, w, dskip, dx, dw, dbias, M, K, N, redp, sp)
        else:
            lib.pw_bwd_bn_sums(x, x2, dz, y, sums, raw, mean_rstd, ab, dg, db_, post, w, dskip, dx, dx2, dw, dbias, M, K, N, ypv, abp, redp, sp)
        return (dx, dx2, _ret(dw, wsrc), _ret(dbias, bsrc), _ret(dg, gamma), _ret(db_, beta), None, None, None, None, None, None,
                (dz if has_res else None), None, None, None, None, None)


class _Affine2Add(_FastFunction):

    @staticmethod
    def forward(ctx, y1, ab1, y2, ab2, link1=None, link2=None):
        _chk(y1, ab1, y2, ab2)
        z = torch.empty_like(y1)
        C = y1.shape[-1]
        lib.affine2_add(y1, ab1, y2, ab2, z, y1.numel() // C, C, dtype_code(y1.dtype))
        ctx.links = (link1, link2)
        if link1 is not None and link2 is not None:
            ctx.save_for_backward(y1, y2)
        return z

    @staticmethod
    def backward(ctx, dz):
        l1, l2 = ctx.links
        if l1 is not None and l2 is not None and BN_FUSE_RED and TRAN_RED2:
            y1, y2 = ctx.saved_tensors
            dz = _as(dz, y1.dtype)
            C = y1.shape[-1]
            dev = y1.device
            r1 = ZERO.get((2 * C,), torch.float64, dev) if ZERO.active else torch.zeros(2 * C, device=dev, dtype=torch.float64)
            r2 = ZERO.get((2 * C,), torch.float64, dev) if ZERO.active else torch.zeros(2 * C, device=dev, dtype=torch.float64)
            lib.bn_bwd_reduce2_raw(y1, y2, dz, y1.numel() // C, C, r1, r2, dtype_code(y1.dtype))
            l1.sums, l2.sums = r1, r2
        return dz, None, dz, None, None, None


TRAN_RED2 = True
TRAN_FUSE = True


def affine2_add(y1, link1, y2, link2):
    if y1.shape != y2.shape or y1.dtype != y2.dtype or y1.shape[-1] % 8:
        raise TcctError('affine2_add: two NHWC tensors of one shape and dtype, channels a multiple of 8')
    return _Affine2Add.apply(y1, link1.ab, y2, link2.ab, link1, link2)


BN_RED_DW = True
BN_DEFER_DW = True
BN_DEFER = True


class _BatchNormDeferred(_FastFunction):

    @staticmethod
    def forward(ctx, x, gamma, beta, rm, rv, nbt, eps, momentum, post, link):
        _chk(x, gamma, beta)
        C = x.shape[-1]
        M = x.numel() // C
        fused = getattr(x, '_bn_sums', None)
        if fused is not None and fused[1] == 0 and fused[0].numel() == 2 * C:
            sums = fused[0]
        else:
            sums = ZERO.get((2 * C,), torch.float64, x.device) if ZERO.active else torch.zeros(2 * C, device=x.device, dtype=torch.float64)
            lib.bn_stats(x, M, C, 0, sums, dtype_code(x.dtype))
        mean_rstd = torch.empty(2 * C, device=x.device, dtype=torch.float32)
        ab = torch.empty(2 * C, device=x.device, dtype=torch.float32)
        lib.bn_finalize(sums, M, C, gamma, beta, eps, momentum, rm, rv, nbt, mean_rstd, ab)
        ctx.save_for_backward(x, gamma, mean_rstd, ab)
        ctx.cfg = (0, post)
        ctx.beta_param = beta
        ctx.has_res = False
        ctx.link = link
        link.y, link.ab = x, ab
        return x.view_as(x)

    backward = None


def _bn_deferred_backward(ctx, dy):
    out = _BatchNorm.backward(ctx, dy)
    return out[0], out[1], out[2], None, None, None, None, None, None, None


_BatchNormDeferred.backward = staticmethod(_bn_deferred_backward)


def batchnorm_deferred_ok(x, bn_training, post_act):
    return (BN_DEFER and BN_FUSE and bn_training and torch.is_grad_enabled() and x.dtype == torch.bfloat16 and x.dim() == 4 and x.shape[-1] in (64, 96)
            and ACT[post_act] == ACT['hswish'] and x.numel() * 2 < 2 ** 31)


def batchnorm_deferred(x, gamma, beta, running_mean, running_var, num_batches_tracked, eps, momentum, post_act):
    link = BnLink(None, None, ACT[post_act])
    y = _BatchNormDeferred.apply(x, gamma, beta, running_mean, running_var, num_batches_tracked, float(eps), float(momentum), ACT[post_act], link)
    return y, link


def pw_conv_bn_ok(x, w, bias, bn_training, pre_act, post_act, x2=None, prev=None):
    if not (BN_FUSE and FUSED_PW_BWD and bn_training and torch.is_grad_enabled() and ACT[pre_act] == 0):
        return False
    if x.dtype != torch.bfloat16 or x.dim() != 4 or not x.is_cuda or (w.dim() == 4 and tuple(w.shape[2:]) != (1, 1)):
        return False
    K = x.shape[-1] + (x2.shape[-1] if x2 is not None else 0)
    N = w.shape[0]
    if x2 is not None and not (x.shape[-1] == 64 and x2.shape == x.shape and x2.dtype == x.dtype):
        return False
    M = x.numel() // x.shape[-1]
    if w.shape[1] != K or M * max(K, N) * 2 >= 2 ** 31:
        return False
    return bool(lib.pw_bwd_bn_supported(K, N, ACT[post_act], -1 if prev is None else prev.post, 1 if x2 is not None else 0))


def pw_conv_bn(x, w, bias, bn, post_act=None, residual=None, fork=False, x2=None, x_final=False, deferred=None, defer_apply=False):
    gamma, beta, rm, rv, nbt, eps, mom = bn
    link = BnLink(None, None, ACT[post_act])
    w4 = w.view(w.shape[0], w.shape[1], 1, 1) if w.dim() == 2 else w
    if deferred is not None:
        if post_act is not None or fork or x2 is not None or x.shape[-1] != w.shape[0] or x.shape[-1] not in (64, 96):
            raise TcctError('pw_conv_bn(deferred=...): square 64 / 96 convolution without activation, fork or concatenation only')
        prev = deferred if (x.shape[-1] == 64 and BN_FUSE_RED) else None
        out = _PwConvBN.apply(x, None, w4, bias, gamma, beta, rm, rv, nbt, float(eps), float(mom), 0, residual, False, link, prev, deferred.ab)
        out._bn_link = link
        return out
    prev = _bn_link_of(x, x_final)
    if prev is not None and not pw_conv_bn_ok(x, w, bias, True, None, post_act, x2, prev):
        prev = None
    if defer_apply:
        if residual is not None or x2 is not None or ACT[post_act] not in (ACT['hswish'], ACT['none']):
            raise TcctError('pw_conv_bn(defer_apply=True): BatchNorm (+ Hardswish) without residual / concatenation only')
        out = _PwConvBN.apply(x, None, w4, bias, gamma, beta, rm, rv, nbt, float(eps), float(mom), ACT[post_act], None, fork, link, prev, None, True)
        return out, link
    out = _PwConvBN.apply(x, x2, w4, bias, gamma, beta, rm, rv, nbt, float(eps), float(mom), ACT[post_act], residual, fork, link, prev)
    z = out[0] if fork else out
    z._bn_link = link
    return out


BN_POOL_FUSE = True


class _BnPoolFork(_FastFunction):

    @staticmethod
    def forward(ctx, x, gamma, beta, rm, rv, nbt, eps, momentum, pre, post):
        ctx.set_materialize_grads(False)
        _chk(x, gamma, beta)
        N, H, W, C = x.shape
        dc = dtype_code(x.dtype)
        fused = getattr(x, '_bn_sums', None)
        if fused is not None and fused[1] == pre and fused[0].numel() == 2 * C:
            sums = fused[0]
        else:
            sums = ZERO.get((2 * C,), torch.float64, x.device)
            lib.bn_stats(x, N * H * W, C, pre, sums, dc)
        mean_rstd = torch.empty(2 * C, device=x.device, dtype=torch.float32)
        ab = torch.empty(2 * C, device=x.device, dtype=torch.float32)
        z = torch.empty_like(x)
        pooled = torch.empty((N, H // 2, W // 2, C), device=x.device, dtype=x.dtype)
        amax = torch.empty((N, H // 2, W // 2, C // 4), device=x.device, dtype=torch.uint8)
        lib.bn_pool_fwd_train(x, z, pooled, amax, N, H, W, C, sums, gamma, beta, eps, momentum, rm, rv, nbt, mean_rstd, ab, pre, post, dc)
        ctx.save_for_backward(x, mean_rstd, ab, amax)
        ctx.cfg = (pre, post, gamma, beta)
        return pooled, z

    @staticmethod
    def backward(ctx, dpool, dskip):
        x, mean_rstd, ab, amax = ctx.saved_tensors
        pre, post, gamma, beta = ctx.cfg
        N, H, W, C = x.shape
        dc = dtype_code(x.dtype)
        if dpool is None and dskip is None:
            return (None,) * 10
        if dpool is None:
            dpool = torch.zeros((N, H // 2, W // 2, C), device=x.device, dtype=x.dtype)
        dpool = _as(dpool, x.dtype)
        if dskip is not None:
            dskip = _as(dskip, x.dtype)
        sums = ZERO.get((2 * C,), torch.float64, x.device)
        dx = torch.empty_like(x)
        dg = _grad_out(gamma) if ZERO.active and getattr(gamma, '_grad_slot', None) is not None else torch.empty(C, device=x.device, dtype=torch.float32)
        db = _grad_out(beta) if ZERO.active and getattr(beta, '_grad_slot', None) is not None else torch.empty(C, device=x.device, dtype=torch.float32)
        lib.bn_pool_bwd(x, dpool, dskip, amax, dx, N, H, W, C, mean_rstd, ab, pre, post, sums, dg, db, dc)
        return dx, _ret(dg, gamma), _ret(db, beta), None, None, None, None, None, None, None


def bn_pool_ok(x, training):
    N, H, W, C = x.shape
    return (BN_POOL_FUSE and training and torch.is_grad_enabled() and x.requires_grad and C % 4 == 0 and C <= 256 and 256 % (C // 4) == 0
            and H % 2 == 0 and W % 2 == 0 and H >= 2 and W >= 2)


def batchnorm_maxpool2_fork(x, gamma, beta, running_mean, running_var, num_batches_tracked=None, eps=1e-5, momentum=0.1, pre_act=None,
                            post_act=None):
    return _BnPoolFork.apply(x, gamma, beta, running_mean, running_var, num_batches_tracked, float(eps), float(momentum), ACT[pre_act], ACT[post_act])


def batchnorm(x, gamma, beta, running_mean, running_var, num_batches_tracked=None, eps=1e-5, momentum=0.1,
              pre_act=None, post_act=None, training=True, residual=None):
    if not training and torch.is_grad_enabled() and x.requires_grad:
        raise TcctError('eval-mode batchnorm is inference-only here')
    link = None
    if (BN_FUSE and training and torch.is_grad_enabled() and x.dtype == torch.bfloat16 and ACT[pre_act] == 0
            and ACT[post_act] in (0, 2) and x.shape[-1] in (64, 96, 128)):
        link = BnLink(None, None, ACT[post_act])
    z = _BatchNorm.apply(x, gamma, beta, running_mean, running_var, num_batches_tracked, float(eps), float(momentum),
                         ACT[pre_act], ACT[post_act], bool(training), residual, link)
    if link is not None:
        z._bn_link = link
    return z


class _Bn2AddAct(_FastFunction):

    @staticmethod
    def forward(ctx, xa, gA, bA, xb, gB, bB, bufs, eps, momentum, pre, act_kind):
        _chk(xa, xb, gA, bA, gB, bB)
        C = xa.shape[-1]
        M = xa.numel() // C
        dc = dtype_code(xa.dtype)
        st, ss = [], []
        for x, g, b, (rm, rv, nbt) in ((xa, gA, bA, bufs[0]), (xb, gB, bB, bufs[1])):
            fused = getattr(x, '_bn_sums', None)
            if fused is not None and fused[1] == pre and fused[0].numel() == 2 * C:
                sums = fused[0]
            else:
                sums = ZERO.get((2 * C,), torch.float64, x.device)
                lib.bn_stats(x, M, C, pre, sums, dc)
            mr = torch.empty(2 * C, device=x.device, dtype=torch.float32)
            ab = torch.empty(2 * C, device=x.device, dtype=torch.float32)
            st += [mr, ab]
            ss.append(sums)
        y = torch.empty_like(xa)
        (rmA, rvA, nbtA), (rmB, rvB, nbtB) = bufs
        lib.bn2_add_act_train(xa, xb, y, M, C, ss[0], gA, bA, rmA, rvA, nbtA, st[0], st[1], ss[1], gB, bB, rmB, rvB, nbtB, st[2], st[3],
                              eps, momentum, pre, act_kind, dc)
        ctx.save_for_backward(xa, xb, *st)
        ctx.cfg = (pre, act_kind)
        ctx.params = (gA, bA, gB, bB)
        return y

    @staticmethod
    def backward(ctx, dy):
        xa, xb, mrA, abA, mrB, abB = ctx.saved_tensors
        pre, act_kind = ctx.cfg
        gA, bA, gB, bB = ctx.params
        dy = _as(dy, xa.dtype)
        C = xa.shape[-1]
        M = xa.numel() // C
        dc = dtype_code(xa.dtype)
        sums = ZERO.get((4 * C,), torch.float64, xa.device)
        lib.bn2_add_act_bwd_reduce(xa, xb, dy, M, C, mrA, abA, mrB, abB, pre, act_kind, sums, dc)
        dxa, dxb = torch.empty_like(xa), torch.empty_like(xb)
        outs = []
        for p in (gA, bA, gB, bB):
            use_slot = ZERO.active and getattr(p, '_grad_slot', None) is not None
            outs.append(_grad_out(p) if use_slot else torch.empty(C, device=xa.device, dtype=torch.float32))
        lib.bn2_add_act_bwd_apply(xa, xb, dy, dxa, dxb, M, C, mrA, abA, mrB, abB, sums, pre, act_kind, outs[0], outs[1], outs[2],
                                  outs[3], dc)
        return (dxa, _ret(outs[0], gA), _ret(outs[1], bA), dxb, _ret(outs[2], gB), _ret(outs[3], bB), None, None, None, None, None)


def bn2_add_act(xa, bnA, xb, bnB, pre_act='lrelu', act_kind='gelu'):
    gA, bA, rmA, rvA, nbtA, eps, mom = bnA
    gB, bB, rmB, rvB, nbtB, _, _ = bnB
    return _Bn2AddAct.apply(xa, gA, bA, xb, gB, bB, ((rmA, rvA, nbtA), (rmB, rvB, nbtB)), float(eps), float(mom), ACT[pre_act],
                            ACT[act_kind])


class _LayerNorm(_FastFunction):
    @staticmethod
    def forward(ctx, x, gamma, beta, eps, fork=False):
        ctx.set_materialize_grads(False)
        _chk(x, gamma, beta)
        C = x.shape[-1]
        M = x.numel() // C
        y = torch.empty_like(x)
        mr = torch.empty(2 * M, device=x.device, dtype=torch.float32)
        lib.layernorm_fwd(x, y, M, C, gamma, beta, eps, mr, dtype_code(x.dtype))
        ctx.save_for_backward(x, gamma, mr)
        ctx.beta_param = beta
        return (y, x.view_as(x)) if fork else y

    @staticmethod
# ... 911 lines not shown
```

Before: 414.8 B-scans/s.

## Defer ViT-stage BatchNorm through stride-2 dwconv fork and transition convs

Extends deferred BatchNorm application so the aggregate output's BN is never materialised. Consumers instead apply the affine on load: the stride-2 forked dwconv, and the 96/128->32 transition pointwise convs through new x-affine MFMA kernel variants. Adds a stride-2 dwconv dgrad kernel that also reduces the previous BN's backward sums, which removes separate apply and reduce passes. The cost is more complex graph bookkeeping, with a node-order check that raises an error if the sums are not delivered.

```diff
diff --git a/include/tcct_hip.h b/include/tcct_hip.h
--- a/include/tcct_hip.h
+++ b/include/tcct_hip.h
@@ -250,6 +250,8 @@
                               tcct_stream_t stream);
 int tcct_dwconv3x3_dgrad_bnred(const void* dy, const float* w, const void* y_prev, const float* ab_prev, void* dx, double* raw, int N, int H, int W, int C,
                                int dtype, tcct_stream_t stream);
+int tcct_dwconv3x3_dgrad_s2_bnred(const void* dy, const float* w, const void* res, const void* y_prev, const float* ab_prev, void* dx, double* raw,
+                                  int N, int H, int W, int C, int dtype, tcct_stream_t stream);
 
 int tcct_metapool_fwd(const void* x, void* y, int B, int64_t N, int C, int dtype, tcct_stream_t stream);
 int tcct_metapool_bwd(const void* dy, void* dx, int B, int64_t N, int C, int dtype, tcct_stream_t stream);
diff --git a/tcct_amd/csrc/dwconv.hip b/tcct_amd/csrc/dwconv.hip
--- a/tcct_amd/csrc/dwconv.hip
+++ b/tcct_amd/csrc/dwconv.hip
@@ -353,13 +353,22 @@
     TCCT_LAUNCH_OK();
 }
 
-template <typename T, int VEC>
+template <typename T, int VEC, bool BNRED = false>
 __global__ void __launch_bounds__(DB) k_dw_dgrad_s2(const T* __restrict__ dy, const float* __restrict__ w, T* __restrict__ dx,
                                                     int N, int H, int W, int C, int Ho, int Wo, int segh, int wblocks, int hstrips,
-                                                    const T* __restrict__ res) {
+                                                    const T* __restrict__ res, const T* __restrict__ yp = nullptr, const float* __restrict__ xab = nullptr,
+                                                    double* __restrict__ stats = nullptr) {
+    static_assert(!BNRED || VEC == 4, "the reduction epilogue needs 4-channel vectors");
+    typedef typename std::conditional<sizeof(T) == 4, double, float>::type SAcc;
+    __shared__ SAcc s_red[BNRED ? DB * 8 : 1];
     const int Qh = (H + 1) / 2, Qw = (W + 1) / 2;
     DwPos p;
-    if (!dw_pos(C, VEC, Qh, Qw, segh, wblocks, hstrips, p)) return;
+    const bool has_work = dw_pos(C, VEC, Qh, Qw, segh, wblocks, hstrips, p);
+    if (!has_work && !BNRED) return;
+    SAcc st_s[VEC], st_q[VEC];
+#pragma unroll
+    for (int k = 0; k < VEC; ++k) st_s[k] = st_q[k] = 0;
+    if (has_work) {
     float wk[9][VEC];
 #pragma unroll
     for (int k = 0; k < VEC; ++k)
@@ -375,6 +384,10 @@
         const __amdgpu_buffer_rsrc_t rg = __builtin_amdgcn_make_buffer_rsrc((void*)(dy + (int64_t)nu * Ho * Wo * C), 0, (uint32_t)Ho * Wo * C * ES, 0x00020000);
         const __amdgpu_buffer_rsrc_t ro = __builtin_amdgcn_make_buffer_rsrc((void*)(dx + (int64_t)nu * H * W * C), 0, in_bytes, 0x00020000);
         const __amdgpu_buffer_rsrc_t rr = __builtin_amdgcn_make_buffer_rsrc((void*)((res ? res : dx) + (int64_t)nu * H * W * C), 0, res ? in_bytes : 0u, 0x00020000);
+        const __amdgpu_buffer_rsrc_t rq = __builtin_amdgcn_make_buffer_rsrc((void*)((BNRED ? yp : dx) + (int64_t)nu * H * W * C), 0, BNRED ? in_bytes : 0u, 0x00020000);
+        float xa[VEC], xb[VEC];
+#pragma unroll
+        for (int k = 0; k < VEC; ++k) { xa[k] = BNRED ? xab[p.c + k] : 1.f; xb[k] = BNRED ? xab[C + p.c + k] : 0.f; }
         const uint32_t cg0 = (uint32_t)(b * C + p.c) * ES, cg1 = b + 1 < Wo ? cg0 + (uint32_t)C * ES : DW_OOB;
         const uint32_t co0 = (uint32_t)(2 * b * C + p.c) * ES, co1 = 2 * b + 1 < W ? co0 + (uint32_t)C * ES : DW_OOB;
         auto ldb = [&](Raw<T, VEC> (&d)[2], int a) {
@@ -383,15 +396,26 @@
             d[0].loadb(rg, rok ? r0 + cg0 : DW_OOB);
             d[1].loadb(rg, (rok && cg1 != DW_OOB) ? r0 + cg1 : DW_OOB);
         };
-        auto ldr = [&](Raw<T, VEC> (&q)[4], int a, bool live) {
+        auto ldq = [&](Raw<T, VEC> (&q)[4], __amdgpu_buffer_rsrc_t rs, int a, bool live) {
             const uint32_t r0 = (uint32_t)(2 * a) * (uint32_t)(W * C) * ES, r1 = r0 + (uint32_t)(W * C) * ES;
             const bool row1 = live && 2 * a + 1 < H;
-            q[0].loadb(rr, live ? r0 + co0 : DW_OOB);
-            q[1].loadb(rr, (live && co1 != DW_OOB) ? r0 + co1 : DW_OOB);
-            q[2].loadb(rr, row1 ? r1 + co0 : DW_OOB);
-            q[3].loadb(rr, (row1 && co1 != DW_OOB) ? r1 + co1 : DW_OOB);
-        };
-        auto emitb = [&](const Raw<T, VEC> (&u)[2], const Raw<T, VEC> (&v)[2], const Raw<T, VEC> (&q)[4], int a, bool live) {
+            q[0].loadb(rs, live ? r0 + co0 : DW_OOB);
+            q[1].loadb(rs, (live && co1 != DW_OOB) ? r0 + co1 : DW_OOB);
+            q[2].loadb(rs, row1 ? r1 + co0 : DW_OOB);
+            q[3].loadb(rs, (row1 && co1 != DW_OOB) ? r1 + co1 : DW_OOB);
+        };
+        auto ldr = [&](Raw<T, VEC> (&q)[4], int a, bool live) { ldq(q, rr, a, live); };
+        auto ldy = [&](Raw<T, VEC> (&q)[4], int a, bool live) { if (BNRED) ldq(q, rq, a, live); };
+        auto red1 = [&](const float (&o)[VEC], const Raw<T, VEC>& yv, bool live) {
+            if (!BNRED || !live) return;
+#pragma unroll
+            for (int k = 0; k < VEC; ++k) {
+                const float yy = yv.get(k), uu = xa[k] * yy + xb[k];
+                const float d = dw_rnd(o[k], (const T*)nullptr) * (uu < -3.f ? 0.f : (uu <= 3.f ? (2.f * uu + 3.f) * (1.f / 6.f) : 1.f));
+                st_s[k] += (SAcc)d; st_q[k] += (SAcc)d * (SAcc)yy;
+            }
+        };
+        auto emitb = [&](const Raw<T, VEC> (&u)[2], const Raw<T, VEC> (&v)[2], const Raw<T, VEC> (&q)[4], const Raw<T, VEC> (&yq)[4], int a, bool live) {
             float o00[VEC], o01[VEC], o10[VEC], o11[VEC];
 #pragma unroll
             for (int k = 0; k < VEC; ++k) {
@@ -407,23 +431,30 @@
             dw_storeb(ro, (live && co1 != DW_OOB) ? r0 + co1 : DW_OOB, o01, (const T*)nullptr);
             dw_storeb(ro, row1 ? r1 + co0 : DW_OOB, o10, (const T*)nullptr);
             dw_storeb(ro, (row1 && co1 != DW_OOB) ? r1 + co1 : DW_OOB, o11, (const T*)nullptr);
+            red1(o00, yq[0], live); red1(o01, yq[1], live && co1 != DW_OOB); red1(o10, yq[2], row1); red1(o11, yq[3], row1 && co1 != DW_OOB);
         };
         Raw<T, VEC> d0[2], d1[2], d2[2], n1[2], n2[2], q0[4], q1[4], m0[4], m1[4];
+        Raw<T, VEC> y0[4], y1[4], ym0[4], ym1[4];
         ldb(d0, p.ho0); ldb(d1, p.ho0 + 1); ldb(d2, p.ho0 + 2);
         ldr(q0, p.ho0, true); ldr(q1, p.ho0 + 1, p.ho0 + 1 < p.ho1);
+        ldy(y0, p.ho0, true); ldy(y1, p.ho0 + 1, p.ho0 + 1 < p.ho1);
         for (int a = p.ho0; a < p.ho1; a += 2) {
             const bool more = a + 2 < p.ho1;
             ldb(n1, more ? a + 3 : Ho); ldb(n2, more ? a + 4 : Ho);
             ldr(m0, a + 2, more); ldr(m1, a + 3, a + 3 < p.ho1);
-            emitb(d0, d1, q0, a, true);
-            emitb(d1, d2, q1, a + 1, a + 1 < p.ho1);
+            ldy(ym0, a + 2, more); ldy(ym1, a + 3, a + 3 < p.ho1);
+            emitb(d0, d1, q0, y0, a, true);
+            emitb(d1, d2, q1, y1, a + 1, a + 1 < p.ho1);
 #pragma unroll
             for (int j = 0; j < 2; ++j) { d0[j] = d2[j]; d1[j] = n1[j]; d2[j] = n2[j]; }
 #pragma unroll
             for (int j = 0; j < 4; ++j) { q0[j] = m0[j]; q1[j] = m1[j]; }
-        }
-        return;
-    }
+            if (BNRED) {
+#pragma unroll
+                for (int j = 0; j < 4; ++j) { y0[j] = ym0[j]; y1[j] = ym1[j]; }
+            }
+        }
+    } else {
     auto ld = [&](float (&d)[2][VEC], int a) {
 #pragma unroll
         for (int j = 0; j < 2; ++j) {
@@ -482,6 +513,20 @@
         if (a + 1 >= p.ho1) break;
         ld(d0, a + 2);
         emit(d1, d0, a + 1);
+    }
+    }
+    }
+    if (BNRED) {
+        const int CV = C / VEC, PW = DB / CV, t = threadIdx.x;
+#pragma unroll
+        for (int k = 0; k < VEC; ++k) { s_red[t * 8 + k] = st_s[k]; s_red[t * 8 + 4 + k] = st_q[k]; }
+        __syncthreads();
+        if (t < C) {
+            const int cvv = t / VEC, k = t % VEC;
+            double sa = 0.0, sb = 0.0;
+            for (int pp = 0; pp < PW; ++pp) { sa += (double)s_red[(pp * CV + cvv) * 8 + k]; sb += (double)s_red[(pp * CV + cvv) * 8 + 4 + k]; }
+            atomicAdd(&stats[t], sa); atomicAdd(&stats[C + t], sb);
+        }
     }
 }
 
@@ -522,6 +567,19 @@
     TCCT_CHECK(N >= 1 && H >= 1 && W >= 1 && C >= 4 && C % 4 == 0 && C <= DB && y_prev && ab_prev && raw, "dwconv3x3_dgrad_bnred: needs C %% 4 == 0, C <= 256, y_prev, ab_prev, raw");
     TCCT_CHECK((int64_t)H * W * C * 4 < (1ll << 31), "dwconv3x3_dgrad_bnred: one image of %d x %d x %d elements exceeds the 32-bit byte offsets of the kernels", H, W, C);
     TCCT_DISPATCH(dtype, (dw_fwd_launch<T, 4, true, 2>(dy, w, nullptr, dx, N, H, W, C, 1, H, W, 0, (hipStream_t)stream, y_prev, raw, ab_prev)));
+    TCCT_LAUNCH_OK();
+}
+
+extern "C" int tcct_dwconv3x3_dgrad_s2_bnred(const void* dy, const float* w, const void* res, const void* y_prev, const float* ab_prev, void* dx, double* raw,
+                                             int N, int H, int W, int C, int dtype, tcct_stream_t stream) {
+    TCCT_CHECK(N >= 1 && H >= 1 && W >= 1 && C >= 4 && C % 4 == 0 && C <= DB && y_prev && ab_prev && raw, "dwconv3x3_dgrad_s2_bnred: needs C %% 4 == 0, C <= 256, y_prev, ab_prev, raw");
+    TCCT_CHECK((int64_t)H * W * C * 4 < (1ll << 31), "dwconv3x3_dgrad_s2_bnred: one image of %d x %d x %d elements exceeds the 32-bit byte offsets of the kernels", H, W, C);
+    const int Ho = (H - 1) / 2 + 1, Wo = (W - 1) / 2 + 1;
+    int segh, wblocks, hstrips;
+    dw_geometry(N, (H + 1) / 2, (W + 1) / 2, C, 4, 1024, 32, segh, wblocks, hstrips);
+    dim3 g((unsigned)((int64_t)N * wblocks * hstrips)), b(DB);
+    TCCT_DISPATCH(dtype, hipLaunchKernelGGL((k_dw_dgrad_s2<T, 4, true>), g, b, 0, (hipStream_t)stream, (const T*)dy, w, (T*)dx, N, H, W, C, Ho, Wo, segh, wblocks, hstrips,
+                                            (const T*)res, (const T*)y_prev, ab_prev, raw));
     TCCT_LAUNCH_OK();
 }
 
diff --git a/tcct_amd/csrc/pw_mfma.hip b/tcct_amd/csrc/pw_mfma.hip
--- a/tcct_amd/csrc/pw_mfma.hip
+++ b/tcct_amd/csrc/pw_mfma.hip
@@ -1214,7 +1214,8 @@
                                         const float* mean_rstd, const float* ab, float* dgamma, float* dbeta, const float* w, const void* res, void* dx,
                                         float* dw, float* dbias, int64_t M, int K, int N, int red_post, double* sums_prev, tcct_stream_t stream) {
     TCCT_CHECK(y_prev && ab_prev && sums && mean_rstd && ab && dgamma && dbeta, "pw_bwd_bn_sums_xaff: NULL argument");
-    TCCT_CHECK(K == N && ((K == 64 && red_post == TCCT_ACT_HSWISH && sums_prev) || (K == 96 && red_post < 0)), "pw_bwd_bn_sums_xaff: K=%d N=%d red_post=%d unsupported", K, N, red_post);
+    TCCT_CHECK((K == N && ((K == 64 && red_post == TCCT_ACT_HSWISH && sums_prev) || (K == 96 && red_post < 0))) || (N == 32 && (K == 96 || K == 128) && red_post < 0),
+               "pw_bwd_bn_sums_xaff: K=%d N=%d red_post=%d unsupported", K, N, red_post);
     if (red_post >= 0 && !tcct_skip_zero_fill() && hipMemsetAsync(sums_prev, 0, sizeof(double) * 2 * K, (hipStream_t)stream) != hipSuccess) { tcct_set_error("pw_bwd_bn_sums_xaff: memset failed"); return -2; }
     return pw_bwd_impl(y_prev, dz, w, res, dx, nullptr, dw, dbias, M, K, N, stream, false, TCCT_ACT_NONE, red_post,
                        PwBnBwd{(const bf16*)y, nullptr, (const bf16*)y_prev, ab_prev, sums_prev, sums, raw, mean_rstd, ab, dgamma, dbeta}, false, TCCT_ACT_HSWISH);
@@ -1289,8 +1290,12 @@
     if (xap >= 0) {
 #define BLXA(NTV, RDV) { static bool at_ = false; if (!at_) { (void)hipFuncSetAttribute((const void*)k_pw_bwd<NTV, NTV, false, 0, RDV, false, 2>, hipFuncAttributeMaxDynamicSharedMemorySize, 160 * 1024); at_ = true; } \
         hipLaunchKernelGGL((k_pw_bwd<NTV, NTV, false, 0, RDV, false, 2>), dim3((unsigned)gx), dim3(PWB), lds, st, (const bf16*)x, (const bf16*)dy, w, (const bf16*)res, (bf16*)dx, (bf16*)dx_plain, dw, dbias, M, bn); }
-        if (NT == 2 && redp == TCCT_ACT_HSWISH) BLXA(2, 2) else if (NT == 3 && redp < 0) BLXA(3, -1)
-        else { tcct_set_error("pw_bwd: x-affine form K=N=%d red_post=%d has no kernel", K, redp); return -1; }
+#define BLXN(KTV) { static bool at_ = false; if (!at_) { (void)hipFuncSetAttribute((const void*)k_pw_bwd<1, KTV, false, 0, -1, false, 2>, hipFuncAttributeMaxDynamicSharedMemorySize, 160 * 1024); at_ = true; } \
+        hipLaunchKernelGGL((k_pw_bwd<1, KTV, false, 0, -1, false, 2>), dim3((unsigned)gx), dim3(PWB), lds, st, (const bf16*)x, (const bf16*)dy, w, (const bf16*)res, (bf16*)dx, (bf16*)dx_plain, dw, dbias, M, bn); }
+        if (NT == 1 && KT == 3 && redp < 0) BLXN(3) else if (NT == 1 && KT == 4 && redp < 0) BLXN(4)
+        else if (NT == 2 && KT == 2 && redp == TCCT_ACT_HSWISH) BLXA(2, 2) else if (NT == 3 && KT == 3 && redp < 0) BLXA(3, -1)
+        else { tcct_set_error("pw_bwd: x-affine form K=%d N=%d red_post=%d has no kernel", K, N, redp); return -1; }
+#undef BLXN
 #undef BLXA
         TCCT_LAUNCH_OK();
     }
@@ -1539,6 +1544,8 @@
         hipLaunchKernelGGL((k_pw_fwd2<T, T, false, false, true, true>), dim3((unsigned)gx), dim3(PWB), lds, st, (const bf16*)x, (const bf16*)x2, w, bias, (bf16*)y, M, stats, stat_pre, pr); }
 #define F2A(T) { static bool at_ = false; if (!at_) { (void)hipFuncSetAttribute((const void*)k_pw_fwd2<T, T, true, false, false, false, 2>, hipFuncAttributeMaxDynamicSharedMemorySize, 160 * 1024); at_ = true; } \
         hipLaunchKernelGGL((k_pw_fwd2<T, T, true, false, false, false, 2>), dim3((unsigned)gx), dim3(PWB), lds, st, (const bf16*)x, (const bf16*)x2, w, bias, (bf16*)y, M, stats, stat_pre, pr); }
+#define F2AN(KTV) { static bool at_ = false; if (!at_) { (void)hipFuncSetAttribute((const void*)k_pw_fwd2<1, KTV, true, false, false, false, 2>, hipFuncAttributeMaxDynamicSharedMemorySize, 160 * 1024); at_ = true; } \
+        hipLaunchKernelGGL((k_pw_fwd2<1, KTV, true, false, false, false, 2>), dim3((unsigned)gx), dim3(PWB), lds, st, (const bf16*)x, (const bf16*)x2, w, bias, (bf16*)y, M, stats, stat_pre, pr); }
 #define F2F(NTV, KTV, SPV, RSV) { static bool at_ = false; if (!at_) { (void)hipFuncSetAttribute((const void*)k_pw_fwd2<NTV, KTV, false, SPV, RSV, false, -1, true>, hipFuncAttributeMaxDynamicSharedMemorySize, 160 * 1024); at_ = true; } \
         hipLaunchKernelGGL((k_pw_fwd2<NTV, KTV, false, SPV, RSV, false, -1, true>), dim3((unsigned)gx), dim3(PWB), lds, st, (const bf16*)x, (const bf16*)x2, w, bias, (bf16*)y, M, stats, stat_pre, pr); }
 #define F2X(T) { static bool at_ = false; if (!at_) { (void)hipFuncSetAttribute((const void*)k_pw_fwd2<T, T, false, false, true, false, 2, true>, hipFuncAttributeMaxDynamicSharedMemorySize, 160 * 1024); at_ = true; } \
@@ -1553,7 +1560,10 @@
         else { if (NT == 2) F2F(2, 2, false, false) else if (NT == 3) F2F(3, 3, false, false) else F2F(4, 4, false, false) }
     }
     else
-    if (pr.xab) { if (NT == 2) F2A(2) else F2A(3) }
+    if (pr.xab) {
+        if (NT == 1 && KT == 3) F2AN(3) else if (NT == 1 && KT == 4) F2AN(4)
+        else if (NT == 2) F2A(2) else F2A(3)
+    }
     else
     if (gelu_x) { if (NT == 2) F2G(2) else F2G(3) }
     else
@@ -1562,6 +1572,7 @@
 #undef F2X
 #undef F2F
 #undef F2G
+#undef F2AN
 #undef F2A
 #undef F2RK
 #undef F2R
@@ -1577,7 +1588,8 @@
 }
 extern "C" int tcct_pw_fwd_bnstats_xaff(const void* y_prev, const float* ab_prev, const float* w, const float* bias, void* y, int64_t M, int K, int N,
                                         double* stats, tcct_stream_t stream) {
-    TCCT_CHECK(K == N && (K == 64 || K == 96) && ab_prev && stats, "pw_fwd_bnstats_xaff: K=%d N=%d unsupported (64 or 96 square) or NULL argument", K, N);
+    TCCT_CHECK(((K == N && (K == 64 || K == 96)) || (N == 32 && (K == 96 || K == 128))) && ab_prev && stats,
+               "pw_fwd_bnstats_xaff: K=%d N=%d unsupported (64 or 96 square, 96 / 128 -> 32) or NULL argument", K, N);
     TCCT_CHECK(M > 0 && M * (int64_t)K * 2 < (1LL << 31), "pw_fwd_bnstats_xaff: tensor exceeds the 2 GiB buffer-descriptor range");
     return pw_fwd2_launch(y_prev, nullptr, w, bias, y, M, K, N, stats, 0, stream, PwRes{nullptr, nullptr, 1, nullptr, ab_prev});
 }
diff --git a/tcct_amd/nets/tcct.py b/tcct_amd/nets/tcct.py
--- a/tcct_amd/nets/tcct.py
+++ b/tcct_amd/nets/tcct.py
@@ -187,7 +187,7 @@
     def forward(self, x, fork=False, deferred=None):
         if fork:
             m = self.dwconv
-            d, alias = ops.dwconv3x3_fork(x, m.weight, m.bias, stride=m.stride[0])
+            d, alias = ops.dwconv3x3_fork(x, m.weight, m.bias, stride=m.stride[0], deferred=deferred)
             return _conv_bn(self.pwconv, self.bn, d, post='hswish'), alias
         return _conv_bn(self.pwconv, self.bn, _dw(self.dwconv, x, deferred=deferred), post='hswish')
 
@@ -371,7 +371,11 @@
         self.InvRes = ResBlock(embed_dim)
         self.aggregate = Conv2d_BN(embed_dim * 2, out_embed_dim, act=True)
 
-    def forward(self, x, scales):
+    def forward(self, x, scales, defer_out=False):
+        out = self._forward(x, scales, defer_out)
+        return (out if isinstance(out, tuple) else (out, None)) if defer_out else out
+
+    def _forward(self, x, scales, defer_out):
         if torch.is_grad_enabled() and x.requires_grad:
             c1 = self.InvRes.conv1
             flink = None
@@ -403,6 +407,8 @@
         ag = self.aggregate
         if ag.bn.training or torch.is_grad_enabled() or not ops.INFER_FUSE:
             if ops.pw_conv_bn_ok(r, ag.conv.weight, None, ag.bn.training, None, 'hswish', x2=e):
+                if defer_out:
+                    return ops.pw_conv_bn(r, ag.conv.weight, None, _bn_args(ag.bn), 'hswish', x2=e, x_final=True, defer_apply=True)
                 return ops.pw_conv_bn(r, ag.conv.weight, None, _bn_args(ag.bn), 'hswish', x2=e, x_final=True)
             y = ops.conv1x1_cat2(r, e, ag.conv.weight, stats_pre='none' if ag.bn.training else None)
             return _bn(ag.bn, y, post='hswish')
@@ -482,19 +488,25 @@
             pass
         return xs
 
-    def iter_stages(self, x, xs):
+    def iter_stages(self, x, xs, pending=None):
         scales = self._dp_scales(x.shape[0], x.device)
         x = self.stem[0](x)
         d0 = self.stem[1].forward_deferred(x)
         x, link0 = d0 if d0 is not None else (self.stem[1](x), None)
+        link = None
         for i in range(4):
             if i == 1:
                 x = ops.grad_mark(x, 'deep')
             if i > 0 and torch.is_grad_enabled() and x.requires_grad:
-                p, xs[-1] = self.patch_embed_stages[i](x, fork=True)
+                p, xs[-1] = self.patch_embed_stages[i](x, fork=True, deferred=link)
             else:
                 p = self.patch_embed_stages[i](x, deferred=link0 if i == 0 else None)
-            x = self.mhca_stages[i](p, scales[i])
+            if (i < 2 and pending is not None and ops.BN_DEFER_AGG and torch.is_grad_enabled() and p.requires_grad
+                    and self.patch_embed_stages[i + 1].patch_embeds[0].patch_conv.dwconv.stride[0] == 2 and p.shape[-1] % 4 == 0 and p.shape[-1] <= 256
+                    and pending(i, p)):
+                x, link = self.mhca_stages[i](p, scales[i], defer_out=True)
+            else:
+                x, link = self.mhca_stages[i](p, scales[i]), None
             xs.append(x)
             yield i
 
@@ -608,16 +620,31 @@
         ops.lib.image_to_nhwc4(x, out, B, Cs, H, W, W, ops.dtype_code(self.compute_dtype))
         return out
 
+    def _vit_pending_ok(self, i, y):
+        tv = getattr(self, f'tran_vit{i}')
+        yo = y.new_empty((1, 1, 1, tv[0].in_channels))
+        return (tv[1].training and ops.pw_conv_bn_deferred_ok(yo, tv[0].weight) and y.numel() // y.shape[-1] * tv[0].in_channels * 2 < 2 ** 31
+                and ops.pw_conv_bn_ok(yo, tv[0].weight, tv[0].bias, True, None, None))
+
     def forward(self, x):
         size = (x.shape[2], x.shape[3])
         x = self._to_nhwc4(x)
         mho = self.main_head_only and not torch.is_grad_enabled() and not self.training
         if self.flag_vit and self.flag_cnn:
             cs, vs = [], []
-            ops.run_interleaved('vit', self.base_cnn.iter_levels(x, cs), self.base_vit.iter_stages(x, vs), vs)
-            (c1, c2, c3, c4, c5), (v2, v3, v4, v5) = [ops.grad_mark(t, 'dec') for t in cs], [ops.grad_mark(t, 'dec') for t in vs]
+            pend = self._vit_pending_ok if (self.training and not self.flag_gate) else None
+            ops.run_interleaved('vit', self.base_cnn.iter_levels(x, cs), self.base_vit.iter_stages(x, vs, pend), vs)
+            (c1, c2, c3, c4, c5) = [ops.grad_mark(t, 'dec') for t in cs]
+            (v2, v3, v4, v5) = [ops.keep_pending(t, ops.grad_mark(t, 'dec')) for t in vs]
             def fuse_level(j, v, c):
                 tv, tc = getattr(self, f'tran_vit{j}'), getattr(self, f'tran_cnn{j}')
+                lp = getattr(v, '_bn_pending', None)
+                if lp is not None:
+                    if ops.TRAN_FUSE and c.shape[-1] % 8 == 0 and ops.pw_conv_bn_ok(c, tc[0].weight, tc[0].bias, tc[1].training, None, None):
+                        yv, lv = ops.pw_conv_bn(v, tv[0].weight, tv[0].bias, _bn_args(tv[1]), None, deferred=lp, defer_apply=True)
+                        yc, lc = ops.pw_conv_bn(c, tc[0].weight, tc[0].bias, _bn_args(tc[1]), None, defer_apply=True)
+                        return ops.affine2_add(yv, lv, yc, lc)
+                    return _conv_bn(tc[0], tc[1], c, residual=ops.pw_conv_bn(v, tv[0].weight, tv[0].bias, _bn_args(tv[1]), None, deferred=lp))
                 if self.flag_gate and self.training:
                     a1, a2 = _conv_bn(tv[0], tv[1], v), _conv_bn(tc[0], tc[1], c)
                     B_, Hh, Ww, Cc = a1.shape
diff --git a/tcct_amd/ops.py b/tcct_amd/ops.py
--- a/tcct_amd/ops.py
+++ b/tcct_amd/ops.py
@@ -1586,8 +1586,8 @@
         ctx.xab = xab
         ctx.xlink = xlink
         if xab is not None:
-            if add_input or fork or C % 4 or C > 256:
-                raise TcctError('dwconv3x3(deferred=...): plain convolution with C % 4 == 0, C <= 256 only')
+            if add_input or (fork and stride != 2) or C % 4 or C > 256:
+                raise TcctError('dwconv3x3(deferred=...): plain convolution (forked: stride 2) with C % 4 == 0, C <= 256 only')
             sums = None
             if stats_box is not None:
                 sums = ZERO.get((2 * C,), torch.float64, x.device) if ZERO.active else torch.zeros(2 * C, device=x.device, dtype=torch.float64)
@@ -1609,13 +1609,20 @@
         x, w = ctx.saved_tensors
         stride, add_input, has_bias = ctx.cfg
         if dy is None:
+            if ctx.xlink is not None:
+                ctx.xlink.expect = False
             return dskip, None, None, None, None, None, None, None, None
         dy = _as(dy, x.dtype)
         N, H, W, C = x.shape
         dx = dw = db = None
         if ctx.needs_input_grad[0]:
             dx = torch.empty_like(x)
-            if dskip is not None:
+            if ctx.xab is not None and ctx.xlink is not None and stride == 2 and BN_FUSE_RED:
+                raw = ZERO.get((2 * C,), torch.float64, x.device) if ZERO.active else torch.zeros(2 * C, device=x.device, dtype=torch.float64)
+                lib.dwconv3x3_dgrad_s2_bnred(dy, w, _as(dskip, x.dtype) if dskip is not None else None, x, ctx.xab, dx, raw, N, H, W, C,
+                                             dtype_code(x.dtype))
+                ctx.xlink.sums = raw
+            elif dskip is not None:
                 lib.dwconv3x3_dgrad_add(dy, w, _as(dskip, x.dtype), dx, N, H, W, C, stride, int(add_input), dtype_code(x.dtype))
             elif ctx.xab is not None and ctx.xlink is not None and stride == 1 and BN_FUSE_RED and BN_RED_DW:
                 raw = ZERO.get((2 * C,), torch.float64, x.device) if ZERO.active else torch.zeros(2 * C, device=x.device, dtype=torch.float64)
@@ -1646,7 +1653,21 @@
     return _DwConv.apply(x, w, bias, stride, add_input, False, None, xab, deferred)
 
 
-def dwconv3x3_fork(x, w, bias=None, stride=1, add_input=False):
+def keep_pending(src, dst):
+    lp = getattr(src, '_bn_pending', None)
+    if lp is not None and dst is not src:
+        dst._bn_pending = lp
+    return dst
+
+
+def dwconv3x3_fork(x, w, bias=None, stride=1, add_input=False, deferred=None):
+    if deferred is not None:
+        if not (torch.is_grad_enabled() and x.requires_grad):
+            raise TcctError('dwconv3x3_fork(deferred=...): training with gradients only')
+        y, alias = _DwConv.apply(x, w, bias, stride, add_input, True, None, deferred.ab, deferred)
+        alias._bn_pending = deferred
+        deferred.expect = stride == 2 and BN_FUSE_RED
+        return y, alias
     if not (torch.is_grad_enabled() and x.requires_grad):
         return dwconv3x3(x, w, bias, stride, add_input), x
     return _DwConv.apply(x, w, bias, stride, add_input, True)
@@ -1719,10 +1740,11 @@
 
 
 class BnLink:
-    __slots__ = ('y', 'ab', 'post', 'sums')
+    __slots__ = ('y', 'ab', 'post', 'sums', 'expect')
 
     def __init__(self, y, ab, post):
         self.y, self.ab, self.post, self.sums = y, ab, post, None
+        self.expect = False
 
 
 def _bn_link_of(x, final):
@@ -1774,6 +1796,8 @@
         if link.sums is not None:
             sums, raw = link.sums, 1
             link.sums = None
+        elif link.expect:
+            raise TcctError('pw_conv_bn: the consumers of the pending BatchNorm did not deliver its backward sums (node order)')
         else:
             sums, raw = ZERO.get((2 * N,), torch.float64, y.device), 0
             lib.bn_bwd_reduce(y, dz, M, N, mean_rstd, ab, 0, post, sums, dtype_code(y.dtype))
@@ -1839,6 +1863,7 @@
 BN_RED_DW = True
 BN_DEFER_DW = True
 BN_DEFER = True
+BN_DEFER_AGG = True
 
 
 class _BatchNormDeferred(_FastFunction):
@@ -1887,6 +1912,12 @@
     return y, link
 
 
+def pw_conv_bn_deferred_ok(x, w, post_act=None):
+    K, N = x.shape[-1], w.shape[0]
+    return (post_act is None and w.shape[1] == K and (w.dim() == 2 or tuple(w.shape[2:]) == (1, 1)) and x.dtype == torch.bfloat16 and x.dim() == 4
+            and ((K == N and K in (64, 96)) or (N == 32 and K in (96, 128))) and x.numel() // K * max(K, N) * 2 < 2 ** 31)
+
+
 def pw_conv_bn_ok(x, w, bias, bn_training, pre_act, post_act, x2=None, prev=None):
     if not (BN_FUSE and FUSED_PW_BWD and bn_training and torch.is_grad_enabled() and ACT[pre_act] == 0):
         return False
@@ -1907,19 +1938,22 @@
     link = BnLink(None, None, ACT[post_act])
     w4 = w.view(w.shape[0], w.shape[1], 1, 1) if w.dim() == 2 else w
     if deferred is not None:
-        if post_act is not None or fork or x2 is not None or x.shape[-1] != w.shape[0] or x.shape[-1] not in (64, 96):
-            raise TcctError('pw_conv_bn(deferred=...): square 64 / 96 convolution without activation, fork or concatenation only')
-        prev = deferred if (x.shape[-1] == 64 and BN_FUSE_RED) else None
-        out = _PwConvBN.apply(x, None, w4, bias, gamma, beta, rm, rv, nbt, float(eps), float(mom), 0, residual, False, link, prev, deferred.ab)
+        if not pw_conv_bn_deferred_ok(x, w, post_act) or fork or x2 is not None or (defer_apply and residual is not None):
+            raise TcctError('pw_conv_bn(deferred=...): square 64 / 96 or 96 / 128 -> 32 convolution without activation, fork or concatenation only')
+        prev = deferred if (x.shape[-1] == 64 and w.shape[0] == 64 and BN_FUSE_RED) else None
+        out = _PwConvBN.apply(x, None, w4, bias, gamma, beta, rm, rv, nbt, float(eps), float(mom), 0, residual, False, link, prev, deferred.ab,
+                              defer_apply)
+        if defer_apply:
+            return out, link
         out._bn_link = link
         return out
     prev = _bn_link_of(x, x_final)
     if prev is not None and not pw_conv_bn_ok(x, w, bias, True, None, post_act, x2, prev):
         prev = None
     if defer_apply:
-        if residual is not None or x2 is not None or ACT[post_act] not in (ACT['hswish'], ACT['none']):
-            raise TcctError('pw_conv_bn(defer_apply=True): BatchNorm (+ Hardswish) without residual / concatenation only')
-        out = _PwConvBN.apply(x, None, w4, bias, gamma, beta, rm, rv, nbt, float(eps), float(mom), ACT[post_act], None, fork, link, prev, None, True)
+        if residual is not None or (x2 is not None and fork) or ACT[post_act] not in (ACT['hswish'], ACT['none']):
+            raise TcctError('pw_conv_bn(defer_apply=True): BatchNorm (+ Hardswish) without residual only')
+        out = _PwConvBN.apply(x, x2, w4, bias, gamma, beta, rm, rv, nbt, float(eps), float(mom), ACT[post_act], None, fork, link, prev, None, True)
         return out, link
     out = _PwConvBN.apply(x, x2, w4, bias, gamma, beta, rm, rv, nbt, float(eps), float(mom), ACT[post_act], residual, fork, link, prev)
     z = out[0] if fork else out
```

After: 419.0 B-scans/s (median of 6 runs). 1.01x the previous value.
